# settylab/Mellon

Hardware: AMD Instinct MI355X
Metric: cells/sec fit_predict (higher is better)
Workload: dtype f64

## Files before the change

include/mellon_hip.h:

```cpp
#ifndef MELLON_HIP_H
#define MELLON_HIP_H

#include <stdint.h>

#ifdef __cplusplus
extern "C" {
#endif

typedef struct mln_ctx mln_ctx;
typedef struct mln_fit mln_fit;

typedef enum {
  MLN_OK = 0,
  MLN_ERR_NOT_PD = 1,
  MLN_ERR_SHAPE = 2,
  MLN_ERR_HIP = 3,
  MLN_ERR_RCCL = 4,
  MLN_ERR_ARG = 5,
  MLN_ERR_UNSUPPORTED = 6,
  MLN_ERR_NOCONV = 7
} mln_status;

typedef enum {
  MLN_K_MATERN32 = 1,
  MLN_K_MATERN52 = 2,
  MLN_K_EXPQUAD = 3,
  MLN_K_EXPONENTIAL = 4,
  MLN_K_RATQUAD = 5,
  MLN_K_LINEAR = 6,
  MLN_K_DISTANCE = 7
} mln_kind;

typedef struct {
  int32_t kind;
  int32_t ndims;
  double ls;
  double alpha;
  const int32_t* dims;
} mln_leaf;

typedef enum { MLN_OP_LEAF = 0, MLN_OP_CONST = 1, MLN_OP_ADD = 2, MLN_OP_MUL = 3, MLN_OP_POW = 4 } mln_op;

typedef struct {
  int32_t op;
  int32_t leaf;
  double value;
} mln_tok;

#define MLN_MAX_LEAVES 4
#define MLN_MAX_TOKS 16
#define MLN_MAX_DIMS 256

typedef struct {
  int32_t n_leaves;
  int32_t n_toks;
  const mln_leaf* leaves;
  const mln_tok* toks;
} mln_kernel_desc;

int mln_ctx_create(int device, mln_ctx** out);
void mln_ctx_destroy(mln_ctx* ctx);
const char* mln_last_error(mln_ctx* ctx);
int mln_device_info(mln_ctx* ctx, char* name, int name_cap, int* n_cu, int64_t* mem_bytes);
int mln_device_count(int* count_out);
int mln_synchronize(mln_ctx* ctx);

int mln_malloc(mln_ctx* ctx, int64_t bytes, void** dev_ptr);
int mln_free(mln_ctx* ctx, void* dev_ptr);
int mln_memcpy(mln_ctx* ctx, void* dst, const void* src, int64_t bytes);
int mln_host_register(mln_ctx* ctx, const void* host_ptr, int64_t bytes);
int mln_host_unregister(mln_ctx* ctx, const void* host_ptr);
int mln_release_cached_memory(void);
int mln_diag_alloc_stats(int64_t* out);

#define MLN_UNIQUE_ID_BYTES 128
int mln_comm_unique_id(void* id_out );
int mln_comm_init(mln_ctx* ctx, const void* id, int n_ranks, int rank);
int mln_comm_allreduce_sum(mln_ctx* ctx, double* buf, int64_t count);
typedef struct mln_loopback mln_loopback;
int mln_loopback_create(int n_ranks , mln_loopback** out);
void mln_loopback_destroy(mln_loopback* group);
int mln_comm_init_loopback(mln_ctx* ctx, mln_loopback* group, int rank);
typedef int (*mln_host_collective_fn)(void* user, int op, double* buf, double* buf2, int64_t count);
int mln_comm_init_host(mln_ctx* ctx, int n_ranks, int rank, mln_host_collective_fn fn, void* user);
void mln_loopback_abort(mln_loopback* group);
int mln_comm_info(mln_ctx* ctx, int32_t* info, double* stats, int32_t flags);

int mln_kernel_matrix(mln_ctx* ctx, const mln_kernel_desc* cov, const double* x, int64_t n,
                      const double* y, int64_t m, int32_t d, double* out);

int mln_kernel_gram(mln_ctx* ctx, const mln_kernel_desc* cov, const double* x, int64_t n_local, int32_t d,
                    const double* xu, int64_t m, double* out );
int mln_nn_distances(mln_ctx* ctx, const double* x, int64_t n, const double* y, int64_t m, int32_t d,
                     int64_t self_offset, double* out );
int mln_knn(mln_ctx* ctx, const double* x, int64_t n, const double* y, int64_t m, int32_t d, int32_t k,
            int32_t exclude, int64_t self_offset, double* dist , int64_t* idx );
int mln_local_dimensionality(mln_ctx* ctx, const double* x, int64_t n, int32_t d, const int64_t* nbr, int64_t q,
                             int32_t k, double* out );

int mln_kmeans(mln_ctx* ctx, const double* x, int64_t n, int32_t d, int64_t m, int64_t seed,
               int32_t max_iter, double tol, double* centers, int32_t* n_iter_out, double* inertia_out);
int mln_kmeans_sklearn(mln_ctx* ctx, const double* x, int64_t n, int32_t d, int64_t m, int64_t first_id,
                       const double* uniforms, int32_t n_local_trials, int32_t max_iter, double tol, double* centers,
                       int64_t* indices_out, int32_t* n_iter_out, double* inertia_out);

int mln_chol_lower(mln_ctx* ctx, double* A, int64_t m, double add_diag);

int mln_trsm_lower(mln_ctx* ctx, const double* Lf, int64_t m, int32_t trans, double* B, int64_t p);

#define MLN_FIT_IMPLICIT 1
int mln_fit_prepare(mln_ctx* ctx, const mln_kernel_desc* cov, const double* x, int64_t n_local,
                    int32_t d, const double* xu, int64_t m, double jitter, const double* Lp_in,
                    int32_t flags, mln_fit** out);
int mln_fit_from_L(mln_ctx* ctx, const double* L, int64_t n_local, int64_t m, const double* Lp,
                   mln_fit** out);
#define MLN_FIT_FULL 2
#define MLN_FIT_DEFER_LP 4
int mln_fit_prepare_from_K(mln_ctx* ctx, const double* Kuu, int64_t n_local, int64_t m, double jitter,
                           const double* Lp_in, int32_t flags, mln_fit** out);
int mln_fit_set_K_rows(mln_fit* fit, int64_t row0, int64_t n_rows, const double* K_rows);
int mln_fit_finish_K(mln_fit* fit);
int mln_gemm(mln_ctx* ctx, int32_t ta, int32_t tb, int64_t M, int64_t N, int64_t K, double alpha, const double* A,
             int64_t lda, const double* B, int64_t ldb, double beta, double* C, int64_t ldc);
int mln_ewise(mln_ctx* ctx, int32_t op, const double* a, const double* b, double scalar, double* out, int64_t count);

void mln_fit_destroy(mln_fit* fit);
int mln_fit_get_Lp(mln_fit* fit, double* out );
int mln_fit_get_L(mln_fit* fit, int64_t row0, int64_t n_rows, double* out );
int mln_fit_rank(mln_fit* fit, int64_t* m_out);

int mln_kernel_grad(mln_ctx* ctx, const mln_kernel_desc* cov, const double* x, int64_t n, const double* y,
                    int64_t m, int32_t d, double* out );
int mln_predict_gradient(mln_ctx* ctx, const mln_kernel_desc* cov, const double* xnew, int64_t n_new,
                         int32_t d, const double* centers, int64_t m, const double* W ,
                         double* out );
int mln_predict_hessian(mln_ctx* ctx, const mln_kernel_desc* cov, const double* xnew, int64_t n_new, int32_t d,
                        const double* centers, int64_t m, const double* W , double* out);


int mln_eigh(mln_ctx* ctx, const double* A, int64_t m, double* w, double* V, int32_t* n_sweeps);
int mln_fit_gram_eigh(mln_fit* fit, double* w , int32_t* n_sweeps);
int mln_fit_gram_rank(mln_fit* fit, double tol, int64_t* rank_out, double* sigma_max_out);
int mln_fit_project(mln_fit* fit, int64_t p, mln_fit** out);

int mln_ridge_init(mln_fit* fit, const double* target, double* z0 );

int mln_precond_build(mln_fit* fit, int64_t row_stride );
int mln_fit_set_row_offset(mln_fit* fit, int64_t global_row0);
int mln_precond_apply(mln_fit* fit, int32_t mode, const double* in, double* out);
int mln_objective_precond(mln_fit* fit, const double* u, double* loss, double* grad_u ,
                          double* z_out );

int mln_fit_set_likelihood(mln_fit* fit, const double* V, const double* Vdr, double mu);

int mln_objective(mln_fit* fit, const double* z, double* loss, double* grad ,
                  double* hess_diag );

int mln_objective_batch(mln_fit* fit, const double* Z, int32_t S, double* loss , double* grad );

typedef struct {
  int32_t maxiter;
  int32_t maxcor;
  int32_t maxls;
  double ftol;
  double gtol;
} mln_solver_opts;
int mln_map_solve(mln_fit* fit, const double* z0, const mln_solver_opts* opts ,
                  double* z_out , double* loss_out, int32_t* n_eval_out, int32_t* n_iter_out,
                  int32_t* status_out);

int mln_fit_set_dim_likelihood(mln_fit* fit, const double* ell, int32_t k, double mu_dim, double mu_dens);
int mln_dim_objective(mln_fit* fit, const double* z, double* loss, double* grad ,
                      double* hess_diag );

int mln_dim_objective_batch(mln_fit* fit, const double* Z, int32_t S, double* loss , double* grad );

int mln_transform(mln_fit* fit, const double* z, double mu, double* f_out );

int mln_weights_cholesky(mln_fit* fit, const double* z, double* w );
int mln_weights_full(mln_fit* fit, const double* y, int64_t p, double mu, double* w );

int mln_sparse_solve(mln_ctx* ctx, const mln_kernel_desc* cov, const double* x, int64_t n_local,
                     int32_t d, const double* xu, int64_t m, const double* y, int64_t p, double mu,
                     double sigma, double jitter, double* W );
int mln_sparse_solve_factors(mln_ctx* ctx, const mln_kernel_desc* cov, const double* x, int64_t n_local,
                             int32_t d, const double* xu, int64_t m, const double* y, int64_t p, double mu,
                             double sigma, double jitter, double* W, double* Lp_out, double* Cs_out);

enum { MLN_SIGMA_SCALAR = 0, MLN_SIGMA_PER_OUTPUT = 1, MLN_SIGMA_PER_CELL = 2 };
int mln_sparse_solve_noise(mln_ctx* ctx, const mln_kernel_desc* cov, const double* x, int64_t n_local,
                           int32_t d, const double* xu, int64_t m, const double* y, int64_t p, double mu,
                           const double* sigma, int32_t sigma_kind, double jitter, double* W );

int mln_full_conditional_noise(mln_ctx* ctx, const mln_kernel_desc* cov, const double* x, int64_t n, int32_t d,
                               const double* y, int64_t p, double mu, const double* sigma , double jitter,
                               double* W, double* leverage, double* corrected_r2, double* variance_W);

int mln_landmark_leverage(mln_ctx* ctx, const mln_kernel_desc* cov, const double* x, int64_t n_local, int32_t d,
                          const double* xu, int64_t m, const double* Lk, const double* sigma, int64_t p,
                          double jitter, double* out );

int mln_predict_mean(mln_ctx* ctx, const mln_kernel_desc* cov, const double* xnew, int64_t n_new,
                     int32_t d, const double* centers, int64_t m, const double* W, int64_t p,
                     double mu, double* out);

int mln_diag_peak(mln_ctx* ctx, int32_t what, int64_t bytes, double* result);
int mln_diag_dgemm(mln_ctx* ctx, int32_t ta, int32_t tb, int64_t M, int64_t N, int64_t K,
                   int32_t lower_only, int32_t split_k, int32_t reps, double* ms_out);
int mln_diag_dgemm_compare(mln_ctx* ctx, int32_t ta, int32_t tb, int64_t M, int64_t N, int64_t K, int32_t lower_only,
                           int32_t kmode, double beta, int32_t any_size, double* out);
int mln_diag_gram_i8(mln_ctx* ctx, const double* A, int64_t rows, int64_t m, double* out, int32_t reps, double* ms_out);
int mln_diag_overlap(mln_ctx* ctx, int64_t n, int64_t m, int32_t d, int64_t gram_rows, double* out );

int mln_predict_covariance(mln_ctx* ctx, const mln_kernel_desc* cov, const double* xnew, int64_t n_new,
                           int32_t d, const double* centers, int64_t m, const double* Lf, int32_t diag,
                           double* out);
int mln_predict_mean_covariance(mln_ctx* ctx, const mln_kernel_desc* cov, const double* xnew, int64_t n_new,
                                int32_t d, const double* centers, int64_t m, const double* W, int64_t q,
                                int32_t diag, double* out);

#define MLN_N_STAGE_TIMES 22
int mln_stage_times(mln_fit* fit, double* out );

#ifdef __cplusplus
}
#endif
#endif
```

mellon_amd/_lib.py:

```python
import ctypes as C
import os
import threading

import numpy as np

_HERE = os.path.dirname(os.path.abspath(__file__))
LIB_PATH = os.path.join(_HERE, "libmellon_hip.so")

MLN_OK, MLN_ERR_NOT_PD, MLN_ERR_SHAPE, MLN_ERR_HIP, MLN_ERR_RCCL, MLN_ERR_ARG, MLN_ERR_UNSUPPORTED = range(7)
MLN_UNIQUE_ID_BYTES = 128
MLN_N_STAGE_TIMES = 22

K_MATERN32, K_MATERN52, K_EXPQUAD, K_EXPONENTIAL, K_RATQUAD, K_LINEAR, K_DISTANCE = 1, 2, 3, 4, 5, 6, 7
OP_LEAF, OP_CONST, OP_ADD, OP_MUL, OP_POW = 0, 1, 2, 3, 4


HOST_COLLECTIVE_FN = C.CFUNCTYPE(C.c_int, C.c_void_p, C.c_int, C.c_void_p, C.c_void_p, C.c_int64)


class MellonHipError(RuntimeError):
    """HIP / RCCL / argument failure inside libmellon_hip.so."""


class Leaf(C.Structure):
    _fields_ = [("kind", C.c_int32), ("ndims", C.c_int32), ("ls", C.c_double), ("alpha", C.c_double),
                ("dims", C.POINTER(C.c_int32))]


class Tok(C.Structure):
    _fields_ = [("op", C.c_int32), ("leaf", C.c_int32), ("value", C.c_double)]


class SolverOpts(C.Structure):
    _fields_ = [("maxiter", C.c_int32), ("maxcor", C.c_int32), ("maxls", C.c_int32), ("ftol", C.c_double),
                ("gtol", C.c_double)]


class KernelDesc(C.Structure):
    _fields_ = [("n_leaves", C.c_int32), ("n_toks", C.c_int32), ("leaves", C.POINTER(Leaf)),
                ("toks", C.POINTER(Tok))]


_vp, _i64, _i32, _dbl, _dp = C.c_void_p, C.c_int64, C.c_int32, C.c_double, C.c_void_p
_KD = C.POINTER(KernelDesc)
SYMBOLS = [
    ("mln_ctx_create", C.c_int, [C.c_int, C.POINTER(_vp)]),
    ("mln_ctx_destroy", None, [_vp]),
    ("mln_last_error", C.c_char_p, [_vp]),
    ("mln_device_info", C.c_int, [_vp, C.c_char_p, C.c_int, C.POINTER(C.c_int), C.POINTER(_i64)]),
    ("mln_device_count", C.c_int, [C.POINTER(C.c_int)]),
    ("mln_synchronize", C.c_int, [_vp]),
    ("mln_malloc", C.c_int, [_vp, _i64, C.POINTER(_vp)]),
    ("mln_free", C.c_int, [_vp, _vp]),
    ("mln_memcpy", C.c_int, [_vp, _vp, _vp, _i64]),
    ("mln_host_register", C.c_int, [_vp, _vp, _i64]),
    ("mln_host_unregister", C.c_int, [_vp, _vp]),
    ("mln_release_cached_memory", C.c_int, []),
    ("mln_diag_alloc_stats", C.c_int, [_vp]),
    ("mln_comm_unique_id", C.c_int, [_vp]),
    ("mln_comm_init", C.c_int, [_vp, _vp, C.c_int, C.c_int]),
    ("mln_comm_allreduce_sum", C.c_int, [_vp, _dp, _i64]),
    ("mln_loopback_create", C.c_int, [C.c_int, C.POINTER(_vp)]),
    ("mln_loopback_destroy", None, [_vp]),
    ("mln_comm_init_loopback", C.c_int, [_vp, _vp, C.c_int]),
    ("mln_comm_init_host", C.c_int, [_vp, C.c_int, C.c_int, _vp, _vp]),
    ("mln_loopback_abort", None, [_vp]),
    ("mln_comm_info", C.c_int, [_vp, C.POINTER(_i32), _dp, _i32]),
    ("mln_kernel_matrix", C.c_int, [_vp, _KD, _dp, _i64, _dp, _i64, _i32, _dp]),
    ("mln_kernel_grad", C.c_int, [_vp, _KD, _dp, _i64, _dp, _i64, _i32, _dp]),
    ("mln_predict_gradient", C.c_int, [_vp, _KD, _dp, _i64, _i32, _dp, _i64, _dp, _dp]),
    ("mln_predict_hessian", C.c_int, [_vp, _KD, _dp, _i64, _i32, _dp, _i64, _dp, _dp]),
    ("mln_kernel_gram", C.c_int, [_vp, _KD, _dp, _i64, _i32, _dp, _i64, _dp]),
    ("mln_nn_distances", C.c_int, [_vp, _dp, _i64, _dp, _i64, _i32, _i64, _dp]),
    ("mln_knn", C.c_int, [_vp, _dp, _i64, _dp, _i64, _i32, _i32, _i32, _i64, _dp, _vp]),
    ("mln_local_dimensionality", C.c_int, [_vp, _dp, _i64, _i32, _vp, _i64, _i32, _dp]),
    ("mln_kmeans", C.c_int, [_vp, _dp, _i64, _i32, _i64, _i64, _i32, _dbl, _dp, C.POINTER(_i32), C.POINTER(_dbl)]),
    ("mln_kmeans_sklearn", C.c_int, [_vp, _dp, _i64, _i32, _i64, _i64, _dp, _i32, _i32, _dbl, _dp, _vp, C.POINTER(_i32),
                                     C.POINTER(_dbl)]),
    ("mln_chol_lower", C.c_int, [_vp, _dp, _i64, _dbl]),
    ("mln_trsm_lower", C.c_int, [_vp, _dp, _i64, _i32, _dp, _i64]),
    ("mln_fit_prepare", C.c_int, [_vp, _KD, _dp, _i64, _i32, _dp, _i64, _dbl, _dp, _i32, C.POINTER(_vp)]),
    ("mln_fit_from_L", C.c_int, [_vp, _dp, _i64, _i64, _dp, C.POINTER(_vp)]),
    ("mln_fit_prepare_from_K", C.c_int, [_vp, _dp, _i64, _i64, _dbl, _dp, _i32, C.POINTER(_vp)]),
    ("mln_fit_set_K_rows", C.c_int, [_vp, _i64, _i64, _dp]),
    ("mln_fit_finish_K", C.c_int, [_vp]),
    ("mln_gemm", C.c_int, [_vp, _i32, _i32, _i64, _i64, _i64, _dbl, _dp, _i64, _dp, _i64, _dbl, _dp, _i64]),
    ("mln_ewise", C.c_int, [_vp, _i32, _dp, _dp, _dbl, _dp, _i64]),
    ("mln_fit_destroy", None, [_vp]),
    ("mln_fit_get_Lp", C.c_int, [_vp, _dp]),
    ("mln_fit_get_L", C.c_int, [_vp, _i64, _i64, _dp]),
    ("mln_fit_rank", C.c_int, [_vp, C.POINTER(_i64)]),
    ("mln_eigh", C.c_int, [_vp, _dp, _i64, _dp, _dp, C.POINTER(_i32)]),
    ("mln_fit_gram_eigh", C.c_int, [_vp, _dp, C.POINTER(_i32)]),
    ("mln_fit_gram_rank", C.c_int, [_vp, _dbl, C.POINTER(_i64), C.POINTER(_dbl)]),
    ("mln_fit_project", C.c_int, [_vp, _i64, C.POINTER(_vp)]),
    ("mln_ridge_init", C.c_int, [_vp, _dp, _dp]),
    ("mln_precond_build", C.c_int, [_vp, _i64]),
    ("mln_fit_set_row_offset", C.c_int, [_vp, _i64]),
    ("mln_precond_apply", C.c_int, [_vp, _i32, _dp, _dp]),
    ("mln_objective_precond", C.c_int, [_vp, _dp, C.POINTER(_dbl), _dp, _dp]),
    ("mln_map_solve", C.c_int, [_vp, _dp, C.POINTER(SolverOpts), _dp, C.POINTER(_dbl), C.POINTER(_i32),
                                C.POINTER(_i32), C.POINTER(_i32)]),
    ("mln_fit_set_likelihood", C.c_int, [_vp, _dp, _dp, _dbl]),
    ("mln_objective", C.c_int, [_vp, _dp, C.POINTER(_dbl), _dp, _dp]),
    ("mln_objective_batch", C.c_int, [_vp, _dp, _i32, _dp, _dp]),
    ("mln_fit_set_dim_likelihood", C.c_int, [_vp, _dp, _i32, _dbl, _dbl]),
    ("mln_dim_objective", C.c_int, [_vp, _dp, C.POINTER(_dbl), _dp, _dp]),
    ("mln_dim_objective_batch", C.c_int, [_vp, _dp, _i32, _dp, _dp]),
    ("mln_transform", C.c_int, [_vp, _dp, _dbl, _dp]),
    ("mln_weights_cholesky", C.c_int, [_vp, _dp, _dp]),
    ("mln_weights_full", C.c_int, [_vp, _dp, _i64, _dbl, _dp]),
    ("mln_sparse_solve", C.c_int, [_vp, _KD, _dp, _i64, _i32, _dp, _i64, _dp, _i64, _dbl, _dbl, _dbl, _dp]),
    ("mln_sparse_solve_factors", C.c_int, [_vp, _KD, _dp, _i64, _i32, _dp, _i64, _dp, _i64, _dbl, _dbl, _dbl, _dp,
                                           _dp, _dp]),
    ("mln_sparse_solve_noise", C.c_int, [_vp, _KD, _dp, _i64, _i32, _dp, _i64, _dp, _i64, _dbl, _dp, _i32, _dbl, _dp]),
    ("mln_full_conditional_noise", C.c_int, [_vp, _KD, _dp, _i64, _i32, _dp, _i64, _dbl, _dp, _dbl, _dp, _dp, _dp, _dp]),
    ("mln_landmark_leverage", C.c_int, [_vp, _KD, _dp, _i64, _i32, _dp, _i64, _dp, _dp, _i64, _dbl, _dp]),
    ("mln_predict_mean", C.c_int, [_vp, _KD, _dp, _i64, _i32, _dp, _i64, _dp, _i64, _dbl, _dp]),
    ("mln_predict_covariance", C.c_int, [_vp, _KD, _dp, _i64, _i32, _dp, _i64, _dp, _i32, _dp]),
    ("mln_predict_mean_covariance", C.c_int, [_vp, _KD, _dp, _i64, _i32, _dp, _i64, _dp, _i64, _i32, _dp]),
    ("mln_stage_times", C.c_int, [_vp, _dp]),
    ("mln_diag_peak", C.c_int, [_vp, _i32, _i64, C.POINTER(_dbl)]),
    ("mln_diag_overlap", C.c_int, [_vp, _i64, _i64, _i32, _i64, _dp]),
    ("mln_diag_gram_i8", C.c_int, [_vp, _vp, _i64, _i64, _vp, _i32, C.POINTER(_dbl)]),
    ("mln_diag_dgemm", C.c_int, [_vp, _i32, _i32, _i64, _i64, _i64, _i32, _i32, _i32, C.POINTER(_dbl)]),
    ("mln_diag_dgemm_compare", C.c_int, [_vp, _i32, _i32, _i64, _i64, _i64, _i32, _i32, _dbl, _i32, C.POINTER(_dbl)]),
]

_lib = None
_lib_lock = threading.Lock()


def load_library():
    global _lib
    with _lib_lock:
        if _lib is not None:
            return _lib
        if not os.path.exists(LIB_PATH):
            raise MellonHipError(
                f"{LIB_PATH} is missing: build it with `python -c \"import __graft_entry__ as g; g.build()\"` "
                "(hipcc --offload-arch=gfx950).  mellon_amd has no CPU fallback.")
        lib = C.CDLL(LIB_PATH, mode=C.RTLD_GLOBAL)
        for name, res, args in SYMBOLS:
            fn = getattr(lib, name)
            fn.restype = res
            fn.argtypes = args
        _lib = lib
        return lib


def device_count():
    n = C.c_int(0)
    load_library().mln_device_count(C.byref(n))
    return int(n.value)


class BlockEvaluatedCov:
    rows_per_block = 8192

    def block(self, x, y):
        raise NotImplementedError


def _needs_program(desc, what):
    if isinstance(desc, BlockEvaluatedCov):
        raise NotImplementedError(
            f"{what} needs a covariance that lowers to one device program (built-in kernels combined with + * ** within "
            "the program limits); user-defined Python kernels and larger trees support k(), fit and the predictive mean.")


class DeviceArray:

    def __init__(self, ctx, shape):
        self.ctx = ctx
        self.shape = tuple(int(s) for s in shape)
        self.size = int(np.prod(self.shape)) if self.shape else 1
        ptr = C.c_void_p()
        ctx._check(ctx.lib.mln_malloc(ctx.handle, self.size * 8, C.byref(ptr)))
        self.ptr = ptr.value

    @property
    def nbytes(self):
        return self.size * 8

    @property
    def ndim(self):
        return len(self.shape)

    def to_host(self):
        out = np.empty(self.shape, dtype=np.float64)
        self.ctx._check(self.ctx.lib.mln_memcpy(self.ctx.handle, out.ctypes.data, self.ptr, self.nbytes))
        return out

    def free(self):
        if self.ptr is not None and self.ctx.handle is not None:
            self.ctx.lib.mln_free(self.ctx.handle, self.ptr)
        self.ptr = None

    def __del__(self):
        try:
            self.free()
        except Exception:
            pass


def _f64(a):
    return np.ascontiguousarray(a, dtype=np.float64)


def _ptr(a):
    if a is None:
        return None
    if isinstance(a, DeviceArray):
        return a.ptr
    return a.ctypes.data


class Context:

    def __init__(self, device=None):
        self.lib = load_library()
        if device is None:
            device = int(os.environ.get("LOCAL_RANK", "0")) if "MELLON_AMD_DEVICE" not in os.environ \
                else int(os.environ["MELLON_AMD_DEVICE"])
        h = C.c_void_p()
        rc = self.lib.mln_ctx_create(int(device), C.byref(h))
        self.handle = None
        if rc != MLN_OK:
            msg = self.lib.mln_last_error(None).decode()
            raise MellonHipError(f"mln_ctx_create(device={device}) failed: {msg}")
        self.handle = h.value
        self.device = int(device)
        self.n_ranks, self.rank = 1, 0

    def close(self):
        if self.handle is not None:
            self.lib.mln_ctx_destroy(self.handle)
            self.handle = None

    def __del__(self):
        try:
            self.close()
        except Exception:
            pass

    def _check(self, rc, jitter=None):
        if rc == MLN_OK:
            return
        msg = self.lib.mln_last_error(self.handle).decode()
        if rc == MLN_ERR_NOT_PD:
            raise ValueError(
                f"Covariance not positively definite with jitter={jitter}. "
                "Consider increasing the jitter for numerical stabilization.")
        if rc == MLN_ERR_SHAPE:
            raise ValueError(f"libmellon_hip: {msg}")
        if rc == MLN_ERR_UNSUPPORTED:
            raise NotImplementedError(f"libmellon_hip: {msg}")
        cause = None
        staged = getattr(self, "_host_collective", None)
        if staged is not None and getattr(staged[1], "failure", None) is not None:
            cause, staged[1].failure = staged[1].failure, None
        raise MellonHipError(f"libmellon_hip error {rc}: {msg}" + (f" ({type(cause).__name__}: {cause})" if cause else "")) from cause

    def device_info(self):
        name = C.create_string_buffer(64)
        cu, mem = C.c_int(), C.c_int64()
        self._check(self.lib.mln_device_info(self.handle, name, 64, C.byref(cu), C.byref(mem)))
        return {"arch": name.value.decode(), "n_cu": cu.value, "mem_bytes": mem.value}

    def synchronize(self):
        self._check(self.lib.mln_synchronize(self.handle))

    def to_device(self, a):
        a = _f64(a)
        d = DeviceArray(self, a.shape)
        self._check(self.lib.mln_memcpy(self.handle, d.ptr, a.ctypes.data, a.nbytes))
        return d

    def empty(self, shape):
        return DeviceArray(self, shape)

    def pinned(self, a):
        return _Pinned(self, a)

    def comm_unique_id(self):
        buf = C.create_string_buffer(MLN_UNIQUE_ID_BYTES)
        self._check(self.lib.mln_comm_unique_id(buf))
        return buf.raw

    def comm_init(self, unique_id, n_ranks, rank):
        buf = C.create_string_buffer(bytes(unique_id), MLN_UNIQUE_ID_BYTES)
        self._check(self.lib.mln_comm_init(self.handle, buf, int(n_ranks), int(rank)))
        self.n_ranks, self.rank = int(n_ranks), int(rank)

    def comm_init_host(self, n_ranks, rank, collective):
        fn = HOST_COLLECTIVE_FN(collective)
        self._check(self.lib.mln_comm_init_host(self.handle, int(n_ranks), int(rank), C.cast(fn, C.c_void_p), None))
        self._host_collective = (fn, collective)
        self.n_ranks, self.rank = int(n_ranks), int(rank)

    def comm_info(self, timing=None, reset=False):
        info = (_i32 * 4)()
        stats = np.zeros(10, dtype=np.float64)
        flags = (1 if timing is True else 2 if timing is False else 0) | (4 if reset else 0)
        self._check(self.lib.mln_comm_info(self.handle, info, stats.ctypes.data, flags))
        names = {0: "none", 1: "rccl", 2: "loopback", 3: "host"}
        return {"transport": names.get(int(info[0]), "?"), "ranks_reported_by_transport": int(info[1]),
                "rank_reported_by_transport": int(info[2]), "rccl_version_code": int(info[3]),
                "allreduce_calls": int(stats[0]), "allreduce_bytes": float(stats[1]),
                "broadcast_calls": int(stats[2]), "broadcast_bytes": float(stats[3]),
                "allgather_calls": int(stats[4]), "allgather_bytes": float(stats[5]),
                "small_allreduce_calls": int(stats[6]), "large_allreduce_ms": float(stats[7]),
                "broadcast_allgather_ms": float(stats[8]), "small_allreduce_ms": float(stats[9])}

    def comm_init_loopback(self, group, rank):
        self._check(self.lib.mln_comm_init_loopback(self.handle, group.handle, int(rank)))
        self._loop_group = group
        self.n_ranks, self.rank = group.n_ranks, int(rank)

    def allreduce_sum(self, a):
        if isinstance(a, DeviceArray):
            self._check(self.lib.mln_comm_allreduce_sum(self.handle, a.ptr, a.size))
            return a
        a = _f64(a).copy()
        self._check(self.lib.mln_comm_allreduce_sum(self.handle, a.ctypes.data, a.size))
        return a

    def kernel_matrix(self, desc, x, y):
        x, y = _as2d(x), _as2d(y)
        if x.shape[1] != y.shape[1]:
            raise ValueError("x and y must have the same number of features")
        if isinstance(desc, BlockEvaluatedCov):
            out = np.empty((x.shape[0], y.shape[0]), dtype=np.float64)
            for i0 in range(0, x.shape[0], desc.rows_per_block):
                blk = desc.block(x[i0:i0 + desc.rows_per_block], y)
                out[i0:i0 + desc.rows_per_block] = blk.to_host() if isinstance(blk, DeviceArray) else blk
            return out
        out = np.empty((x.shape[0], y.shape[0]), dtype=np.float64)
        self._check(self.lib.mln_kernel_matrix(self.handle, desc.ref, _ptr(x), x.shape[0], _ptr(y), y.shape[0],
                                               x.shape[1], out.ctypes.data))
        return out

    def kernel_gram(self, desc, x, xu):
        if isinstance(desc, BlockEvaluatedCov):
            xh = x.to_host() if isinstance(x, DeviceArray) else _as2d(x)
            xu = _as2d(xu)
            G = self.to_device(np.zeros((xu.shape[0], xu.shape[0])))
            for i0 in range(0, xh.shape[0], desc.rows_per_block):
                blk = desc.block(xh[i0:i0 + desc.rows_per_block], xu)
                self.gemm(blk, blk, ta=True, out=G, beta=1.0)
            G = self.allreduce_sum(G)
            return G.to_host()
        x = x if isinstance(x, DeviceArray) else _as2d(x)
        xu = _as2d(xu)
        out = np.empty((xu.shape[0], xu.shape[0]), dtype=np.float64)
        self._check(self.lib.mln_kernel_gram(self.handle, desc.ref, _ptr(x), x.shape[0], x.shape[1], _ptr(xu),
                                             xu.shape[0], out.ctypes.data))
        return out

    def kernel_grad(self, desc, x, y):
        _needs_program(desc, "kernel_grad")
        x, y = _as2d(x), _as2d(y)
        if x.shape[1] != y.shape[1]:
            raise ValueError("x and y must have the same number of features")
        out = np.empty((x.shape[0], y.shape[0], x.shape[1]), dtype=np.float64)
        self._check(self.lib.mln_kernel_grad(self.handle, desc.ref, _ptr(x), x.shape[0], _ptr(y), y.shape[0],
                                             x.shape[1], out.ctypes.data))
        return out

    def predict_gradient(self, desc, xnew, centers, W):
        _needs_program(desc, "predict_gradient")
        xnew = xnew if isinstance(xnew, DeviceArray) else _as2d(xnew)
        centers = centers if isinstance(centers, DeviceArray) else _as2d(centers)
        Wd = _f64(W)
        if Wd.ndim != 1 or Wd.shape[0] != centers.shape[0]:
            raise NotImplementedError("gradients are available for single-output predictors (weights of shape (m,))")
        n_new, d = xnew.shape
        out = np.empty((n_new, d), dtype=np.float64)
        self._check(self.lib.mln_predict_gradient(self.handle, desc.ref, _ptr(xnew), n_new, d, _ptr(centers),
                                                  centers.shape[0], Wd.ctypes.data, out.ctypes.data))
        return out


    def predict_hessian(self, desc, xnew, centers, W):
        _needs_program(desc, "predict_hessian")
        xnew = xnew if isinstance(xnew, DeviceArray) else _as2d(xnew)
        centers = centers if isinstance(centers, DeviceArray) else _as2d(centers)
        Wd = _f64(W)
        if Wd.ndim != 1 or Wd.shape[0] != centers.shape[0]:
            raise NotImplementedError("hessians are available for single-output predictors (weights of shape (m,))")
        n_new, d = xnew.shape
        out = np.empty((n_new, d, d), dtype=np.float64)
        self._check(self.lib.mln_predict_hessian(self.handle, desc.ref, _ptr(xnew), n_new, d, _ptr(centers),
                                                 centers.shape[0], Wd.ctypes.data, out.ctypes.data))
        return out

    def nn_distances(self, x, y=None, self_offset=0):
        x = x if isinstance(x, DeviceArray) else _as2d(x)
        y = x if y is None else (y if isinstance(y, DeviceArray) else _as2d(y))
        out = np.empty(x.shape[0], dtype=np.float64)
        self._check(self.lib.mln_nn_distances(self.handle, _ptr(x), x.shape[0], _ptr(y), y.shape[0], x.shape[1],
                                              int(self_offset), out.ctypes.data))
        return out

    KNN_MAX_K = 64

    def knn(self, x, k, y=None, exclude_self=False, self_offset=0, return_index=True):
        x = x if isinstance(x, DeviceArray) else _as2d(x)
        y = x if y is None else (y if isinstance(y, DeviceArray) else _as2d(y))
        k = int(k)
        avail = y.shape[0] - (1 if exclude_self else 0)
        if not 1 <= k <= self.KNN_MAX_K or k > avail:
            raise ValueError(f"k={k} is outside [1, min({self.KNN_MAX_K}, {avail})] for {y.shape[0]} candidate rows")
        if x.shape[1] != y.shape[1]:
            raise ValueError(f"x has {x.shape[1]} features, y has {y.shape[1]}")
        n = x.shape[0]
        dist = np.empty((n, k), dtype=np.float64)
        idx = np.empty((n, k), dtype=np.int64) if return_index else None
        self._check(self.lib.mln_knn(self.handle, _ptr(x), n, _ptr(y), y.shape[0], x.shape[1], k, int(bool(exclude_self)),
                                     int(self_offset), dist.ctypes.data, None if idx is None else idx.ctypes.data))
        return (dist, idx) if return_index else dist

    def local_dimensionality(self, x, neighbor_idx):
        x = x if isinstance(x, DeviceArray) else _as2d(x)
        nbr = np.ascontiguousarray(neighbor_idx, dtype=np.int64)
        if nbr.ndim != 2:
            raise ValueError(f"neighbor_idx must be 2-d, got shape {nbr.shape}")
        q, k = nbr.shape
        if not 2 <= k <= self.KNN_MAX_K:
            raise ValueError(f"neighbourhoods of {k} rows: the local dimension needs 2 ... {self.KNN_MAX_K}")
        if nbr.size and (nbr.min() < -x.shape[0] or nbr.max() >= x.shape[0]):
            raise IndexError(f"neighbor_idx outside [0, {x.shape[0]})")
        nbr = np.where(nbr < 0, nbr + x.shape[0], nbr)
        out = np.empty(q, dtype=np.float64)
        self._check(self.lib.mln_local_dimensionality(self.handle, _ptr(x), x.shape[0], x.shape[1], nbr.ctypes.data, q, k,
                                                      out.ctypes.data))
        return out

    def kmeans(self, x, m, seed=42, max_iter=300, tol=1e-4, return_info=False, init="device"):
        x = x if isinstance(x, DeviceArray) else _as2d(x)
        centers = np.empty((int(m), x.shape[1]), dtype=np.float64)
        nit, inertia = C.c_int32(), C.c_double()
        if init == "sklearn":
            if not sklearn_seeding_compatible():
                import warnings
                warnings.warn("kmeans(init='sklearn'): the installed sklearn does not draw its k-means++ seeds the way this "
                              "library replays them (or is not importable); the seeds are k-means++ seeds of RandomState(seed), "
                              "but not necessarily the cells sklearn.cluster.k_means would pick.", RuntimeWarning)
            first, uni, trials = sklearn_seeding_numbers(x.shape[0], int(m), seed)
            idx = np.empty(int(m), dtype=np.int64)
            self._check(self.lib.mln_kmeans_sklearn(self.handle, _ptr(x), x.shape[0], x.shape[1], int(m), int(first),
                                                    uni.ctypes.data, trials, int(max_iter), float(tol), centers.ctypes.data,
                                                    idx.ctypes.data, C.byref(nit), C.byref(inertia) if return_info else None))
            self.last_kmeans_seed_indices = idx
            return (centers, nit.value, inertia.value) if return_info else centers
        if init != "device":
            raise ValueError("init must be 'device' or 'sklearn'")
        self._check(self.lib.mln_kmeans(self.handle, _ptr(x), x.shape[0], x.shape[1], int(m), int(seed),
                                        int(max_iter), float(tol), centers.ctypes.data, C.byref(nit),
                                        C.byref(inertia) if return_info else None))
        return (centers, nit.value, inertia.value) if return_info else centers

    def chol_lower(self, A, add_diag=0.0, jitter=None):
        A = _f64(A).copy()
        if A.ndim != 2 or A.shape[0] != A.shape[1]:
            raise ValueError("A must be square")
        self._check(self.lib.mln_chol_lower(self.handle, A.ctypes.data, A.shape[0], float(add_diag)),
                    jitter=add_diag if jitter is None else jitter)
        return A

    def eigh(self, A):
        A = _f64(A)
        if A.ndim != 2 or A.shape[0] != A.shape[1]:
            raise ValueError("A must be square")
        m = A.shape[0]
        w, V, sw = np.empty(m), np.empty((m, m)), _i32(0)
        self._check(self.lib.mln_eigh(self.handle, A.ctypes.data, m, w.ctypes.data, V.ctypes.data, C.byref(sw)))
        self.last_eigh_sweeps = int(sw.value)
        return w, V

    def trsm_lower(self, Lf, B, trans=False):
        Lf = _f64(Lf)
        B2 = _f64(B).copy()
        shape = B2.shape
        B2 = B2.reshape(Lf.shape[0], -1)
        self._check(self.lib.mln_trsm_lower(self.handle, Lf.ctypes.data, Lf.shape[0], 1 if trans else 0,
                                            B2.ctypes.data, B2.shape[1]))
        return B2.reshape(shape)

    def predict_mean(self, desc, xnew, centers, W, mu, out=None):
        xnew = xnew if isinstance(xnew, DeviceArray) else _as2d(xnew)
        centers = centers if isinstance(centers, DeviceArray) else _as2d(centers)
        Wd = W if isinstance(W, DeviceArray) else _f64(W)
        n_new, d = xnew.shape
        m = centers.shape[0]
        p = 1 if len(Wd.shape) == 1 else Wd.shape[1]
        shape = (n_new,) if len(Wd.shape) == 1 else (n_new, p)
        if out is not None:
            if not isinstance(out, DeviceArray) or tuple(out.shape) != shape:
                raise ValueError(f"out must be a DeviceArray of shape {shape}")
            _needs_program(desc, "predict_mean(out=DeviceArray)")
            self._check(self.lib.mln_predict_mean(self.handle, desc.ref, _ptr(xnew), n_new, d, _ptr(centers), m,
                                                  _ptr(Wd), p, float(mu), out.ptr))
            return out
        out = np.empty(shape, dtype=np.float64)
        if isinstance(desc, BlockEvaluatedCov):
            xh = xnew.to_host() if isinstance(xnew, DeviceArray) else xnew
            ch = centers.to_host() if isinstance(centers, DeviceArray) else centers
            W2 = Wd if isinstance(Wd, DeviceArray) else self.to_device(np.ascontiguousarray(Wd.reshape(m, p)))
            for i0 in range(0, n_new, desc.rows_per_block):
                blk = desc.block(xh[i0:i0 + desc.rows_per_block], ch)
                res = self.gemm(blk, W2).to_host() + float(mu)
                out[i0:i0 + desc.rows_per_block] = res[:, 0] if out.ndim == 1 else res
            return out
        self._check(self.lib.mln_predict_mean(self.handle, desc.ref, _ptr(xnew), n_new, d, _ptr(centers), m,
                                              _ptr(Wd), p, float(mu), out.ctypes.data))
        return out

    def _rows_sq_blocks(self, desc, xnew, centers, Mt, diag):
        xnew, centers = _as2d(xnew), _as2d(centers)
        Md = self.to_device(np.ascontiguousarray(Mt))
        n = xnew.shape[0]
        if not diag:
            blk = desc.block(xnew, centers)
            T = self.gemm(blk if isinstance(blk, DeviceArray) else self.to_device(blk), Md)
            return self.gemm(T, T, tb=True).to_host()
        out = np.empty(n)
        ones = self.to_device(np.ones((Md.shape[1], 1)))
        for i0 in range(0, n, desc.rows_per_block):
            blk = desc.block(xnew[i0:i0 + desc.rows_per_block], centers)
            T = self.gemm(blk if isinstance(blk, DeviceArray) else self.to_device(blk), Md)
            out[i0:i0 + desc.rows_per_block] = self.gemm(self.ewise(OP_MUL, T, T), ones).to_host()[:, 0]
        return out

    def predict_covariance(self, desc, xnew, centers, Lf, diag=True):
        if isinstance(desc, BlockEvaluatedCov):
            Lf = _f64(Lf)
            LinvT = np.ascontiguousarray(self.trsm_lower(Lf, np.eye(Lf.shape[0])).T)
            kss = desc.diag(_as2d(xnew)) if diag else desc.block(_as2d(xnew), _as2d(xnew))
            kss = kss.to_host() if isinstance(kss, DeviceArray) else kss
            return kss - self._rows_sq_blocks(desc, xnew, centers, LinvT, diag)
        xnew, centers, Lf = _as2d(xnew), _as2d(centers), _f64(Lf)
        n = xnew.shape[0]
        out = np.empty((n,) if diag else (n, n), dtype=np.float64)
        self._check(self.lib.mln_predict_covariance(self.handle, desc.ref, _ptr(xnew), n, xnew.shape[1],
                                                    _ptr(centers), centers.shape[0], _ptr(Lf), 1 if diag else 0,
                                                    out.ctypes.data))
        return out

    def predict_mean_covariance(self, desc, xnew, centers, W, diag=True):
        if isinstance(desc, BlockEvaluatedCov):
            return self._rows_sq_blocks(desc, xnew, centers, _as2d(W), diag)
        xnew, centers, W = _as2d(xnew), _as2d(centers), _as2d(W)
        n = xnew.shape[0]
        out = np.empty((n,) if diag else (n, n), dtype=np.float64)
        self._check(self.lib.mln_predict_mean_covariance(self.handle, desc.ref, _ptr(xnew), n, xnew.shape[1],
                                                         _ptr(centers), centers.shape[0], _ptr(W), W.shape[1],
                                                         1 if diag else 0, out.ctypes.data))
        return out

    def sparse_solve(self, desc, x, xu, y, mu, sigma, jitter, return_factors=False):
        if isinstance(desc, BlockEvaluatedCov):
            W, Lp, Cs = self._sparse_solve_blocks(desc, x, xu, y, mu, np.array([float(sigma)]), jitter, return_factors)
            return (W, Lp, Cs) if return_factors else W
        x = x if isinstance(x, DeviceArray) else _as2d(x)
        xu = _as2d(xu)
        y2 = y if isinstance(y, DeviceArray) else _f64(y)
        y_ndim = len(y2.shape)
        m = xu.shape[0]
        p = 1 if y_ndim == 1 else y2.shape[1]
        W = np.empty((m,) if y_ndim == 1 else (m, p), dtype=np.float64)
        if not return_factors:
            self._check(self.lib.mln_sparse_solve(self.handle, desc.ref, _ptr(x), x.shape[0], x.shape[1], _ptr(xu),
                                                  m, _ptr(y2), p, float(mu), float(sigma),
                                                  float(jitter), W.ctypes.data), jitter=jitter)
            return W
        Lp, Cs = np.empty((m, m)), np.empty((m, m))
        self._check(self.lib.mln_sparse_solve_factors(self.handle, desc.ref, _ptr(x), x.shape[0], x.shape[1],
                                                      _ptr(xu), m, _ptr(y2), p, float(mu), float(sigma),
                                                      float(jitter), W.ctypes.data, Lp.ctypes.data,
                                                      Cs.ctypes.data), jitter=jitter)
        return W, Lp, Cs

    SIGMA_SCALAR, SIGMA_PER_OUTPUT, SIGMA_PER_CELL = 0, 1, 2

    def _sparse_solve_blocks(self, desc, x, xu, y, mu, sigma, jitter, return_factors):
        xh = x.to_host() if isinstance(x, DeviceArray) else _as2d(x)
        xu = _as2d(xu)
        yh = y.to_host() if isinstance(y, DeviceArray) else _f64(y)
        y_ndim = yh.ndim
        r = (yh - float(mu)).reshape(xh.shape[0], -1)
        m, p = xu.shape[0], r.shape[1]
        if sigma.shape[0] not in (1, p):
            raise ValueError(f"sigma has shape {sigma.shape}, expected (1,) or ({p},)")
        G, R = self.to_device(np.zeros((m, m))), self.to_device(np.zeros((m, p)))
        for i0 in range(0, xh.shape[0], desc.rows_per_block):
            blk = desc.block(xh[i0:i0 + desc.rows_per_block], xu)
            blk = blk if isinstance(blk, DeviceArray) else self.to_device(blk)
            self.gemm(blk, blk, ta=True, out=G, beta=1.0)
            self.gemm(blk, np.ascontiguousarray(r[i0:i0 + desc.rows_per_block]), ta=True, out=R, beta=1.0)
        G, R = self.allreduce_sum(G).to_host(), self.allreduce_sum(R).to_host()
        Kuu = desc.block(xu, xu)
        Kuu = Kuu.to_host() if isinstance(Kuu, DeviceArray) else Kuu
        Lp = self.chol_lower(Kuu, add_diag=float(jitter))
        T = self.trsm_lower(Lp, G)
        AAt = self.trsm_lower(Lp, np.ascontiguousarray(T.T))
        AAt = 0.5 * (AAt + AAt.T)
        Ar = self.trsm_lower(Lp, R)
        W = np.empty((m, p))
        Cs = None
        sig_cols = np.broadcast_to(sigma, (p,))
        for sg in np.unique(sig_cols):
            cols = np.nonzero(sig_cols == sg)[0]
            s2 = float(sg) ** 2
            L_B = self.chol_lower(AAt / s2, add_diag=1.0)
            c = self.trsm_lower(L_B, np.ascontiguousarray(Ar[:, cols]) / s2)
            W[:, cols] = self.trsm_lower(Lp, self.trsm_lower(L_B, c, trans=True), trans=True)
            if return_factors:
                Cs = self.gemm(Lp, L_B).to_host()
        W = W[:, 0] if y_ndim == 1 else W
        return W, Lp, Cs

    def sparse_solve_noise(self, desc, x, xu, y, mu, sigma, kind, jitter):
        if isinstance(desc, BlockEvaluatedCov):
            if kind == self.SIGMA_PER_CELL:
                _needs_program(desc, "sparse_solve_noise with one sigma per cell")
            return self._sparse_solve_blocks(desc, x, xu, y, mu, _f64(np.atleast_1d(sigma)), jitter, False)[0]
        x = x if isinstance(x, DeviceArray) else _as2d(x)
        xu = _as2d(xu)
        y2 = _f64(y)
        sig = _f64(np.atleast_1d(sigma))
        m = xu.shape[0]
        p = 1 if y2.ndim == 1 else y2.shape[1]
        want = {self.SIGMA_SCALAR: 1, self.SIGMA_PER_OUTPUT: p, self.SIGMA_PER_CELL: x.shape[0]}[kind]
        if sig.shape != (want,):
            raise ValueError(f"sigma has shape {sig.shape}, expected {(want,)} for noise kind {kind}")
        W = np.empty((m,) if y2.ndim == 1 else (m, p), dtype=np.float64)
        self._check(self.lib.mln_sparse_solve_noise(self.handle, desc.ref, _ptr(x), x.shape[0], x.shape[1], _ptr(xu),
                                                    m, y2.ctypes.data, p, float(mu), sig.ctypes.data, int(kind),
                                                    float(jitter), W.ctypes.data), jitter=jitter)
        return W

    def full_conditional_noise(self, desc, x, y, mu, sigma, jitter, leverage=False, obs_variance=False):
        _needs_program(desc, "full_conditional_noise")
        x = _as2d(x)
        y2 = np.ascontiguousarray(_f64(y))
        sig = _f64(np.atleast_1d(sigma))
        n, p = y2.shape
        if sig.shape != (p,) or x.shape[0] != n:
            raise ValueError("sigma must hold one value per output column and x, y must agree in length")
        leverage = leverage or obs_variance
        W = np.empty((n, p))
        H = np.empty((n, p)) if leverage else None
        Cr, VW = (np.empty((n, p)), np.empty((n, p))) if obs_variance else (None, None)
        ptr = lambda a: None if a is None else a.ctypes.data
        self._check(self.lib.mln_full_conditional_noise(self.handle, desc.ref, _ptr(x), n, x.shape[1], y2.ctypes.data, p,
                                                        float(mu), sig.ctypes.data, float(jitter), W.ctypes.data,
                                                        ptr(H), ptr(Cr), ptr(VW)), jitter=jitter)
        if obs_variance:
            return W, H, Cr, VW
        return (W, H) if leverage else W

    def pairwise_distance(self, x, y):
        from .base_cov import LoweredCov
        d = _as2d(x).shape[1]
        desc = LoweredCov([(K_DISTANCE, 1.0, 1.0, np.arange(d))], [(OP_LEAF, 0, 0.0)])
        return self.kernel_matrix(desc, x, y)

    def landmark_leverage(self, desc, x, xu, Lk, sigma, jitter):
        _needs_program(desc, "landmark_leverage")
        x = x if isinstance(x, DeviceArray) else _as2d(x)
        xu = _as2d(xu)
        Lk = _f64(Lk)
        sig = _f64(np.atleast_1d(sigma))
        m = xu.shape[0]
        if Lk.shape != (m, m):
            raise ValueError(f"Lk has shape {Lk.shape}, expected {(m, m)}")
        out = np.empty((x.shape[0], sig.shape[0]), dtype=np.float64)
        self._check(self.lib.mln_landmark_leverage(self.handle, desc.ref, _ptr(x), x.shape[0], x.shape[1], _ptr(xu), m,
                                                   Lk.ctypes.data, sig.ctypes.data, sig.shape[0], float(jitter),
                                                   out.ctypes.data), jitter=jitter)
        return out

    def diag_overlap(self, n, m, d, gram_rows):
        out = np.zeros(6)
        self._check(self.lib.mln_diag_overlap(self.handle, int(n), int(m), int(d), int(gram_rows), out.ctypes.data))
        return dict(zip(["k_ms", "gram_ms", "k_par_gram_ms", "chol_ms", "k_par_chol_ms", "k_par_chol_gram_ms"], out))

    def diag_gram_i8(self, a, reps=1):
        a = np.ascontiguousarray(a, dtype=np.float64)
        out = np.empty((a.shape[1], a.shape[1]))
        ms = C.c_double()
        self._check(self.lib.mln_diag_gram_i8(self.handle, a.ctypes.data, a.shape[0], a.shape[1], out.ctypes.data, int(reps),
                                              C.byref(ms)))
        return out, ms.value

    def diag_peak(self, what, nbytes=1 << 32):
        r = C.c_double()
        self._check(self.lib.mln_diag_peak(self.handle, int(what), int(nbytes), C.byref(r)))
        return r.value

    def diag_dgemm(self, ta, tb, M, N, K, lower_only=0, split_k=1, reps=3):
        r = C.c_double()
        self._check(self.lib.mln_diag_dgemm(self.handle, ta, tb, M, N, K, lower_only, split_k, reps, C.byref(r)))
        return r.value

    def fit_prepare(self, desc, x, landmarks, jitter, Lp=None, implicit=False):
        if isinstance(desc, BlockEvaluatedCov):
            return Fit.from_blocks(self, desc, x, landmarks, jitter, Lp, implicit)
        return Fit(self, desc, x, landmarks, jitter, Lp, implicit)

    def diag_dgemm_compare(self, ta, tb, M, N, K, lower_only=0, kmode=0, beta=0.0, any_size=True):
        r = (C.c_double * 2)()
        self._check(self.lib.mln_diag_dgemm_compare(self.handle, int(ta), int(tb), M, N, K, lower_only, kmode, float(beta),
                                                    1 if any_size else 0, r))
        return float(r[0]), float(r[1])

    def diag_dgemm_batch(self, ta, tb, M, N, K, lower_only=0, kmode=0, beta=0.0):
        r = (C.c_double * 2)()
        self._check(self.lib.mln_diag_dgemm_compare(self.handle, int(ta), int(tb), M, N, K, lower_only, kmode, float(beta), 2, r))
        return float(r[0])

    def gemm(self, A, B, ta=False, tb=False, alpha=1.0, beta=0.0, out=None):
        A = A if isinstance(A, DeviceArray) else _as2d(A)
        B = B if isinstance(B, DeviceArray) else _as2d(B)
        M, K = (A.shape[1], A.shape[0]) if ta else A.shape
        Kb, N = (B.shape[1], B.shape[0]) if tb else B.shape
        if K != Kb:
            raise ValueError(f"gemm: inner dimensions differ ({K} vs {Kb})")
        if out is None:
            out = self.empty((M, N))
            beta = 0.0
        if tuple(out.shape) != (M, N):
            raise ValueError(f"gemm: out has shape {tuple(out.shape)}, expected {(M, N)}")
        self._check(self.lib.mln_gemm(self.handle, 1 if ta else 0, 1 if tb else 0, M, N, K, float(alpha), _ptr(A),
                                      A.shape[1], _ptr(B), B.shape[1], float(beta), _ptr(out), N))
        return out

    def ewise(self, op, a, b, out=None):
        a = a if isinstance(a, DeviceArray) else self.to_device(a)
        out = a if out is None else out
        scalar = 0.0
        bp = None
        if isinstance(b, (int, float, np.floating, np.integer)):
            scalar = float(b)
        else:
            b = b if isinstance(b, DeviceArray) else self.to_device(b)
            if tuple(b.shape) != tuple(a.shape):
                raise ValueError("ewise: shapes differ")
            bp = b.ptr
        self._check(self.lib.mln_ewise(self.handle, int(op), a.ptr, bp, scalar, out.ptr, a.size))
        return out


class LoopbackGroup:

    def __init__(self, n_ranks):
        self.lib = load_library()
        h = C.c_void_p()
        if self.lib.mln_loopback_create(int(n_ranks), C.byref(h)) != MLN_OK:
            raise MellonHipError(f"mln_loopback_create({n_ranks}) failed")
        self.handle, self.n_ranks = h.value, int(n_ranks)

    def abort(self):
        if self.handle is not None:
            self.lib.mln_loopback_abort(self.handle)

    def __del__(self):
        try:
            if self.handle is not None:
                self.lib.mln_loopback_destroy(self.handle)
            self.handle = None
        except Exception:
            pass


def _as2d(a):
    a = _f64(a)
    if a.ndim == 1:
        a = a.reshape(-1, 1)
    return np.ascontiguousarray(a)


def sklearn_seeding_numbers(n, m, seed):
    rs = np.random.RandomState(seed)
    trials = 2 + int(np.log(m))
    sw = np.ones(n, dtype=np.float64)
    first = int(rs.choice(n, p=sw / sw.sum()))
    uni = np.ascontiguousarray(rs.uniform(size=(max(m - 1, 0), trials)), dtype=np.float64)
    return first, uni, trials


_sklearn_seeding_ok = None


def sklearn_seeding_compatible():
    global _sklearn_seeding_ok
    if _sklearn_seeding_ok is not None:
        return _sklearn_seeding_ok
    try:
        from sklearn.cluster import kmeans_plusplus
        n, m, seed = 60, 6, 11
        g = np.random.RandomState(5)
        x = np.ascontiguousarray(g.normal(size=(n, 3)) + 20.0 * g.randint(0, 6, size=(n, 1)))
        _, want = kmeans_plusplus(x, m, random_state=seed)
        first, uni, trials = sklearn_seeding_numbers(n, m, seed)
        got = [first]
        d2 = ((x - x[first]) ** 2).sum(1)
        for c in range(1, m):
            cand = np.searchsorted(np.cumsum(d2), uni[c - 1] * d2.sum())
            cand = np.clip(cand, None, n - 1)
            dc = ((x[cand][:, None, :] - x[None, :, :]) ** 2).sum(2)
            pots = np.minimum(d2[None, :], dc).sum(1)
            best = int(np.argmin(pots))
            got.append(int(cand[best]))
            d2 = np.minimum(d2, dc[best])
        _sklearn_seeding_ok = [int(v) for v in want] == got
    except Exception:
        _sklearn_seeding_ok = False
    return _sklearn_seeding_ok


class _Pinned:
    def __init__(self, ctx, a):
        if not (isinstance(a, np.ndarray) and a.flags.c_contiguous):
            raise TypeError("pinned(): a C-contiguous NumPy array is required")
        self.ctx, self.a, self.on = ctx, a, False

    def __enter__(self):
        self.ctx._check(self.ctx.lib.mln_host_register(self.ctx.handle, self.a.ctypes.data, self.a.nbytes))
        self.on = True
        return self.a

    def __exit__(self, *exc):
        if self.on:
            self.on = False
            self.ctx._check(self.ctx.lib.mln_host_unregister(self.ctx.handle, self.a.ctypes.data))
        return False


class Fit:

    @classmethod
    def from_L(cls, ctx, L, Lp=None):
        self = cls.__new__(cls)
        self.ctx, self.lib, self.handle = ctx, ctx.lib, None
        L = L if isinstance(L, DeviceArray) else _as2d(L)
        n, m = L.shape
        Lp_ = None if Lp is None else _f64(Lp)
        if Lp_ is not None and Lp_.shape != (m, m):
            raise ValueError(f"Lp has shape {Lp_.shape}, expected {(m, m)}")
        h = C.c_void_p()
        ctx._check(self.lib.mln_fit_from_L(ctx.handle, _ptr(L), n, m, _ptr(Lp_), C.byref(h)))
        self.handle = h.value
        self.n, self.d, self.m, self.jitter = n, None, m, None
        self.implicit = False
        self._has_lp = Lp_ is not None
        return self

    @classmethod
    def from_blocks(cls, ctx, cov, x, landmarks, jitter, Lp=None, implicit=False):
        self = cls.__new__(cls)
        self.ctx, self.lib, self.handle = ctx, ctx.lib, None
        xh = x.to_host() if isinstance(x, DeviceArray) else _as2d(x)
        n, d = xh.shape
        full = landmarks is None
        xu = xh if full else (landmarks.to_host() if isinstance(landmarks, DeviceArray) else _as2d(landmarks))
        m = xu.shape[0]
        self.implicit = bool(implicit) and not full
        Lp_ = None if Lp is None else _f64(Lp)
        if Lp_ is not None and Lp_.shape != (m, m):
            raise ValueError(f"Lp has shape {Lp_.shape}, expected {(m, m)}")
        Kuu = None
        if Lp_ is None:
            Kuu = cov.block(xu, xu)
        flags = (1 if self.implicit else 0) | (2 if full else 0)
        h = C.c_void_p()
        ctx._check(self.lib.mln_fit_prepare_from_K(ctx.handle, _ptr(Kuu), n, m, float(jitter), _ptr(Lp_), flags,
                                                   C.byref(h)), jitter=jitter)
        self.handle = h.value
        self.n, self.d, self.m, self.jitter = n, d, m, jitter
        self._has_lp = True
        if not full:
            for i0 in range(0, n, cov.rows_per_block):
                blk = cov.block(xh[i0:i0 + cov.rows_per_block], xu)
                rows = min(cov.rows_per_block, n - i0)
                if tuple(blk.shape) != (rows, m):
                    raise ValueError(f"covariance returned a block of shape {tuple(blk.shape)}, expected {(rows, m)}")
                blk = blk if isinstance(blk, DeviceArray) else _f64(blk)
                ctx._check(self.lib.mln_fit_set_K_rows(self.handle, i0, rows, _ptr(blk)))
        ctx._check(self.lib.mln_fit_finish_K(self.handle))
        return self

    def gram_eigh(self):
        w, sw = np.empty(self.m), _i32(0)
        self._check(self.lib.mln_fit_gram_eigh(self.handle, w.ctypes.data, C.byref(sw)))
        self.last_eigh_sweeps = int(sw.value)
        return w

    def gram_rank(self, tol):
        r, smax = _i64(0), C.c_double()
        self._check(self.lib.mln_fit_gram_rank(self.handle, float(tol), C.byref(r), C.byref(smax)))
        return int(r.value), smax.value

    def project(self, p):
        new = Fit.__new__(Fit)
        new.ctx, new.lib, new.handle = self.ctx, self.lib, None
        h = C.c_void_p()
        self._check(self.lib.mln_fit_project(self.handle, int(p), C.byref(h)))
        new.handle = h.value
        new.n, new.d, new.m, new.jitter = self.n, None, int(p), None
        new.implicit = False
        new._has_lp = False
        return new

    def __init__(self, ctx, desc, x, landmarks, jitter, Lp=None, implicit=False):
        self.ctx, self.lib, self.handle = ctx, ctx.lib, None
        self.implicit = bool(implicit) and landmarks is not None
        x = x if isinstance(x, DeviceArray) else _as2d(x)
        n, d = x.shape
        xu = None if landmarks is None else (landmarks if isinstance(landmarks, DeviceArray) else _as2d(landmarks))
        m = n if xu is None else xu.shape[0]
        Lp_ = None if Lp is None else _f64(Lp)
        if Lp_ is not None and Lp_.shape != (m, m):
            raise ValueError(f"Lp has shape {Lp_.shape}, expected {(m, m)}")
        h = C.c_void_p()
        flags = (1 | (4 if Lp_ is None else 0)) if self.implicit else 0
        ctx._check(self.lib.mln_fit_prepare(ctx.handle, desc.ref, _ptr(x), n, d, _ptr(xu), m, float(jitter),
                                            _ptr(Lp_), flags, C.byref(h)), jitter=jitter)
        self.handle = h.value
        self.n, self.d, self.m, self.jitter = n, d, m, jitter
        self._has_lp = True

    def _check(self, rc, jitter=None):
        if rc == MLN_ERR_NOT_PD and self.lib.mln_last_error(self.ctx.handle).startswith(b"cov(xu, xu)"):
            jitter = self.jitter
        self.ctx._check(rc, jitter=jitter)

    def close(self):
        if self.handle is not None and self.ctx.handle is not None:
            self.lib.mln_fit_destroy(self.handle)
        self.handle = None

    def __del__(self):
        try:
            self.close()
        except Exception:
            pass

    def Lp(self):
        out = np.empty((self.m, self.m), dtype=np.float64)
        self._check(self.lib.mln_fit_get_Lp(self.handle, out.ctypes.data))
        return out

    def L(self, row0=0, n_rows=None):
        n_rows = self.n - row0 if n_rows is None else n_rows
        out = np.empty((n_rows, self.m), dtype=np.float64)
        self._check(self.lib.mln_fit_get_L(self.handle, row0, n_rows, out.ctypes.data))
        return out

    def ridge_init(self, target):
        target = target if isinstance(target, DeviceArray) else _f64(target)
        z0 = np.empty(self.m, dtype=np.float64)
        self._check(self.lib.mln_ridge_init(self.handle, _ptr(target), z0.ctypes.data), jitter="ridge")
        return z0

    def set_likelihood(self, V, Vdr, mu):
        V = V if isinstance(V, DeviceArray) else _f64(V)
        Vdr = Vdr if isinstance(Vdr, DeviceArray) else _f64(Vdr)
        self._check(self.lib.mln_fit_set_likelihood(self.handle, _ptr(V), _ptr(Vdr), float(mu)))

    def objective(self, z, with_hess=False):
        z = _f64(z)
        loss = C.c_double()
        grad = np.empty(self.m, dtype=np.float64)
        hess = np.empty(self.m, dtype=np.float64) if with_hess else None
        self._check(self.lib.mln_objective(self.handle, z.ctypes.data, C.byref(loss), grad.ctypes.data,
                                               _ptr(hess)))
        return (loss.value, grad, hess) if with_hess else (loss.value, grad)

    def objective_batch(self, Z):
        Z = _f64(Z)
        if Z.ndim != 2 or Z.shape[1] != self.m or Z.shape[0] < 1:
            raise ValueError(f"Z has shape {Z.shape}, expected (S >= 1, {self.m})")
        loss = np.empty(Z.shape[0], dtype=np.float64)
        grad = np.empty(Z.shape, dtype=np.float64)
        self._check(self.lib.mln_objective_batch(self.handle, Z.ctypes.data, int(Z.shape[0]), loss.ctypes.data,
                                                 grad.ctypes.data))
        return loss, grad

    def set_dim_likelihood(self, ell, mu_dim, mu_dens):
        ell = _f64(ell)
        if ell.ndim != 2 or ell.shape[0] != self.n:
            raise ValueError(f"ell has shape {ell.shape}, expected ({self.n}, k)")
        self._check(self.lib.mln_fit_set_dim_likelihood(self.handle, ell.ctypes.data, int(ell.shape[1]), float(mu_dim),
                                                        float(mu_dens)))

    def dim_objective(self, z, with_hess=False):
        z = _f64(z)
# ... 109 lines not shown
```

mellon_amd/csrc/api.hip:

```cpp
#include "api_internal.h"

static thread_local std::string g_last_error;

void mln_set_error(mln_ctx* ctx, const std::string& msg) {
  g_last_error = msg;
  if (ctx) ctx->err = msg;
}

int mln_hip_fail(mln_ctx* ctx, hipError_t e, const char* what, const char* file, int line) {
  mln_set_error(ctx, std::string("HIP error ") + hipGetErrorString(e) + " in " + what + " (" + file + ":" +
                         std::to_string(line) + ")");
  (void)hipGetLastError();
  return MLN_ERR_HIP;
}

double now_s() {
  return std::chrono::duration<double>(std::chrono::steady_clock::now().time_since_epoch()).count();
}

bool is_device_ptr(const void* p) {
  if (!p) return false;
  hipPointerAttribute_t attr;
  hipError_t e = hipPointerGetAttributes(&attr, p);
  if (e != hipSuccess) { (void)hipGetLastError(); return false; }
// ... 31 lines not shown
    out->leaves[l].kind = lf.kind; out->leaves[l].ndims = lf.ndims; out->leaves[l].dims_off = off;
    out->leaves[l].ls = lf.ls; out->leaves[l].alpha = lf.alpha;
    out->leaves[l].alpha_inv_ls[0] = lf.alpha; out->leaves[l].alpha_inv_ls[1] = 1.0 / lf.ls;
    for (int k = 0; k < lf.ndims; ++k) {
      if (lf.dims[k] < 0 || lf.dims[k] >= d) { mln_set_error(ctx, "active dim out of range"); return MLN_ERR_SHAPE; }
      out->dims[off + k] = (short)lf.dims[k];
    }
    off += lf.ndims;
  }
  int depth = 0;
  for (int t = 0; t < cov->n_toks; ++t) {
    const mln_tok& tk = cov->toks[t];
    out->tok_op[t] = tk.op; out->tok_leaf[t] = tk.leaf; out->tok_val[t] = tk.value;
    if (tk.op == MLN_OP_LEAF) {
      if (tk.leaf < 0 || tk.leaf >= cov->n_leaves) { mln_set_error(ctx, "token references unknown leaf"); return MLN_ERR_ARG; }
      ++depth;
    } else if (tk.op == MLN_OP_CONST) {
      ++depth;
    } else if (tk.op == MLN_OP_ADD || tk.op == MLN_OP_MUL || tk.op == MLN_OP_POW) {
      if (depth < 2) { mln_set_error(ctx, "malformed covariance program"); return MLN_ERR_ARG; }
      --depth;
    } else { mln_set_error(ctx, "unknown token op"); return MLN_ERR_ARG; }
    if (depth > 3) { mln_set_error(ctx, "covariance expression nests deeper than the device stack (3)"); return MLN_ERR_UNSUPPORTED; }
  }
  if (depth != 1) { mln_set_error(ctx, "malformed covariance program"); return MLN_ERR_ARG; }
  if (cov->n_toks == 1 && cov->toks[0].op != MLN_OP_LEAF) { mln_set_error(ctx, "constant covariance"); return MLN_ERR_ARG; }
  return MLN_OK;
}

extern "C" const char* mln_last_error(mln_ctx* ctx) { return ctx ? ctx->err.c_str() : g_last_error.c_str(); }

extern "C" int mln_ctx_create(int device, mln_ctx** out) {
  if (!out) return MLN_ERR_ARG;
  *out = nullptr;
  int count = 0;
  hipError_t e = hipGetDeviceCount(&count);
  if (e != hipSuccess || count <= 0) {
    (void)hipGetLastError();
    mln_set_error(nullptr, "no HIP device visible: libmellon_hip has no CPU fallback");
    return MLN_ERR_HIP;
  }
  if (device < 0 || device >= count) { mln_set_error(nullptr, "device index out of range"); return MLN_ERR_ARG; }
  hipDeviceProp_t prop;
  if (hipGetDeviceProperties(&prop, device) != hipSuccess) { mln_set_error(nullptr, "hipGetDeviceProperties failed"); return MLN_ERR_HIP; }
  if (std::strncmp(prop.gcnArchName, "gfx950", 6) != 0) {
    mln_set_error(nullptr, std::string("device is ") + prop.gcnArchName + "; this library is built for gfx950 only");
    return MLN_ERR_UNSUPPORTED;
  }
  mln_ctx* ctx = new mln_ctx();
  ctx->device = device;
  ctx->n_cu = prop.multiProcessorCount;
  if (hipSetDevice(device) != hipSuccess || hipStreamCreate(&ctx->stream) != hipSuccess ||
      ctx->d_info.alloc(ctx, 4, "d_info") != MLN_OK) {
    mln_set_error(nullptr, "failed to initialise the HIP context");
    delete ctx;
    return MLN_ERR_HIP;
  }
  *out = ctx;
  return MLN_OK;
}

void fit_release_copy_lane(mln_ctx* ctx);

extern "C" void mln_ctx_destroy(mln_ctx* ctx) {
  if (!ctx) return;
  (void)hipSetDevice(ctx->device);
  (void)hipStreamSynchronize(ctx->stream);
  comm_release(ctx);
  fit_release_copy_lane(ctx);
  ctx->scratch.reset();
  ctx->d_info.reset();
  (void)hipStreamDestroy(ctx->stream);
  delete ctx;
}

extern "C" int mln_device_info(mln_ctx* ctx, char* name, int name_cap, int* n_cu, int64_t* mem_bytes) {
  if (!ctx) return MLN_ERR_ARG;
  hipDeviceProp_t prop;
  MLN_HIP(ctx, hipGetDeviceProperties(&prop, ctx->device));
  if (name && name_cap > 0) { std::strncpy(name, prop.gcnArchName, name_cap - 1); name[name_cap - 1] = 0; }
  if (n_cu) *n_cu = prop.multiProcessorCount;
  if (mem_bytes) *mem_bytes = (int64_t)prop.totalGlobalMem;
  return MLN_OK;
}

extern "C" int mln_device_count(int* count_out) {
  if (!count_out) return MLN_ERR_ARG;
  int count = 0;
  if (hipGetDeviceCount(&count) != hipSuccess) { (void)hipGetLastError(); count = 0; }
  *count_out = count;
  return MLN_OK;
}

extern "C" int mln_synchronize(mln_ctx* ctx) {
  if (!ctx) return MLN_ERR_ARG;
  MLN_HIP(ctx, hipStreamSynchronize(ctx->stream));
  return MLN_OK;
}

extern "C" int mln_malloc(mln_ctx* ctx, int64_t bytes, void** dev_ptr) {
  if (!ctx || !dev_ptr || bytes < 0) return MLN_ERR_ARG;
  MLN_HIP(ctx, hipSetDevice(ctx->device));
  MLN_HIP(ctx, hipMalloc(dev_ptr, (size_t)(bytes > 0 ? bytes : 8)));
  return MLN_OK;
}

extern "C" int mln_free(mln_ctx* ctx, void* dev_ptr) {
  if (!ctx) return MLN_ERR_ARG;
  if (dev_ptr) { MLN_HIP(ctx, hipStreamSynchronize(ctx->stream)); MLN_HIP(ctx, hipFree(dev_ptr)); }
  return MLN_OK;
}

extern "C" int mln_host_register(mln_ctx* ctx, const void* host_ptr, int64_t bytes) {
  if (!ctx || !host_ptr || bytes < 1) return MLN_ERR_ARG;
  MLN_HIP(ctx, hipSetDevice(ctx->device));
  MLN_HIP(ctx, hipHostRegister(const_cast<void*>(host_ptr), (size_t)bytes, hipHostRegisterDefault));
  return MLN_OK;
}

extern "C" int mln_host_unregister(mln_ctx* ctx, const void* host_ptr) {
  if (!ctx || !host_ptr) return MLN_ERR_ARG;
  MLN_HIP(ctx, hipSetDevice(ctx->device));
  MLN_HIP(ctx, hipStreamSynchronize(ctx->stream));
  MLN_HIP(ctx, hipHostUnregister(const_cast<void*>(host_ptr)));
  return MLN_OK;
}

extern "C" int mln_release_cached_memory(void) {
  mln_dcache_flush();
  return MLN_OK;
}

extern "C" int mln_memcpy(mln_ctx* ctx, void* dst, const void* src, int64_t bytes) {
  if (!ctx || bytes < 0 || (bytes > 0 && (!dst || !src))) return MLN_ERR_ARG;
  if (bytes == 0) return MLN_OK;
  MLN_HIP(ctx, hipMemcpyAsync(dst, src, (size_t)bytes, hipMemcpyDefault, ctx->stream));
  MLN_HIP(ctx, hipStreamSynchronize(ctx->stream));
  return MLN_OK;
}

int dev_allreduce(mln_ctx* ctx, double* dev, int64_t count) { return comm_allreduce(ctx, dev, count); }
int dev_bcast0(mln_ctx* ctx, double* dev, int64_t count) { return comm_bcast0(ctx, dev, count); }

extern "C" int mln_comm_allreduce_sum(mln_ctx* ctx, double* buf, int64_t count) {
  if (!ctx || (count > 0 && !buf)) return MLN_ERR_ARG;
  if (!ctx->comm && !ctx->loop && ctx->n_ranks <= 1) return MLN_OK;
  MLN_HIP(ctx, hipSetDevice(ctx->device));
  DevOut o;
  MLN_TRY(o.init(ctx, buf, (size_t)count, true));
  MLN_TRY(dev_allreduce(ctx, o.dev, count));
  return o.commit();
}

extern "C" int mln_kernel_matrix(mln_ctx* ctx, const mln_kernel_desc* cov, const double* x, int64_t n,
                                 const double* y, int64_t m, int32_t d, double* out) {
  if (!ctx) return MLN_ERR_ARG;
  if (n < 0 || m < 0 || d < 1) { mln_set_error(ctx, "bad shape"); return MLN_ERR_SHAPE; }
  if (n == 0 || m == 0) return MLN_OK;
  if (!x || !y || !out) return MLN_ERR_ARG;
  MLN_HIP(ctx, hipSetDevice(ctx->device));
  DevCov dc;
  MLN_TRY(mln_lower_cov(ctx, cov, d, &dc));
  DevIn dx, dy;
  DevOut o;
  MLN_TRY(dx.init(ctx, x, (size_t)n * d));
  MLN_TRY(dy.init(ctx, y, (size_t)m * d));
  MLN_TRY(o.init(ctx, out, (size_t)n * m));
  MLN_TRY(launch_kernel_matrix(ctx, dc, dx.dev, n, dy.dev, m, d, o.dev, m, 0.0));
  return o.commit();
}

int reject_distance_leaf(mln_ctx* ctx, const DevCov& dc) {
  for (int l = 0; l < dc.n_leaves; ++l)
    if (dc.leaves[l].kind == MLN_K_DISTANCE) {
      mln_set_error(ctx, "MLN_K_DISTANCE is a value-only leaf: no derivatives");
      return MLN_ERR_UNSUPPORTED;
    }
  return MLN_OK;
}

extern "C" int mln_kernel_grad(mln_ctx* ctx, const mln_kernel_desc* cov, const double* x, int64_t n,
                               const double* y, int64_t m, int32_t d, double* out) {
  if (!ctx) return MLN_ERR_ARG;
  if (n < 0 || m < 0 || d < 1) { mln_set_error(ctx, "bad shape"); return MLN_ERR_SHAPE; }
  if (n == 0 || m == 0) return MLN_OK;
  if (!x || !y || !out) return MLN_ERR_ARG;
  MLN_HIP(ctx, hipSetDevice(ctx->device));
  DevCov dc;
  MLN_TRY(mln_lower_cov(ctx, cov, d, &dc));
  MLN_TRY(reject_distance_leaf(ctx, dc));
  DevIn dx, dy;
  DevOut o;
  MLN_TRY(dx.init(ctx, x, (size_t)n * d));
  MLN_TRY(dy.init(ctx, y, (size_t)m * d));
  MLN_TRY(o.init(ctx, out, (size_t)n * m * d));
  MLN_TRY(launch_kernel_grad(ctx, dc, dx.dev, n, dy.dev, m, d, 0, o.dev));
  return o.commit();
}

extern "C" int mln_predict_gradient(mln_ctx* ctx, const mln_kernel_desc* cov, const double* xnew, int64_t n_new,
                                    int32_t d, const double* centers, int64_t m, const double* W, double* out) {
  if (!ctx) return MLN_ERR_ARG;
  if (n_new < 0 || m < 0 || d < 1) { mln_set_error(ctx, "bad shape"); return MLN_ERR_SHAPE; }
  if (n_new == 0) return MLN_OK;
  if (!xnew || !out || (m > 0 && (!centers || !W))) return MLN_ERR_ARG;
  MLN_HIP(ctx, hipSetDevice(ctx->device));
  DevCov dc;
  MLN_TRY(mln_lower_cov(ctx, cov, d, &dc));
  MLN_TRY(reject_distance_leaf(ctx, dc));
  DevIn dx, dc_, dw;
  DevOut o;
  MLN_TRY(dx.init(ctx, xnew, (size_t)n_new * d));
  MLN_TRY(dc_.init(ctx, centers, (size_t)m * d));
  MLN_TRY(dw.init(ctx, W, (size_t)m));
  MLN_TRY(o.init(ctx, out, (size_t)n_new * d));
  MLN_TRY(launch_predict_gradient(ctx, dc, dx.dev, n_new, dc_.dev, m, d, dw.dev, o.dev));
  return o.commit();
}

extern "C" int mln_predict_hessian(mln_ctx* ctx, const mln_kernel_desc* cov, const double* xnew, int64_t n_new,
                                   int32_t d, const double* centers, int64_t m, const double* W, double* out) {
  if (!ctx) return MLN_ERR_ARG;
  if (n_new < 0 || m < 1 || d < 1) { mln_set_error(ctx, "bad shape"); return MLN_ERR_SHAPE; }
  if (n_new == 0) return MLN_OK;
  if (!xnew || !out || !centers || !W) return MLN_ERR_ARG;
  MLN_HIP(ctx, hipSetDevice(ctx->device));
  DevCov dc;
  MLN_TRY(mln_lower_cov(ctx, cov, d, &dc));
  MLN_TRY(reject_distance_leaf(ctx, dc));
  DevIn dx, dc_, dw;
  DevOut o;
  MLN_TRY(dx.init(ctx, xnew, (size_t)n_new * d));
  MLN_TRY(dc_.init(ctx, centers, (size_t)m * d));
  MLN_TRY(dw.init(ctx, W, (size_t)m));
  MLN_TRY(o.init(ctx, out, (size_t)n_new * d * d));
  MLN_TRY(launch_predict_hessian(ctx, dc, dx.dev, n_new, dc_.dev, m, d, dw.dev, o.dev));
  return o.commit();
}


extern "C" int mln_kernel_gram(mln_ctx* ctx, const mln_kernel_desc* cov, const double* x, int64_t n, int32_t d,
                               const double* xu, int64_t m, double* out) {
  if (!ctx) return MLN_ERR_ARG;
  if (n < 0 || m < 1 || d < 1) { mln_set_error(ctx, "bad shape"); return MLN_ERR_SHAPE; }
  if (!xu || !out || (n > 0 && !x)) return MLN_ERR_ARG;
  MLN_HIP(ctx, hipSetDevice(ctx->device));
  DevCov dc;
  MLN_TRY(mln_lower_cov(ctx, cov, d, &dc));
  DevIn dx, du;
  DevOut o;
  if (n > 0) MLN_TRY(dx.init(ctx, x, (size_t)n * d));
  MLN_TRY(du.init(ctx, xu, (size_t)m * d));
  MLN_TRY(o.init(ctx, out, (size_t)m * m));
  const int64_t ld = pad16(m);
  const int64_t chunk = (n < 65536) ? (n > 0 ? n : 1) : 65536;
  DevBuf<double> K, G, acc;
  MLN_TRY(K.alloc(ctx, (size_t)chunk * ld, "K"));
  MLN_TRY(G.alloc(ctx, (size_t)m * ld, "G"));
  MLN_TRY(acc.alloc(ctx, (size_t)m * ld, "acc"));
  int rc = (hipMemsetAsync(acc, 0, sizeof(double) * (size_t)m * ld, ctx->stream) == hipSuccess) ? MLN_OK : MLN_ERR_HIP;
  bool any = false;
  for (int64_t r0 = 0; (r0 < n || !any) && rc == MLN_OK; r0 += chunk) {
    const int64_t rows = (n - r0 < chunk) ? (n - r0 > 0 ? n - r0 : 0) : chunk;
    if (rows > 0) rc = launch_kernel_matrix(ctx, dc, dx.dev + r0 * d, rows, du.dev, m, d, K, ld, 0.0);
    if (rc == MLN_OK) rc = gram_of(ctx, K, ld, rows, m, 1.0, G, ld);
    if (rc == MLN_OK) rc = launch_axpby(ctx, m * ld, 1.0, G, 1.0, acc);
    any = true;
    if (n == 0) break;
  }
  if (rc == MLN_OK) rc = launch_copy_block(ctx, acc, ld, o.dev, m, m, m);
  if (rc == MLN_OK) rc = o.commit();
  (void)hipStreamSynchronize(ctx->stream);
  return rc;
}

extern "C" int mln_nn_distances(mln_ctx* ctx, const double* x, int64_t n, const double* y, int64_t m, int32_t d,
                                int64_t self_offset, double* out) {
  if (!ctx) return MLN_ERR_ARG;
  if (n < 0 || m < 0 || d < 1) { mln_set_error(ctx, "bad shape"); return MLN_ERR_SHAPE; }
  if (n == 0) return MLN_OK;
  if (!x || !y || !out) return MLN_ERR_ARG;
  MLN_HIP(ctx, hipSetDevice(ctx->device));
  DevIn dx, dy;
  DevOut o;
  MLN_TRY(dx.init(ctx, x, (size_t)n * d));
  if (y == x && m == n) dy.dev = dx.dev, dy.ctx = ctx; else MLN_TRY(dy.init(ctx, y, (size_t)m * d));
  MLN_TRY(o.init(ctx, out, (size_t)n));
  MLN_TRY(launch_nn_distances(ctx, dx.dev, n, dy.dev, m, d, self_offset, o.dev));
  return o.commit();
}

int64_t pad16(int64_t m) { return ((m + 15) / 16) * 16; }

extern "C" int mln_chol_lower(mln_ctx* ctx, double* A, int64_t m, double add_diag) {
  if (!ctx || (m > 0 && !A)) return MLN_ERR_ARG;
  if (m < 0 || m > 65535) { mln_set_error(ctx, "cholesky: m out of range"); return MLN_ERR_SHAPE; }
  if (m == 0) return MLN_OK;
  MLN_HIP(ctx, hipSetDevice(ctx->device));
  DevOut o;
  MLN_TRY(o.init(ctx, A, (size_t)m * m, true));
  if (add_diag != 0.0) MLN_TRY(launch_add_diag(ctx, o.dev, m, m, add_diag));
  MLN_TRY(dev_cholesky_lower(ctx, o.dev, m, m));
  return o.commit();
}

extern "C" int mln_trsm_lower(mln_ctx* ctx, const double* Lf, int64_t m, int32_t trans, double* B, int64_t p) {
  if (!ctx || (m > 0 && (!Lf || (p > 0 && !B)))) return MLN_ERR_ARG;
  if (m < 0 || p < 0) return MLN_ERR_SHAPE;
  if (m == 0 || p == 0) return MLN_OK;
  MLN_HIP(ctx, hipSetDevice(ctx->device));
  DevIn dl;
  DevOut b;
  MLN_TRY(dl.init(ctx, Lf, (size_t)m * m));
  MLN_TRY(b.init(ctx, B, (size_t)m * p, true));
  TriInv t;
  MLN_TRY(triinv_build(ctx, dl.dev, m, m, trans == 0, trans != 0, &t));
  int rc = trans == 0 ? triinv_solve_left(ctx, t, b.dev, p, p) : triinv_solve_left_T(ctx, t, b.dev, p, p);
  if (rc == MLN_OK) rc = b.commit();
  (void)hipStreamSynchronize(ctx->stream);
  return rc;
}

__global__ void k_ewise(int op, const double* __restrict__ a, const double* __restrict__ b, double scalar,
                        double* __restrict__ out, int64_t count) {
  for (int64_t i = blockIdx.x * (int64_t)blockDim.x + threadIdx.x; i < count; i += (int64_t)gridDim.x * blockDim.x) {
    const double l = a[i], r = b ? b[i] : scalar;
    out[i] = op == MLN_OP_ADD ? l + r : (op == MLN_OP_MUL ? l * r : pow(l, r));
  }
}

extern "C" int mln_ewise(mln_ctx* ctx, int32_t op, const double* a, const double* b, double scalar, double* out,
                         int64_t count) {
  if (!ctx || count < 0 || (count > 0 && (!a || !out))) return MLN_ERR_ARG;
  if (op != MLN_OP_ADD && op != MLN_OP_MUL && op != MLN_OP_POW) { mln_set_error(ctx, "mln_ewise: unknown operation"); return MLN_ERR_ARG; }
  if (count == 0) return MLN_OK;
  MLN_HIP(ctx, hipSetDevice(ctx->device));
  DevIn da, db;
  DevOut o;
  const bool alias = (out == a);
  MLN_TRY(o.init(ctx, out, (size_t)count, alias));
  if (alias && is_device_ptr(a)) da.dev = a; else if (alias) da.dev = o.dev; else MLN_TRY(da.init(ctx, a, (size_t)count));
  if (b) MLN_TRY(db.init(ctx, b, (size_t)count));
  const int64_t blocks = std::min<int64_t>((count + 255) / 256, 65535);
  hipLaunchKernelGGL(k_ewise, dim3((unsigned)blocks), dim3(256), 0, ctx->stream, op, da.dev, b ? db.dev : nullptr, scalar, o.dev, count);
  MLN_HIP(ctx, hipGetLastError());
  return o.commit();
}

extern "C" int mln_gemm(mln_ctx* ctx, int32_t ta, int32_t tb, int64_t M, int64_t N, int64_t K, double alpha,
                        const double* A, int64_t lda, const double* B, int64_t ldb, double beta, double* Cm, int64_t ldc) {
  if (!ctx || M < 0 || N < 0 || K < 0) return MLN_ERR_ARG;
  if (M == 0 || N == 0) return MLN_OK;
  if (!A || !B || !Cm) return MLN_ERR_ARG;
  const int64_t ar = ta ? K : M, ac = ta ? M : K, br = tb ? N : K, bc = tb ? K : N;
  if (lda < ac || ldb < bc || ldc < N) { mln_set_error(ctx, "mln_gemm: leading dimension too small"); return MLN_ERR_SHAPE; }
  MLN_HIP(ctx, hipSetDevice(ctx->device));
  DevIn da, db;
  DevOut oc;
  const bool a_dev = is_device_ptr(A), b_dev = is_device_ptr(B), c_dev = is_device_ptr(Cm);
  std::vector<double> ha, hb, hc;
  const double* Ah = A; const double* Bh = B;
  int64_t lda_d = lda, ldb_d = ldb, ldc_d = ldc;
  if (!a_dev && lda != ac) { ha.resize((size_t)ar * ac); for (int64_t r = 0; r < ar; ++r) std::memcpy(&ha[(size_t)r * ac], A + r * lda, sizeof(double) * ac); Ah = ha.data(); }
  if (!b_dev && ldb != bc) { hb.resize((size_t)br * bc); for (int64_t r = 0; r < br; ++r) std::memcpy(&hb[(size_t)r * bc], B + r * ldb, sizeof(double) * bc); Bh = hb.data(); }
  if (!a_dev) lda_d = ac;
  if (!b_dev) ldb_d = bc;
  MLN_TRY(da.init(ctx, Ah, a_dev ? 1 : (size_t)ar * ac));
  MLN_TRY(db.init(ctx, Bh, b_dev ? 1 : (size_t)br * bc));
  if (a_dev) da.dev = A;
  if (b_dev) db.dev = B;
  double* Cd = Cm;
  DevBuf<double> c_owned;
  if (!c_dev) {
    ldc_d = (N + 1) & ~(int64_t)1;
    MLN_TRY(c_owned.alloc(ctx, (size_t)M * ldc_d, "c_owned"));
    Cd = c_owned;
    if (beta != 0.0)
      MLN_HIP(ctx, hipMemcpy2DAsync(Cd, sizeof(double) * ldc_d, Cm, sizeof(double) * ldc, sizeof(double) * N, (size_t)M, hipMemcpyHostToDevice, ctx->stream));
  }
  GemmArgs g{};
  g.A = da.dev; g.lda = lda_d; g.B = db.dev; g.ldb = ldb_d; g.C = Cd; g.ldc = ldc_d;
  g.M = M; g.N = N; g.K = K; g.alpha = alpha; g.beta = beta; g.ta = ta ? 1 : 0; g.tb = tb ? 1 : 0;
  int rc = (K > 0) ? launch_dgemm(ctx, g) : MLN_OK;
  if (rc == MLN_OK && K == 0) {
    mln_set_error(ctx, "mln_gemm: K = 0");
    rc = MLN_ERR_SHAPE;
  }
  if (rc == MLN_OK && !c_dev) {
    hipError_t e = hipMemcpy2DAsync(Cm, sizeof(double) * ldc, Cd, sizeof(double) * ldc_d, sizeof(double) * N, (size_t)M, hipMemcpyDeviceToHost, ctx->stream);
    if (e != hipSuccess) rc = mln_hip_fail(ctx, e, "mln_gemm download", __FILE__, __LINE__);
  }
  (void)hipStreamSynchronize(ctx->stream);
  return rc;
}

extern "C" int mln_eigh(mln_ctx* ctx, const double* A, int64_t m, double* w, double* V, int32_t* n_sweeps) {
  if (!ctx || (m > 0 && (!A || !w || !V))) return MLN_ERR_ARG;
  if (m < 0 || m > 32768) { mln_set_error(ctx, "eigh: m out of range"); return MLN_ERR_SHAPE; }
  if (n_sweeps) *n_sweeps = 0;
  if (m == 0) return MLN_OK;
  MLN_HIP(ctx, hipSetDevice(ctx->device));
  DevIn a;
  DevOut v;
  MLN_TRY(a.init(ctx, A, (size_t)m * m));
  MLN_TRY(v.init(ctx, V, (size_t)m * m));
  DevBuf<double> rows;
  MLN_TRY(rows.alloc(ctx, (size_t)m * m, "rows"));
  std::vector<double> wh((size_t)m);
  int sweeps = 0;
  int rc = dev_eigh(ctx, a.dev, m, m, wh.data(), rows, m, &sweeps);
  if (rc == MLN_OK) rc = launch_transpose(ctx, rows, m, v.dev, m, m);
  if (rc == MLN_OK) rc = v.commit();
  (void)hipStreamSynchronize(ctx->stream);
  rows.reset();
  if (rc != MLN_OK) return rc;
  if (n_sweeps) *n_sweeps = sweeps;
  if (is_device_ptr(w)) MLN_HIP(ctx, hipMemcpy(w, wh.data(), sizeof(double) * (size_t)m, hipMemcpyHostToDevice));
  else std::memcpy(w, wh.data(), sizeof(double) * (size_t)m);
  return MLN_OK;
}

extern "C" int mln_predict_mean(mln_ctx* ctx, const mln_kernel_desc* cov, const double* xnew, int64_t n_new,
                                int32_t d, const double* centers, int64_t m, const double* W, int64_t p,
                                double mu, double* out) {
  if (!ctx) return MLN_ERR_ARG;
  if (n_new < 0 || m < 1 || p < 1 || d < 1) { mln_set_error(ctx, "bad shape"); return MLN_ERR_SHAPE; }
  if (n_new == 0) return MLN_OK;
  if (!xnew || !centers || !W || !out) return MLN_ERR_ARG;
  MLN_HIP(ctx, hipSetDevice(ctx->device));
  DevCov dc;
  MLN_TRY(mln_lower_cov(ctx, cov, d, &dc));
  DevIn dx, dc_, dw;
  DevOut o;
  MLN_TRY(dx.init(ctx, xnew, (size_t)n_new * d));
  MLN_TRY(dc_.init(ctx, centers, (size_t)m * d));
  MLN_TRY(dw.init(ctx, W, (size_t)m * p));
  MLN_TRY(o.init(ctx, out, (size_t)n_new * p));
  if (p == 1) {
    MLN_TRY(launch_predict_mean1(ctx, dc, dx.dev, n_new, dc_.dev, m, d, dw.dev, mu, o.dev));
    return o.commit();
  }
  int64_t chunk = (int64_t)((1ull << 30) / (sizeof(double) * (size_t)m));
  chunk = (chunk / 128) * 128;
  if (chunk < 128) chunk = 128;
  if (chunk > n_new) chunk = n_new;
  DevBuf<double> Kc;
  DevBuf<double> mus;
  MLN_TRY(Kc.alloc(ctx, (size_t)chunk * m, "Kc"));
  int rc = MLN_OK;
  if (mu != 0.0) {
    std::vector<double> h((size_t)(chunk * p), mu);
    rc = (mus.alloc(ctx, h.size(), "mus") == MLN_OK &&
          hipMemcpy(mus, h.data(), sizeof(double) * h.size(), hipMemcpyHostToDevice) == hipSuccess) ? MLN_OK : MLN_ERR_HIP;
  }
  for (int64_t r0 = 0; r0 < n_new && rc == MLN_OK; r0 += chunk) {
    const int64_t rc_n = (n_new - r0 < chunk) ? (n_new - r0) : chunk;
    rc = launch_kernel_matrix(ctx, dc, dx.dev + r0 * d, rc_n, dc_.dev, m, d, Kc, m, 0.0);
    if (rc != MLN_OK) break;
    double* oc = o.dev + r0 * p;
    double beta = 0.0;
    if (mus) {
      rc = (hipMemcpyAsync(oc, mus, sizeof(double) * rc_n * p, hipMemcpyDeviceToDevice, ctx->stream) == hipSuccess) ? MLN_OK : MLN_ERR_HIP;
      beta = 1.0;
    }
    if (rc != MLN_OK) break;
    GemmArgs g{};
    g.A = Kc; g.lda = m; g.B = dw.dev; g.ldb = p; g.C = oc; g.ldc = p;
    g.M = rc_n; g.N = p; g.K = m; g.alpha = 1.0; g.beta = beta; g.ta = 0; g.tb = 0;
    rc = launch_dgemm(ctx, g);
  }
  if (rc == MLN_OK) rc = o.commit();
  (void)hipStreamSynchronize(ctx->stream);
  return rc;
}

extern "C" int mln_predict_covariance(mln_ctx* ctx, const mln_kernel_desc* cov, const double* xnew, int64_t n_new,
                                      int32_t d, const double* centers, int64_t m, const double* Lf, int32_t diag,
                                      double* out) {
  if (!ctx) return MLN_ERR_ARG;
  if (n_new < 0 || m < 1 || d < 1) { mln_set_error(ctx, "bad shape"); return MLN_ERR_SHAPE; }
  if (n_new == 0) return MLN_OK;
  if (!xnew || !centers || !Lf || !out) return MLN_ERR_ARG;
  if (!diag && n_new > 32768) { mln_set_error(ctx, "full covariance is limited to 32768 points"); return MLN_ERR_UNSUPPORTED; }
  MLN_HIP(ctx, hipSetDevice(ctx->device));
  DevCov dc;
  MLN_TRY(mln_lower_cov(ctx, cov, d, &dc));
  DevIn dx, dcen, dl;
  DevOut o;
  MLN_TRY(dx.init(ctx, xnew, (size_t)n_new * d));
  MLN_TRY(dcen.init(ctx, centers, (size_t)m * d));
  MLN_TRY(dl.init(ctx, Lf, (size_t)m * m));
  MLN_TRY(o.init(ctx, out, diag ? (size_t)n_new : (size_t)n_new * n_new));
  const int64_t ld = pad16(m);
  TriInv t;
  MLN_TRY(triinv_build(ctx, dl.dev, m, m, true, false, &t));
  int64_t chunk = diag ? (int64_t)((1ull << 30) / (sizeof(double) * (size_t)ld)) : n_new;
  if (chunk > n_new) chunk = n_new;
  if (chunk < 1) chunk = 1;
  DevBuf<double> A, kss;
  int rc = MLN_OK;
  if (rc == MLN_OK) rc = A.alloc(ctx, (size_t)chunk * ld, "A");
  if (rc == MLN_OK) rc = kss.alloc(ctx, (size_t)chunk, "kss");
  for (int64_t r0 = 0; r0 < n_new && rc == MLN_OK; r0 += chunk) {
    const int64_t rows = (n_new - r0 < chunk) ? (n_new - r0) : chunk;
    rc = launch_kernel_matrix(ctx, dc, dx.dev + r0 * d, rows, dcen.dev, m, d, A, ld, 0.0);
    if (rc == MLN_OK) rc = triinv_solve_right_T(ctx, t, A, rows, ld);
    if (rc != MLN_OK) break;
    if (diag) {
      rc = launch_cov_diag(ctx, dc, dx.dev + r0 * d, rows, d, kss);
      if (rc == MLN_OK) rc = launch_row_sumsq(ctx, A, ld, rows, m, kss, -1.0, o.dev + r0);
    } else {
      rc = launch_kernel_matrix(ctx, dc, dx.dev, n_new, dx.dev, n_new, d, o.dev, n_new, 0.0);
      GemmArgs g{};
      g.A = A; g.lda = ld; g.B = A; g.ldb = ld; g.C = o.dev; g.ldc = n_new;
      g.M = n_new; g.N = n_new; g.K = m; g.alpha = -1.0; g.beta = 1.0; g.ta = 0; g.tb = 1;
      if (rc == MLN_OK) rc = launch_dgemm(ctx, g);
    }
  }
  if (rc == MLN_OK) rc = o.commit();
  (void)hipStreamSynchronize(ctx->stream);
  return rc;
}

extern "C" int mln_predict_mean_covariance(mln_ctx* ctx, const mln_kernel_desc* cov, const double* xnew,
                                           int64_t n_new, int32_t d, const double* centers, int64_t m,
                                           const double* W, int64_t q, int32_t diag, double* out) {
  if (!ctx) return MLN_ERR_ARG;
  if (n_new < 0 || m < 1 || d < 1 || q < 1) { mln_set_error(ctx, "bad shape"); return MLN_ERR_SHAPE; }
  if (n_new == 0) return MLN_OK;
  if (!xnew || !centers || !W || !out) return MLN_ERR_ARG;
  if (!diag && n_new > 32768) { mln_set_error(ctx, "full covariance is limited to 32768 points"); return MLN_ERR_UNSUPPORTED; }
  MLN_HIP(ctx, hipSetDevice(ctx->device));
  DevCov dc;
  MLN_TRY(mln_lower_cov(ctx, cov, d, &dc));
  DevIn dx, dcen, dw;
  DevOut o;
  MLN_TRY(dx.init(ctx, xnew, (size_t)n_new * d));
  MLN_TRY(dcen.init(ctx, centers, (size_t)m * d));
  MLN_TRY(dw.init(ctx, W, (size_t)m * q));
  MLN_TRY(o.init(ctx, out, diag ? (size_t)n_new : (size_t)n_new * n_new));
  const int64_t ldq = pad16(q);
  int64_t chunk = diag ? (int64_t)((1ull << 30) / (sizeof(double) * (size_t)(m + ldq))) : n_new;
  if (chunk > n_new) chunk = n_new;
  if (chunk < 1) chunk = 1;
  DevBuf<double> Kc, T;
  int rc = MLN_OK;
  if (rc == MLN_OK) rc = Kc.alloc(ctx, (size_t)chunk * m, "Kc");
  if (rc == MLN_OK) rc = T.alloc(ctx, (size_t)chunk * ldq, "T");
  for (int64_t r0 = 0; r0 < n_new && rc == MLN_OK; r0 += chunk) {
    const int64_t rows = (n_new - r0 < chunk) ? (n_new - r0) : chunk;
    rc = launch_kernel_matrix(ctx, dc, dx.dev + r0 * d, rows, dcen.dev, m, d, Kc, m, 0.0);
    GemmArgs g{};
    g.A = Kc; g.lda = m; g.B = dw.dev; g.ldb = q; g.C = T; g.ldc = ldq;
    g.M = rows; g.N = q; g.K = m; g.alpha = 1.0; g.beta = 0.0; g.ta = 0; g.tb = 0;
    if (rc == MLN_OK) rc = launch_dgemm(ctx, g);
    if (rc != MLN_OK) break;
    if (diag) {
      rc = launch_row_sumsq(ctx, T, ldq, rows, q, nullptr, 1.0, o.dev + r0);
    } else {
      GemmArgs h{};
      h.A = T; h.lda = ldq; h.B = T; h.ldb = ldq; h.C = o.dev; h.ldc = n_new;
      h.M = n_new; h.N = n_new; h.K = q; h.alpha = 1.0; h.beta = 0.0; h.ta = 0; h.tb = 1;
      rc = launch_dgemm(ctx, h);
    }
  }
  if (rc == MLN_OK) rc = o.commit();
  (void)hipStreamSynchronize(ctx->stream);
  return rc;
}
```

mellon_amd/csrc/api_internal.h:

```cpp
#pragma once
#include <chrono>
#include <cmath>
#include <cstdio>
#include <cstdlib>
#include <algorithm>
#include <atomic>
#include <cstring>
#include <memory>
#include <mutex>
#include <string>
#include <thread>
#include <vector>

#include "linalg.h"
#include "mln_internal.h"
#include "objective.h"
#include "precond_rebuild.h"
#include "solver.h"

void fit_events_borrow(mln_ctx* ctx, std::vector<hipEvent_t>* evs);
void fit_events_return(mln_ctx* ctx, std::vector<hipEvent_t>* evs);

bool is_device_ptr(const void* p);
double now_s();

struct DevIn {
  mln_ctx* ctx;
  const double* dev = nullptr;
  DevBuf<double> owned;
  int init(mln_ctx* c, const double* p, size_t count) {
    ctx = c;
    if (count == 0 || !p) { dev = p; return MLN_OK; }
    if (is_device_ptr(p)) { dev = p; return MLN_OK; }
    MLN_TRY(owned.alloc(ctx, count, "device copy of an input"));
    MLN_HIP(ctx, hipMemcpyAsync(owned, p, count * sizeof(double), hipMemcpyHostToDevice, ctx->stream));
    dev = owned;
    return MLN_OK;
  }
  ~DevIn() {
    if (owned) (void)hipStreamSynchronize(ctx->stream);
  }
};

struct DevOut {
  mln_ctx* ctx;
  double* dev = nullptr;
  DevBuf<double> owned;
  double* host = nullptr;
  size_t count = 0;
  int init(mln_ctx* c, double* p, size_t n, bool copy_in = false) {
    ctx = c; count = n;
    if (n == 0) { dev = p; return MLN_OK; }
    if (is_device_ptr(p)) { dev = p; return MLN_OK; }
    host = p;
    MLN_TRY(owned.alloc(ctx, n, "device copy of an output"));
    if (copy_in) MLN_HIP(ctx, hipMemcpyAsync(owned, p, n * sizeof(double), hipMemcpyHostToDevice, ctx->stream));
    dev = owned;
    return MLN_OK;
  }
  int commit() {
    if (owned && count) {
      MLN_HIP(ctx, hipMemcpyAsync(host, owned, count * sizeof(double), hipMemcpyDeviceToHost, ctx->stream));
    }
    MLN_HIP(ctx, hipStreamSynchronize(ctx->stream));
    return MLN_OK;
  }
  ~DevOut() {
    if (owned) (void)hipStreamSynchronize(ctx->stream);
  }
};

struct Precond { DevBuf<double> C, Cinv, P, Q1, Q2; };

struct mln_fit {
  mln_ctx* ctx = nullptr;
  DevCov cov;
  int d = 0;
  int64_t n = 0, m = 0, ldl = 0, ldp = 0;
  bool full = false;
  DevBuf<double> L_own;
  double* L = nullptr;
  DevBuf<double> Lp;
  TriInv tri;
  DevBuf<double> V, Vdr;
  double mu = 0.0;
  int n_wg = 0;
  DevBuf<double> part_grad, part_hess, part_loss;
  DevBuf<double> d_z, d_out;
  PinnedBuf<double> h_z, h_out;
  hipEvent_t ev0 = nullptr, ev1 = nullptr;
  double times[MLN_N_STAGE_TIMES] = {0};
  Precond pc, pc_saved;
  DevBuf<double> d_u, d_gu, d_tmp;
  int n_wg_cap = 0;
  bool kspace = false;
  DevBuf<double> Kj;
  bool lp_pending = false, lp_failed = false, tri_pending = false;
  double jitter = 0.0;
  DevBuf<double> d_w;
  std::vector<double> z_cached;
  DevBuf<double> d_w_cached;
  DevBuf<double> d_zw, d_zr;
  DevBuf<double> eigU;
  DevBuf<float> L32;
  double emu_excluded = 0.0;
  bool cov_bounded01 = false;
  int l32_fixed = 0;
  int evals32 = 0;
  double times32 = 0.0;
  int64_t ld2 = 0;
  DevBuf<int> d_over;
  int64_t row0 = 0;
  SolverBuffers sv{};
  DevBuf<double> sv_block;
  PinnedBuf<SolverState> h_state;
  int sv_maxcor = 0;
  std::vector<hipEvent_t> evs;
  DevBuf<double> f_keep[2];
  int f_final = -1;
  int64_t precond_stride = 0;
  bool from_K = false, k_finished = false;
  int64_t k_rows_done = 0;
  int n_revert = 0, n_rebuild_skipped = 0, n_start_halvings = 0, rank_path = 0;
  double build_seconds = 0.0;
  double times_sub = 0.0, times_rebuild = 0.0, sub_pass_equiv = 0.0;
  int evals_sub = 0, n_rebuild = 0;
  DevBuf<double> dim_ell;
  int dim_k = 0;
  double mu_dim = 0.0, mu_dens = 0.0;
  DevBuf<double> dim_part, dim_z, dim_out;
  ~mln_fit();
};

int dev_allreduce(mln_ctx* ctx, double* dev, int64_t count);
int dev_bcast0(mln_ctx* ctx, double* dev, int64_t count);
int reject_distance_leaf(mln_ctx* ctx, const DevCov& dc);
int64_t pad16(int64_t m);
void fit_sample_rows(const mln_fit* f, int64_t s, int64_t* first, int64_t* rows);
int fit_alloc_workspace(mln_fit* f);
int fit_prepare_impl(mln_ctx* ctx, const mln_kernel_desc* cov, const double* x, int64_t n, int32_t d,
                            const double* xu, int64_t m, double jitter, const double* Lp_in, int32_t flags,
                            mln_fit* f);
ObjArgs obj_args(mln_fit* f);
void obj_account(mln_fit* f, bool f32 = false);
int fit_w_from_z(mln_fit* f, const double* z_dev, double* w_dev, const double* z_host = nullptr);
int fit_cache_pair_from_u(mln_fit* f, const double* u_dev);
int fit_enqueue_eval(mln_fit* f, const double* u_dev, double* gn_dev, bool use32, const int* gate,
                            hipEvent_t* ev, const std::vector<int64_t>* sub_strides = nullptr);
int fit_objective_u(mln_fit* f, const double* u, double* loss, double* grad_u, double* z_out,
                           bool use32 = false);
int fit_solver_alloc(mln_fit* f, int maxcor);
int gram_of(mln_ctx* ctx, const double* A, int64_t lda, int64_t rows, int64_t m, double alpha, double* G,
                   int64_t ldg, bool quantised = false);
int emulated_ranks(const mln_ctx* ctx);
int fit_ensure_kj(mln_fit* f);
int fit_ensure_lp(mln_fit* f, bool need_tri = true);
int fit_lp_finish(mln_fit* f, int rc_chol, double t0);
int fit_gram(mln_fit* f, double* G, int64_t ldg, int64_t row_stride, bool whiten = true);
int fit_gemvT(mln_fit* f, const double* t_dev, double* rhs_dev);
int fit_factor_precond(mln_fit* f);
int fit_build_precond(mln_fit* f, int64_t row_stride);
int fit_rebuild_precond(mln_fit* f, const double* f_dev, double rows_per_m, int* outcome, double cap = 1e300);
int fit_precond_revert(mln_fit* f);
int fit_small_gemv(mln_fit* f, const double* M, int trans, const double* w, double* y);
int launch_scale_rows_cols(mln_ctx* ctx, double* A, int64_t ld, int64_t rows, int64_t cols, const double* row,
                                  const double* col);
int sparse_solve_impl(mln_ctx* ctx, const mln_kernel_desc* cov, const double* x, int64_t n_local,
                             int32_t d, const double* xu, int64_t m, const double* y, int64_t p, double mu,
                             const double* sigmas, int32_t kind, double jitter, double* W, double* Lp_out,
                             double* Cs_out);
unsigned grid_1d(int64_t count);
```

mellon_amd/csrc/api_precond.hip:

```cpp
#include "api_internal.h"
#include "mln_options.h"

namespace {
__global__ void k_pack_lower(const double* __restrict__ G, int64_t m, int64_t ld, double* __restrict__ out) {
  const int64_t i = blockIdx.y;
  const int64_t j = (int64_t)blockIdx.x * blockDim.x + threadIdx.x;
  if (j <= i) out[i * (i + 1) / 2 + j] = G[i * ld + j];
}
__global__ void k_unpack_symmetric(const double* __restrict__ in, int64_t m, int64_t ld, double* __restrict__ G) {
  const int64_t i = blockIdx.y;
  const int64_t j = (int64_t)blockIdx.x * blockDim.x + threadIdx.x;
  if (j < m) G[i * ld + j] = (j <= i) ? in[i * (i + 1) / 2 + j] : in[j * (j + 1) / 2 + i];
}
}

int allreduce_symmetric_lower(mln_ctx* ctx, double* G, int64_t m, int64_t ldg) {
  const int64_t cnt = m * (m + 1) / 2;
  DevBuf<double> packed;
  MLN_TRY(packed.alloc(ctx, (size_t)cnt, "packed"));
  const dim3 grid((unsigned)((m + 255) / 256), (unsigned)m), block(256);
  hipLaunchKernelGGL(k_pack_lower, grid, block, 0, ctx->stream, G, m, ldg, packed);
  int rc = dev_allreduce(ctx, packed, cnt);
  if (rc == MLN_OK) {
    hipLaunchKernelGGL(k_unpack_symmetric, grid, block, 0, ctx->stream, packed, m, ldg, G);
    if (hipGetLastError() != hipSuccess) rc = MLN_ERR_HIP;
  }
  (void)hipStreamSynchronize(ctx->stream);
  return rc;
}

int gram_of(mln_ctx* ctx, const double* A, int64_t lda, int64_t rows, int64_t m, double alpha, double* G,
                   int64_t ldg, bool quantised) {
  int split = quantised ? gram_i8_splits(rows, m) : (int)(rows / 8192);
  if (split < 1) split = 1;
  if (split > 16 && !quantised) split = 16;
  const size_t stride = (size_t)m * ldg;
  DevBuf<double> parts;
  if (split > 1) MLN_TRY(parts.alloc(ctx, stride * split, "parts"));
  GemmArgs g{};
  g.A = A; g.lda = lda; g.B = A; g.ldb = lda;
  g.C = (split > 1) ? parts : G; g.ldc = ldg;
  g.M = m; g.N = m; g.K = rows; g.alpha = alpha; g.beta = 0.0; g.ta = 1; g.tb = 0; g.lower_only = 1;
  g.split_k = split; g.c_split_stride = (int64_t)stride;
  int rc = MLN_OK;
  if (split > 1) rc = (hipMemsetAsync(parts, 0, sizeof(double) * stride * split, ctx->stream) == hipSuccess) ? MLN_OK : MLN_ERR_HIP;
  else rc = (hipMemsetAsync(G, 0, sizeof(double) * stride, ctx->stream) == hipSuccess) ? MLN_OK : MLN_ERR_HIP;
  if (rc == MLN_OK && rows > 0)
    rc = quantised ? launch_gram_i8(ctx, A, lda, rows, m, alpha, g.C, ldg, (int64_t)stride, split) : launch_dgemm(ctx, g);
  if (rc == MLN_OK && split > 1) rc = launch_sum_partials(ctx, parts, split, (int64_t)stride, G, (int64_t)stride, 0.0);
  if (rc == MLN_OK && ctx->n_ranks > 1) rc = allreduce_symmetric_lower(ctx, G, m, ldg);
  else if (rc == MLN_OK) rc = launch_symmetrize_from_lower(ctx, G, m, ldg);
  (void)hipStreamSynchronize(ctx->stream);
  return rc;
}

extern "C" int mln_diag_gram_i8(mln_ctx* ctx, const double* A, int64_t rows, int64_t m, double* out, int32_t reps,
                                double* ms_out) {
  if (!ctx || !A || !out || rows < 1 || m < 1) return MLN_ERR_ARG;
  MLN_HIP(ctx, hipSetDevice(ctx->device));
  DevIn a;
  DevOut o;
  MLN_TRY(a.init(ctx, A, (size_t)rows * m));
  MLN_TRY(o.init(ctx, out, (size_t)m * m));
  const int split = gram_i8_splits(rows, m);
  const size_t stride = (size_t)m * m;
  DevBuf<double> parts, G;
  MLN_TRY(parts.alloc(ctx, stride * split, "parts"));
  MLN_TRY(G.alloc(ctx, stride, "G"));
  hipEvent_t e0, e1;
  MLN_HIP(ctx, hipEventCreate(&e0));
  MLN_HIP(ctx, hipEventCreate(&e1));
  int rc = MLN_OK;
  if (reps < 1) reps = 1;
  for (int r = 0; r <= reps && rc == MLN_OK; ++r) {
    if (r == 1) (void)hipEventRecord(e0, ctx->stream);
    rc = (hipMemsetAsync(parts, 0, sizeof(double) * stride * split, ctx->stream) == hipSuccess) ? MLN_OK : MLN_ERR_HIP;
    if (rc == MLN_OK) rc = launch_gram_i8(ctx, a.dev, m, rows, m, 1.0, parts, m, (int64_t)stride, split);
    if (rc == MLN_OK) rc = launch_sum_partials(ctx, parts, split, (int64_t)stride, G, (int64_t)stride, 0.0);
  }
  (void)hipEventRecord(e1, ctx->stream);
  (void)hipStreamSynchronize(ctx->stream);
  float ms = 0.f;
  (void)hipEventElapsedTime(&ms, e0, e1);
  if (ms_out) *ms_out = ms / reps;
  if (rc == MLN_OK) rc = launch_symmetrize_from_lower(ctx, G, m, m);
  if (rc == MLN_OK) rc = launch_copy_block(ctx, G, m, o.dev, m, m, m);
  if (rc == MLN_OK) rc = o.commit();
  (void)hipStreamSynchronize(ctx->stream);
  (void)hipEventDestroy(e0); (void)hipEventDestroy(e1);
  return rc;
}

int emulated_ranks(const mln_ctx* ctx) {
  if (ctx->n_ranks > 1) return 0;
  if (const char* ev = std::getenv("MELLON_AMD_EMULATE_RANKS")) { const int n = std::atoi(ev); return n > 1 ? n : 0; }
  return 0;
}

int fit_ensure_kj(mln_fit* f) {
  if (f->Kj) return MLN_OK;
  mln_ctx* ctx = f->ctx;
  if (!f->Lp) { mln_set_error(ctx, "this fit handle holds no Lp"); return MLN_ERR_ARG; }
  MLN_TRY(f->Kj.alloc_zeroed(ctx, (size_t)f->m * f->ldp, "Kj"));
  GemmArgs g{};
  g.A = f->Lp; g.lda = f->ldp; g.B = f->Lp; g.ldb = f->ldp; g.C = f->Kj; g.ldc = f->ldp;
  g.M = f->m; g.N = f->m; g.K = f->m; g.alpha = 1.0; g.beta = 0.0; g.ta = 0; g.tb = 1; g.lower_only = 1;
  MLN_TRY(launch_dgemm(ctx, g));
  return launch_symmetrize_from_lower(ctx, f->Kj, f->m, f->ldp);
}

int fit_gram(mln_fit* f, double* G, int64_t ldg, int64_t row_stride, bool whiten) {
  mln_ctx* ctx = f->ctx;
  if (row_stride < 1) row_stride = 1;
  const int64_t first = (row_stride - f->row0 % row_stride) % row_stride;
  const int64_t rows = (f->n > first) ? (f->n - first + row_stride - 1) / row_stride : 0;
  const double* Ls = f->L + first * f->ldl;
  if (!f->kspace) return gram_of(ctx, Ls, f->ldl * row_stride, rows, f->m, (double)row_stride, G, ldg);
  bool quant = f->cov_bounded01 && f->m >= 256 && row_stride > 1;
  if (const char* ev = mln_experiment("MELLON_AMD_GRAM_I8")) quant = quant && std::atoi(ev) != 0;
  int rc = gram_of(ctx, Ls, f->ldl * row_stride, rows, f->m, (double)row_stride, G, ldg, quant);
  if (rc != MLN_OK || !whiten) return rc;
  MLN_TRY(fit_ensure_lp(f));
  DevBuf<double> T;
  rc = T.alloc_zeroed(ctx, (size_t)f->m * ldg, "Gram temp");
  if (rc == MLN_OK) rc = triinv_solve_left(ctx, f->tri, G, f->m, ldg);
  if (rc == MLN_OK) rc = launch_transpose(ctx, G, ldg, T, ldg, f->m);
  if (rc == MLN_OK) rc = triinv_solve_left(ctx, f->tri, T, f->m, ldg);
  if (rc == MLN_OK) rc = (hipMemcpyAsync(G, T, sizeof(double) * (size_t)f->m * ldg, hipMemcpyDeviceToDevice,
                                         ctx->stream) == hipSuccess) ? MLN_OK : MLN_ERR_HIP;
  (void)hipStreamSynchronize(ctx->stream);
  return rc;
}

int fit_gemvT(mln_fit* f, const double* t_dev, double* rhs_dev) {
  mln_ctx* ctx = f->ctx;
  ObjArgs a = obj_args(f);
  a.weights = t_dev;
  a.part_loss = nullptr;
  MLN_TRY(launch_objective(ctx, a));
  MLN_TRY(launch_reduce_obj(ctx, a, f->d_out));
  MLN_TRY(dev_allreduce(ctx, f->d_out, 1 + f->m));
  if (f->kspace) { MLN_TRY(fit_ensure_lp(f)); MLN_TRY(triinv_solve_left(ctx, f->tri, f->d_out + 1, 1, 1)); }
  MLN_HIP(ctx, hipMemcpyAsync(rhs_dev, f->d_out + 1, sizeof(double) * f->m, hipMemcpyDeviceToDevice, ctx->stream));
  return MLN_OK;
}

int fit_factor_precond(mln_fit* f) {
  mln_ctx* ctx = f->ctx;
  const int64_t m = f->m, ldg = f->ldl;
  const size_t count = (size_t)m * ldg;
  int rc = f->kspace ? MLN_OK : launch_add_diag(ctx, f->pc.C, m, ldg, 1.0);
  if (rc == MLN_OK && f->kspace && f->lp_pending && !f->lp_failed && f->ldp == ldg) {
    const double t0 = now_s();
    int bad = 0;
    rc = dev_cholesky_lower2(ctx, f->pc.C, f->Lp, m, ldg, &bad);
    const int rc_lp = (rc == MLN_ERR_NOT_PD && !(bad & 2)) ? MLN_OK : rc;
    if (rc == MLN_OK || rc == MLN_ERR_NOT_PD) {
      const std::string msg = ctx->err;
      const int rl = fit_lp_finish(f, rc_lp, t0);
      if (rl != MLN_OK) return rl;
      if (rc != MLN_OK) mln_set_error(ctx, msg);
    }
  } else if (rc == MLN_OK) {
    rc = dev_cholesky_lower(ctx, f->pc.C, m, ldg);
  }
  TriInv t;
  if (rc == MLN_OK) rc = triinv_build(ctx, f->pc.C, m, ldg, true, false, &t);
  DevBuf<double> inv;
  if (rc == MLN_OK) rc = inv.alloc_zeroed(ctx, count, "factor inverse");
  if (rc == MLN_OK) rc = launch_add_diag(ctx, inv, m, ldg, 1.0);
  if (rc == MLN_OK) rc = triinv_solve_left(ctx, t, inv, m, ldg, true);
  if (rc == MLN_OK && f->kspace) {
    rc = f->pc.P.alloc_zeroed(ctx, count, "P");
    if (rc == MLN_OK) rc = launch_transpose(ctx, inv, ldg, f->pc.P, ldg, m);
  } else if (rc == MLN_OK) {
    const int64_t ld = ldg;
    rc = f->pc.Q1.alloc_zeroed(ctx, count, "stacked operator Q1");
    if (rc == MLN_OK) rc = f->pc.Q2.alloc_zeroed(ctx, count * 2, "stacked operator Q2");
    if (rc == MLN_OK) rc = launch_transpose(ctx, inv, ld, f->pc.Q1, ld, m);
    if (rc == MLN_OK) rc = launch_copy_block(ctx, inv, ld, f->pc.Q2, ld * 2, m, ld);
    if (rc == MLN_OK) rc = launch_copy_block(ctx, inv, ld, f->pc.Q2 + ld, ld * 2, m, ld);
  }
  (void)hipStreamSynchronize(ctx->stream);
  if (rc == MLN_OK) f->pc.Cinv = std::move(inv);
  return rc;
}

int fit_build_precond(mln_fit* f, int64_t row_stride) {
  if (f->pc.Cinv) return MLN_OK;
  mln_ctx* ctx = f->ctx;
  const int64_t m = f->m, ldg = f->ldl;
  double t0 = now_s();
  MLN_TRY(f->pc.C.alloc(ctx, (size_t)m * ldg, "C"));
  int rc = fit_gram(f, f->pc.C, ldg, row_stride, false);
  if (rc == MLN_OK && f->kspace) rc = fit_ensure_kj(f);
  if (rc == MLN_OK && f->kspace) rc = launch_axpby(ctx, m * ldg, 1.0, f->Kj, 1.0, f->pc.C);
  MLN_HIP(ctx, hipStreamSynchronize(ctx->stream));
  f->times[3] += now_s() - t0;
  double t1 = now_s();
  if (rc == MLN_OK) rc = fit_factor_precond(f);
  f->times[4] += now_s() - t1;
  if (rc == MLN_OK) { f->precond_stride = row_stride < 1 ? 1 : row_stride; f->build_seconds = now_s() - t0; }
  return rc;
}

int fit_precond_revert(mln_fit* f) {
  if (!f->pc_saved.C || !f->pc_saved.Cinv) return MLN_ERR_ARG;
  (void)hipStreamSynchronize(f->ctx->stream);
  f->pc = std::move(f->pc_saved);
  return MLN_OK;
}

int fit_rebuild_precond(mln_fit* f, const double* f_dev, double rows_per_m, int* outcome, double cap) {
  mln_ctx* ctx = f->ctx;
  const int64_t m = f->m, ldg = f->ldl;
  *outcome = 0;
  RebuildSelection sel;
  double target = rows_per_m * (double)m;
  if (const int n_emu = emulated_ranks(ctx)) target /= (double)n_emu;
  const bool tr_on = std::getenv("MELLON_AMD_TRACE") != nullptr;
  double tt[6] = {0, 0, 0, 0, 0, 0};
  auto lap = [&](int i, double& t0) { if (tr_on) { (void)hipStreamSynchronize(ctx->stream); const double t1 = now_s(); tt[i] += t1 - t0; t0 = t1; } };
  double tl = now_s();
  MLN_TRY(rebuild_select_rows(ctx, f_dev, f->V, f->n, f->row0, target, 0x6d656c6c6f6eull, &sel, cap));
  lap(0, tl);
  if (tr_on)
    fprintf(stderr, "[trace] rebuild: %lld of %lld local rows kept (target %.0f global), c = %.4g, 1/c = %.4g, w_max = %.4g, sum a = %.6g\n",
            (long long)sel.rows, (long long)f->n, target, sel.c, 1.0 / sel.c, sel.w_max, sel.sum_a);
  double range_cap = 1e7;
  if (const char* ev = mln_experiment("MELLON_AMD_REBUILD_RANGE")) range_cap = std::atof(ev);
  if (!(sel.w_max * sel.c <= range_cap) || !std::isfinite(sel.sum_a)) {
    (void)hipStreamSynchronize(ctx->stream);
    *outcome = 1;
    return MLN_OK;
  }
  DevBuf<double> R;
  const int64_t rr = sel.rows > 0 ? sel.rows : 1;
  int rc = R.alloc(ctx, (size_t)rr * f->ldl, "R");
  if (rc == MLN_OK) rc = launch_gather_scale_rows(ctx, f->L, f->ldl, sel.idx, sel.scale, sel.rows, R);
  Precond old = std::move(f->pc);
  if (rc == MLN_OK) rc = f->pc.C.alloc(ctx, (size_t)m * ldg, "C");
  lap(1, tl);
  if (rc == MLN_OK) {
    bool quant = f->kspace && f->cov_bounded01 && m >= 256;
    if (const char* ev = mln_experiment("MELLON_AMD_GRAM_I8")) quant = quant && std::atoi(ev) != 0;
    rc = gram_of(ctx, R, f->ldl, sel.rows, m, sel.w_max, f->pc.C, ldg, quant);
  }
  (void)hipStreamSynchronize(ctx->stream);
  R.reset();
  (void)hipStreamSynchronize(ctx->stream);
  sel.reset();
  lap(2, tl);
  if (rc == MLN_OK && f->kspace) rc = fit_ensure_kj(f);
  if (rc == MLN_OK && f->kspace) rc = launch_axpby(ctx, m * ldg, 1.0, f->Kj, 1.0, f->pc.C);
  lap(3, tl);
  if (rc == MLN_OK) rc = fit_factor_precond(f);
  lap(4, tl);
  if (tr_on) fprintf(stderr, "[trace] rebuild ms: select %.2f, gather %.2f, gram %.2f, + Kj %.2f, factor+inverses+stacks %.2f (rc %d)\n",
                     1e3 * tt[0], 1e3 * tt[1], 1e3 * tt[2], 1e3 * tt[3], 1e3 * tt[4], rc);
  if (rc != MLN_OK) {
    (void)hipStreamSynchronize(ctx->stream);
    f->pc = std::move(old);
    if (rc != MLN_ERR_NOT_PD) return rc;
    *outcome = 2;
    return MLN_OK;
  }
  if (f->pc_saved.C) (void)hipStreamSynchronize(ctx->stream);
  f->pc_saved = std::move(old);
  return MLN_OK;
}

int fit_small_gemv(mln_fit* f, const double* M, int trans, const double* w, double* y) {
  mln_ctx* ctx = f->ctx;
  ObjArgs a{};
  a.L = M; a.ldl = f->ldl; a.n = f->m; a.m = f->m; a.mu = 0.0;
  a.part_grad = f->part_grad; a.part_hess = nullptr; a.part_loss = nullptr;
  a.m_pad = f->ldl;
  int64_t steps = (f->m + 1) / 2;
  a.n_wg = (int)((steps < f->n_wg_cap) ? (steps > 0 ? steps : 1) : f->n_wg_cap);
  if (trans) {
    a.weights = w;
    MLN_TRY(launch_objective(ctx, a));
    MLN_TRY(launch_reduce_obj(ctx, a, f->d_tmp));
    MLN_HIP(ctx, hipMemcpyAsync(y, f->d_tmp + 1, sizeof(double) * f->m, hipMemcpyDeviceToDevice, ctx->stream));
  } else {
    a.z = w;
    a.f_out = y;
    MLN_TRY(launch_objective(ctx, a));
  }
  return MLN_OK;
}

extern "C" int mln_fit_set_row_offset(mln_fit* f, int64_t global_row0) {
  if (!f || global_row0 < 0) return MLN_ERR_ARG;
  f->row0 = global_row0;
  return MLN_OK;
}

extern "C" int mln_precond_build(mln_fit* f, int64_t row_stride) {
  if (!f) return MLN_ERR_ARG;
  MLN_HIP(f->ctx, hipSetDevice(f->ctx->device));
  if (row_stride < 1) row_stride = 1;
  if (f->pc.Cinv && f->precond_stride != row_stride) {
    (void)hipStreamSynchronize(f->ctx->stream);
    f->pc = Precond();
    f->precond_stride = 0;
  }
  return fit_build_precond(f, row_stride);
}

extern "C" int mln_ridge_init(mln_fit* f, const double* target, double* z0) {
  if (!f || !z0 || (f->n > 0 && !target)) return MLN_ERR_ARG;
  mln_ctx* ctx = f->ctx;
  MLN_HIP(ctx, hipSetDevice(ctx->device));
  MLN_TRY(fit_build_precond(f, 1));
  double t0 = now_s();
  DevIn dt;
  MLN_TRY(dt.init(ctx, target, (size_t)f->n));
  int64_t rs = (f->precond_stride >= 11 && f->m <= objective_max_m_one_pass()) ? f->precond_stride : 1;
  if (const char* ev = mln_experiment("MELLON_AMD_SUBSAMPLE")) { if (std::atoi(ev) == 0) rs = 1; }
  ObjArgs a = obj_args(f);
  a.weights = dt.dev;
  a.part_loss = nullptr;
  if (rs > 1) {
    int64_t first = 0, rows = 0;
    fit_sample_rows(f, rs, &first, &rows);
    a.n = rows; a.row_first = first; a.row_stride = rs; a.out_scale = (double)rs;
  }
  if (f->kspace) {
    a.L32 = f->L32;
    a.l32_fixed = f->l32_fixed;
    MLN_TRY(launch_objective(ctx, a));
    MLN_TRY(launch_reduce_obj(ctx, a, f->d_out));
    MLN_TRY(dev_allreduce(ctx, f->d_out, 1 + f->m));
    MLN_TRY(fit_small_gemv(f, f->pc.Cinv, 0, f->d_out + 1, f->d_gu));
    MLN_TRY(fit_small_gemv(f, f->pc.P, 0, f->d_gu, f->d_w));
    MLN_TRY(fit_ensure_lp(f, false));
    MLN_TRY(fit_small_gemv(f, f->Lp, 1, f->d_w, f->d_z));
  } else {
    MLN_TRY(launch_objective(ctx, a));
    MLN_TRY(launch_reduce_obj(ctx, a, f->d_out));
    MLN_TRY(dev_allreduce(ctx, f->d_out, 1 + f->m));
    MLN_TRY(fit_small_gemv(f, f->pc.Cinv, 0, f->d_out + 1, f->d_gu));
  }
  if (!f->kspace) MLN_TRY(fit_small_gemv(f, f->pc.Cinv, 1, f->d_gu, f->d_z));
  MLN_TRY(fit_cache_pair_from_u(f, f->d_gu));
  MLN_HIP(ctx, hipMemcpyAsync(z0, f->d_z, sizeof(double) * f->m, hipMemcpyDefault, ctx->stream));
  MLN_HIP(ctx, hipStreamSynchronize(ctx->stream));
  f->times[4] += now_s() - t0;
  return MLN_OK;
}

extern "C" int mln_precond_apply(mln_fit* f, int32_t mode, const double* in, double* out) {
  if (!f || !in || !out) return MLN_ERR_ARG;
  mln_ctx* ctx = f->ctx;
  MLN_HIP(ctx, hipSetDevice(ctx->device));
  MLN_TRY(fit_build_precond(f, 1));
  MLN_HIP(ctx, hipMemcpyAsync(f->d_u, in, sizeof(double) * f->m, hipMemcpyDefault, ctx->stream));
  if (f->kspace && mode >= 0 && mode <= 2) {
    MLN_TRY(fit_ensure_lp(f));
    if (mode == 0) {
      MLN_TRY(fit_w_from_z(f, f->d_u, f->d_w, is_device_ptr(in) ? nullptr : in));
      MLN_TRY(fit_small_gemv(f, f->pc.C, 1, f->d_w, f->d_gu));
    } else if (mode == 1) {
      MLN_TRY(fit_small_gemv(f, f->pc.P, 0, f->d_u, f->d_w));
      MLN_TRY(fit_small_gemv(f, f->Lp, 1, f->d_w, f->d_gu));
    } else {
      MLN_TRY(fit_small_gemv(f, f->Lp, 0, f->d_u, f->d_w));
      MLN_TRY(fit_small_gemv(f, f->pc.Cinv, 0, f->d_w, f->d_gu));
    }
  }
  else if (mode == 0) MLN_TRY(fit_small_gemv(f, f->pc.C, 1, f->d_u, f->d_gu));
  else if (mode == 1) MLN_TRY(fit_small_gemv(f, f->pc.Cinv, 1, f->d_u, f->d_gu));
  else if (mode == 2) MLN_TRY(fit_small_gemv(f, f->pc.Cinv, 0, f->d_u, f->d_gu));
  else { mln_set_error(ctx, "mln_precond_apply: unknown mode"); return MLN_ERR_ARG; }
  MLN_HIP(ctx, hipMemcpyAsync(out, f->d_gu, sizeof(double) * f->m, hipMemcpyDefault, ctx->stream));
  MLN_HIP(ctx, hipStreamSynchronize(ctx->stream));
  return MLN_OK;
}
```

mellon_amd/csrc/gram_i8.hip:

```cpp
#include "mln_internal.h"

#include <algorithm>
#include <cmath>
#include <vector>

namespace {

typedef int v4i_t __attribute__((ext_vector_type(4)));
typedef int v16i_t __attribute__((ext_vector_type(16)));

constexpr int GQ_SCALE = 8355711;
constexpr int GT = 128;
constexpr int GBK = 64;
constexpr int GROW = GBK + 16;
constexpr int GSTAGE = 2 * 3 * GT * GROW;

__device__ __forceinline__ void lds_barrier() { asm volatile("s_waitcnt lgkmcnt(0)\n\ts_barrier" ::: "memory"); }

__global__ __launch_bounds__(256) void k_gram_digits(const double* __restrict__ K, int64_t ldk, int64_t rows, int64_t m,
                                                     int8_t* __restrict__ planes, int64_t Mp, int64_t Kp) {
  __shared__ uint32_t tile[3][64][17];
  const int t = threadIdx.x, li = t & 63, kq = t >> 6;
  const int64_t k0 = (int64_t)blockIdx.x * 64, i0 = (int64_t)blockIdx.y * 64;
  const int64_t gi = i0 + li;
#pragma unroll
  for (int r = 0; r < 4; ++r) {
    const int g = kq * 4 + r;
    uint32_t w0 = 0, w1 = 0, w2 = 0;
#pragma unroll
    for (int e = 0; e < 4; ++e) {
      const int64_t k = k0 + g * 4 + e;
      double v = 0.0;
      if (k < rows && gi < m) v = K[k * ldk + gi];
      v = fmin(fmax(v, 0.0), 1.0);
      const int q = (int)rint(v * (double)GQ_SCALE);
      const int d0 = ((q + 128) & 255) - 128;
      const int q1 = (q - d0) >> 8;
      const int d1 = ((q1 + 128) & 255) - 128;
      const int d2 = (q1 - d1) >> 8;
      w0 |= (uint32_t)(d0 & 255) << (8 * e);
      w1 |= (uint32_t)(d1 & 255) << (8 * e);
      w2 |= (uint32_t)(d2 & 255) << (8 * e);
    }
    tile[0][li][g] = w0; tile[1][li][g] = w1; tile[2][li][g] = w2;
  }
  __syncthreads();
  const int oi = t >> 2, seg = t & 3;
#pragma unroll
  for (int a = 0; a < 3; ++a) {
    v4i_t o;
    o.x = (int)tile[a][oi][seg * 4 + 0]; o.y = (int)tile[a][oi][seg * 4 + 1];
    o.z = (int)tile[a][oi][seg * 4 + 2]; o.w = (int)tile[a][oi][seg * 4 + 3];
    const int64_t gi2 = i0 + oi;
    *reinterpret_cast<v4i_t*>(planes + (int64_t)a * Mp * Kp + (((gi2 >> 7) * (Kp >> 6) + (k0 >> 6)) * 128 + (gi2 & 127)) * 64 +
                              seg * 16) = o;
  }
}

struct GramTile { int ti, tj; };

template <int PASS, int NW>
__device__ __forceinline__ void gram_sweep(unsigned char* lds, const int8_t* gA, const int8_t* gB, int64_t plane_sz, int64_t half,
                                           int n_steps, int ldst0, int fa, int fb, double (&res)[2][8 / NW][16]) {
  constexpr int NP = PASS == 0 ? 3 : 2;
  constexpr int NA = PASS == 0 ? 3 : 2;
  constexpr int NBJ = 8 / NW;
  constexpr int NRH = 512 / (64 * NW);
  v4i_t stage[2][NRH * NP];
  auto g_load = [&](int st) {
#pragma unroll
    for (int o = 0; o < 2; ++o)
#pragma unroll
      for (int j = 0; j < NRH * NP; ++j) {
        const int8_t* src = (o == 0 ? gA : gB) + (j / NRH) * plane_sz + (j % NRH) * half + (int64_t)st * (GT * GBK);
        stage[o][j] = *reinterpret_cast<const v4i_t*>(src);
      }
  };
  auto l_store = [&](int buf) {
#pragma unroll
    for (int o = 0; o < 2; ++o)
#pragma unroll
      for (int j = 0; j < NRH * NP; ++j)
        *reinterpret_cast<v4i_t*>(lds + buf * GSTAGE + ldst0 + ((o * 3 + (j / NRH)) * GT + 64 * (j % NRH)) * GROW) = stage[o][j];
  };
  v16i_t acc[NA][2][NBJ];
#pragma unroll
  for (int w = 0; w < NA; ++w)
#pragma unroll
    for (int bi = 0; bi < 2; ++bi)
#pragma unroll
      for (int bj = 0; bj < NBJ; ++bj) acc[w][bi][bj] = v16i_t{};

  struct Ops { v4i_t A[NP][2], B[NP][NBJ]; };
  auto read_ops = [&](Ops& o, int buf, int ks) {
    const unsigned char* base = lds + buf * GSTAGE;
#pragma unroll
    for (int a = 0; a < NP; ++a) {
#pragma unroll
      for (int b = 0; b < 2; ++b) o.A[a][b] = *reinterpret_cast<const v4i_t*>(base + fa + (a * GT + b * 32) * GROW + ks * 32);
#pragma unroll
      for (int b = 0; b < NBJ; ++b) o.B[a][b] = *reinterpret_cast<const v4i_t*>(base + fb + (a * GT + b * 32) * GROW + ks * 32);
    }
  };
  auto mfma1 = [&](const Ops& o, int bi, int bj, int k) {
    if constexpr (PASS == 0) {
      if (k == 0) acc[0][bi][bj] = __builtin_amdgcn_mfma_i32_32x32x32_i8(o.A[2][bi], o.B[2][bj], acc[0][bi][bj], 0, 0, 0);
      if (k == 1) acc[1][bi][bj] = __builtin_amdgcn_mfma_i32_32x32x32_i8(o.A[1][bi], o.B[2][bj], acc[1][bi][bj], 0, 0, 0);
      if (k == 2) acc[2][bi][bj] = __builtin_amdgcn_mfma_i32_32x32x32_i8(o.A[0][bi], o.B[2][bj], acc[2][bi][bj], 0, 0, 0);
      if (k == 3) acc[1][bi][bj] = __builtin_amdgcn_mfma_i32_32x32x32_i8(o.A[2][bi], o.B[1][bj], acc[1][bi][bj], 0, 0, 0);
      if (k == 4) acc[2][bi][bj] = __builtin_amdgcn_mfma_i32_32x32x32_i8(o.A[1][bi], o.B[1][bj], acc[2][bi][bj], 0, 0, 0);
      if (k == 5) acc[2][bi][bj] = __builtin_amdgcn_mfma_i32_32x32x32_i8(o.A[2][bi], o.B[0][bj], acc[2][bi][bj], 0, 0, 0);
    } else {
      if (k == 0) acc[0][bi][bj] = __builtin_amdgcn_mfma_i32_32x32x32_i8(o.A[0][bi], o.B[1][bj], acc[0][bi][bj], 0, 0, 0);
      if (k == 1) acc[1][bi][bj] = __builtin_amdgcn_mfma_i32_32x32x32_i8(o.A[0][bi], o.B[0][bj], acc[1][bi][bj], 0, 0, 0);
      if (k == 2) acc[0][bi][bj] = __builtin_amdgcn_mfma_i32_32x32x32_i8(o.A[1][bi], o.B[0][bj], acc[0][bi][bj], 0, 0, 0);
    }
  };
  constexpr int NK = PASS == 0 ? 6 : 3;
  auto mfmas2 = [&](const Ops& o, int k0, int k1) {
#pragma unroll
    for (int k = k0; k < k1; ++k)
#pragma unroll
      for (int bj = 0; bj < NBJ; ++bj) { mfma1(o, 0, bj, k); mfma1(o, 1, bj, k); }
  };
  g_load(0); l_store(0);
  if (n_steps > 1) g_load(1);
  lds_barrier();
  Ops o0, o1;
  read_ops(o0, 0, 0);
  if (n_steps > 1) l_store(1);
  if (n_steps > 2) g_load(2);
  for (int st = 0; st < n_steps; ++st) {
    const int buf = st & 1;
    read_ops(o1, buf, 1);
    mfmas2(o0, 0, NK);
    __builtin_amdgcn_sched_barrier(0);
    lds_barrier();
    __builtin_amdgcn_sched_barrier(0);
    read_ops(o0, buf ^ 1, 0);
    mfmas2(o1, 0, NK / 2);
    l_store(buf);
    g_load(st + 3 < n_steps ? st + 3 : n_steps - 1);
    mfmas2(o1, NK / 2, NK);
  }
#pragma unroll
  for (int bi = 0; bi < 2; ++bi)
#pragma unroll
    for (int bj = 0; bj < NBJ; ++bj)
#pragma unroll
      for (int r = 0; r < 16; ++r) {
        if constexpr (PASS == 0)
          res[bi][bj][r] = ((double)acc[2][bi][bj][r] * 65536.0 + (double)acc[1][bi][bj][r] * 16777216.0) +
                           (double)acc[0][bi][bj][r] * 4294967296.0;
        else
          res[bi][bj][r] += (double)acc[1][bi][bj][r] + (double)acc[0][bi][bj][r] * 256.0;
      }
}

template <int NW>
__global__ __launch_bounds__(64 * NW, 1) void k_gram_i8(const int8_t* __restrict__ planes, int64_t Mp, int64_t Kp, int64_t kchunk,
                                                        const GramTile* __restrict__ tiles, int n_tiles, int n_wg, double scale,
                                                        double* __restrict__ parts, int64_t ldg, int64_t part_stride, int64_t m) {
  extern __shared__ __attribute__((aligned(16))) unsigned char lds[];
  const int id = blockIdx.x;
  const int per = (n_wg + 7) / 8;
  const int logical = (id & 7) * per + (id >> 3);
  if (logical >= n_wg) return;
  const int split = logical / n_tiles;
  const GramTile tl = tiles[logical - split * n_tiles];
  constexpr int NBJ = 8 / NW, WJ = 64 / (32 * NBJ) * 1;
  const int t = threadIdx.x, lane = t & 63, w = t >> 6;
  const int wi = (NW == 4) ? (w >> 1) : (w >> 2), wj = (NW == 4) ? (w & 1) : (w & 3);
  const int64_t kbeg = (int64_t)split * kchunk;
  const int n_steps = (int)(kchunk / GBK);
  const int64_t plane_sz = Mp * Kp;
  const int seg = t & 3, q = t >> 2, r0 = (q & ~7) | ((q & 1) << 2) | ((q >> 1) & 3);
  const int8_t* gA = planes + (((int64_t)tl.ti * (Kp >> 6) + (kbeg >> 6)) * GT + r0) * GBK + seg * 16;
  const int8_t* gB = planes + (((int64_t)tl.tj * (Kp >> 6) + (kbeg >> 6)) * GT + r0) * GBK + seg * 16;
  const int64_t half = 64 * GBK;
  const int ldst0 = r0 * GROW + seg * 16;
  const int fa = ((wi * 64 + (lane & 31)) * GROW) + (lane >> 5) * 16;
  const int fb = (3 * GT * GROW) + ((wj * 32 * NBJ + (lane & 31)) * GROW) + (lane >> 5) * 16;
  (void)WJ;

  double res[2][NBJ][16];
  gram_sweep<0, NW>(lds, gA, gB, plane_sz, half, n_steps, ldst0, fa, fb, res);
  gram_sweep<1, NW>(lds, gA, gB, plane_sz, half, n_steps, ldst0, fa, fb, res);

  double* out = parts + (int64_t)split * part_stride;
#pragma unroll
  for (int bi = 0; bi < 2; ++bi)
#pragma unroll
    for (int bj = 0; bj < NBJ; ++bj) {
      const int64_t gj = (int64_t)tl.tj * GT + wj * 32 * NBJ + bj * 32 + (lane & 31);
#pragma unroll
      for (int r = 0; r < 16; ++r) {
        const int64_t gi = (int64_t)tl.ti * GT + wi * 64 + bi * 32 + (r & 3) + 8 * (r >> 2) + 4 * (lane >> 5);
        if (gi < m && gj < m) out[gi * ldg + gj] = scale * res[bi][bj][r];
      }
    }
}

}

int gram_i8_splits(int64_t rows, int64_t m) {
  const int64_t T = (m + GT - 1) / GT, tiles = T * (T + 1) / 2;
  int smin = (int)((rows + 32767) / 32768);
  if (smin < 1) smin = 1;
  int best = smin;
  double best_eff = -1.0;
  for (int s = smin; s <= smin + 7; ++s) {
    if ((rows + s - 1) / s < 2048 && s > smin) break;
    const double wg = (double)tiles * s;
    const double eff = wg / (std::ceil(wg / 256.0) * 256.0);
    if (eff > best_eff + 0.02) { best_eff = eff; best = s; }
  }
  return best;
}

int launch_gram_i8(mln_ctx* ctx, const double* K, int64_t ldk, int64_t rows, int64_t m, double alpha, double* parts,
                   int64_t ldg, int64_t part_stride, int n_splits) {
  if (rows <= 0 || m <= 0) return MLN_OK;
  const int64_t T = (m + GT - 1) / GT, Mp = T * GT;
  int64_t kchunk = (rows + n_splits - 1) / n_splits;
  kchunk = (kchunk + GBK - 1) / GBK * GBK;
  if (kchunk > 32768) { mln_set_error(ctx, "gram_i8: k-chunk exceeds the exact int32 range"); return MLN_ERR_ARG; }
  const int64_t Kp = kchunk * n_splits;
  DevBuf<int8_t> planes;
  DevBuf<GramTile> d_tiles;
  MLN_TRY(planes.alloc(ctx, (size_t)3 * Mp * Kp, "Gram digit planes"));
  std::vector<GramTile> order;
  order.reserve((size_t)(T * (T + 1) / 2));
  for (int64_t s0 = 0; s0 < T; s0 += 8)
    for (int64_t j = 0; j < std::min(T, s0 + 8); ++j)
      for (int64_t i = std::max(s0, j); i < std::min(T, s0 + 8); ++i) order.push_back(GramTile{(int)i, (int)j});
  const int n_tiles = (int)order.size();
  MLN_TRY(d_tiles.alloc(ctx, order.size(), "Gram tile list"));
  int rc = MLN_OK;
  hipError_t e = hipMemcpyAsync(d_tiles, order.data(), sizeof(GramTile) * order.size(), hipMemcpyHostToDevice, ctx->stream);
  if (e == hipSuccess) e = hipStreamSynchronize(ctx->stream);
  if (e != hipSuccess) rc = mln_hip_fail(ctx, e, "upload Gram tile list", __FILE__, __LINE__);
  if (rc == MLN_OK) {
    hipLaunchKernelGGL(k_gram_digits, dim3((unsigned)(Kp / 64), (unsigned)(Mp / 64)), dim3(256), 0, ctx->stream, K, ldk, rows, m,
                       planes, Mp, Kp);
    static bool attr_set = false;
    const int lds_bytes = 2 * GSTAGE;
    if (!attr_set) {
      e = hipFuncSetAttribute(reinterpret_cast<const void*>(k_gram_i8<8>), hipFuncAttributeMaxDynamicSharedMemorySize, lds_bytes);
      if (e != hipSuccess) rc = mln_hip_fail(ctx, e, "gram_i8 LDS size", __FILE__, __LINE__);
      attr_set = true;
    }
    if (rc == MLN_OK) {
      const int n_wg = n_tiles * n_splits;
      const int grid = (n_wg + 7) / 8 * 8;
      const double scale = alpha / ((double)GQ_SCALE * (double)GQ_SCALE);
      hipLaunchKernelGGL(k_gram_i8<8>, dim3((unsigned)grid), dim3(512), lds_bytes, ctx->stream, planes, Mp, Kp, kchunk, d_tiles,
                         n_tiles, n_wg, scale, parts, ldg, part_stride, m);
      e = hipGetLastError();
      if (e != hipSuccess) rc = mln_hip_fail(ctx, e, "k_gram_i8", __FILE__, __LINE__);
    }
  }
  (void)hipStreamSynchronize(ctx->stream);
  return rc;
}
```

mellon_amd/csrc/linalg.hip:

```cpp
#include <cstdlib>
#include <map>
#include <mutex>
#include <vector>

#include "mln_internal.h"
#include "linalg.h"
#include "mln_options.h"

namespace {

constexpr int PB = 64;
constexpr int TB = 128;

__global__ __launch_bounds__(256) void k_trtri64(const double* __restrict__ Lf, int64_t m, int64_t ld,
                                                 double* __restrict__ W, int64_t ldw) {
  __shared__ double T[PB][PB + 1];
  __shared__ double X[PB][PB + 1];
  const int tid = threadIdx.x;
  const int64_t j0 = (int64_t)blockIdx.x * PB;
  const int nb = (int)((m - j0 < PB) ? (m - j0) : PB);
  for (int e = tid; e < PB * PB; e += 256) {
    int i = e / PB, j = e % PB;
    T[i][j] = (i < nb && j <= i) ? Lf[(j0 + i) * ld + j0 + j] : ((i == j) ? 1.0 : 0.0);
  }
  __syncthreads();
  if (tid < PB) {
    const int j = tid;
    for (int i = 0; i < PB; ++i) {
      double s = (i == j) ? 1.0 : 0.0;
      if (i < j) { X[i][j] = 0.0; continue; }
      for (int k = j; k < i; ++k) s = fma(-T[i][k], X[k][j], s);
      X[i][j] = s / T[i][i];
    }
  }
  __syncthreads();
  for (int e = tid; e < PB * PB; e += 256) {
    int i = e / PB, j = e % PB;
    if (i < nb && j < nb) W[(j0 + i) * ldw + j0 + j] = X[i][j];
  }
}

__global__ __launch_bounds__(256) void k_trtri_merge128(const double* __restrict__ Lf, int64_t m, int64_t ld,
                                                        double* W, int64_t ldw) {
  __shared__ double Ta[PB][PB + 1];
  __shared__ double Xa[PB][PB + 1];
  __shared__ double Xb[PB][PB + 1];
  const int tid = threadIdx.x;
  const int64_t j0 = (int64_t)blockIdx.x * TB;
  const int64_t r0 = j0 + PB;
  if (r0 >= m) return;
  const int nb2 = (int)((m - r0 < PB) ? (m - r0) : PB);
  for (int e = tid; e < PB * PB; e += 256) {
    int i = e / PB, j = e % PB;
    Ta[i][j] = (i < nb2) ? Lf[(r0 + i) * ld + j0 + j] : 0.0;
    Xa[i][j] = W[(j0 + i) * ldw + j0 + j];
    Xb[i][j] = (i < nb2 && j < nb2) ? W[(r0 + i) * ldw + r0 + j] : 0.0;
  }
  __syncthreads();
  const int ti = tid >> 2, tc = (tid & 3) * 16;
  double tmp[16];
#pragma unroll
  for (int q = 0; q < 16; ++q) tmp[q] = 0.0;
  for (int k = 0; k < PB; ++k) {
    const double a = Ta[ti][k];
#pragma unroll
    for (int q = 0; q < 16; ++q) tmp[q] = fma(a, Xa[k][tc + q], tmp[q]);
  }
  __syncthreads();
#pragma unroll
  for (int q = 0; q < 16; ++q) Ta[ti][tc + q] = tmp[q];
  __syncthreads();
  double out[16];
#pragma unroll
  for (int q = 0; q < 16; ++q) out[q] = 0.0;
  for (int k = 0; k < PB; ++k) {
    const double a = Xb[ti][k];
#pragma unroll
    for (int q = 0; q < 16; ++q) out[q] = fma(a, Ta[k][tc + q], out[q]);
  }
  if (ti < nb2) {
#pragma unroll
    for (int q = 0; q < 16; ++q) W[(r0 + ti) * ldw + j0 + tc + q] = -out[q];
  }
}

__global__ void k_add_diag(double* A, int64_t m, int64_t lda, double v) {
  int64_t i = (int64_t)blockIdx.x * blockDim.x + threadIdx.x;
  if (i < m) A[i * lda + i] += v;
}

__global__ void k_zero_upper(double* A, int64_t m, int64_t lda) {
  int64_t j = (int64_t)blockIdx.x * blockDim.x + threadIdx.x;
  int64_t i = blockIdx.y;
  if (j < m && j > i) A[i * lda + j] = 0.0;
}

__global__ void k_sym_from_lower(double* A, int64_t m, int64_t lda) {
  int64_t j = (int64_t)blockIdx.x * blockDim.x + threadIdx.x;
  int64_t i = blockIdx.y;
  if (j < m && j > i) A[i * lda + j] = A[j * lda + i];
}

__global__ void k_axpby(int64_t n, double a, const double* __restrict__ x, double b, double* __restrict__ y) {
  for (int64_t i = (int64_t)blockIdx.x * blockDim.x + threadIdx.x; i < n; i += (int64_t)gridDim.x * blockDim.x)
    y[i] = a * x[i] + ((b != 0.0) ? b * y[i] : 0.0);
}

__global__ void k_copy_block(const double* __restrict__ src, int64_t lds, double* __restrict__ dst, int64_t ldd,
                             int64_t rows, int64_t cols) {
  int64_t j = (int64_t)blockIdx.x * blockDim.x + threadIdx.x;
  int64_t i = blockIdx.y;
  if (i < rows && j < cols) dst[i * ldd + j] = src[i * lds + j];
}

__global__ void k_transpose(const double* __restrict__ src, int64_t lds, double* __restrict__ dst, int64_t ldd,
                            int64_t m) {
  __shared__ double tile[32][33];
  const int64_t bx = (int64_t)blockIdx.x * 32, by = (int64_t)blockIdx.y * 32;
  for (int r = threadIdx.y; r < 32; r += 8) {
    int64_t i = by + r, j = bx + threadIdx.x;
    tile[r][threadIdx.x] = (i < m && j < m) ? src[i * lds + j] : 0.0;
  }
  __syncthreads();
  for (int r = threadIdx.y; r < 32; r += 8) {
    int64_t i = bx + r, j = by + threadIdx.x;
    if (i < m && j < m) dst[i * ldd + j] = tile[threadIdx.x][r];
  }
}

}

int launch_transpose(mln_ctx* ctx, const double* src, int64_t lds, double* dst, int64_t ldd, int64_t m) {
  if (m <= 0) return MLN_OK;
  const unsigned t = (unsigned)((m + 31) / 32);
  hipLaunchKernelGGL(k_transpose, dim3(t, t), dim3(32, 8), 0, ctx->stream, src, lds, dst, ldd, m);
  MLN_HIP(ctx, hipGetLastError());
  return MLN_OK;
}

int launch_add_diag(mln_ctx* ctx, double* A, int64_t m, int64_t lda, double v) {
  if (m <= 0) return MLN_OK;
  hipLaunchKernelGGL(k_add_diag, dim3((unsigned)((m + 255) / 256)), dim3(256), 0, ctx->stream, A, m, lda, v);
  MLN_HIP(ctx, hipGetLastError());
  return MLN_OK;
}

int launch_symmetrize_from_lower(mln_ctx* ctx, double* A, int64_t m, int64_t lda) {
  if (m <= 0) return MLN_OK;
  hipLaunchKernelGGL(k_sym_from_lower, dim3((unsigned)((m + 255) / 256), (unsigned)m), dim3(256), 0, ctx->stream, A, m, lda);
  MLN_HIP(ctx, hipGetLastError());
  return MLN_OK;
}

int launch_axpby(mln_ctx* ctx, int64_t n, double a, const double* x, double b, double* y) {
  if (n <= 0) return MLN_OK;
  int64_t nb = (n + 255) / 256;
  if (nb > 8192) nb = 8192;
  hipLaunchKernelGGL(k_axpby, dim3((unsigned)nb), dim3(256), 0, ctx->stream, n, a, x, b, y);
  MLN_HIP(ctx, hipGetLastError());
  return MLN_OK;
}

int launch_copy_block(mln_ctx* ctx, const double* src, int64_t lds, double* dst, int64_t ldd, int64_t rows,
                      int64_t cols) {
  if (rows <= 0 || cols <= 0) return MLN_OK;
  if (rows > 65535) {
    for (int64_t r = 0; r < rows; r += 65535) {
      int64_t nr = (rows - r < 65535) ? rows - r : 65535;
      MLN_TRY(launch_copy_block(ctx, src + r * lds, lds, dst + r * ldd, ldd, nr, cols));
    }
    return MLN_OK;
  }
  hipLaunchKernelGGL(k_copy_block, dim3((unsigned)((cols + 255) / 256), (unsigned)rows), dim3(256), 0, ctx->stream,
                     src, lds, dst, ldd, rows, cols);
  MLN_HIP(ctx, hipGetLastError());
  return MLN_OK;
}

namespace {
__global__ void k_copy_below_blocks(const double* __restrict__ src, double* __restrict__ dst, int64_t m, int64_t ld) {
  const int64_t j = (int64_t)blockIdx.x * blockDim.x + threadIdx.x;
  const int64_t i = blockIdx.y;
  if (j < m && (j >> 7) < (i >> 7)) dst[i * ld + j] = src[i * ld + j];
}

}

static int cholesky_lower_batched(mln_ctx* ctx, double* A, int64_t m, int64_t lda, int nbatch, int64_t a_bs, int* bad) {
  if (bad) *bad = 0;
  if (m <= 0) return MLN_OK;
  constexpr int CB = 128;
  DevBuf<double> Dinv, Ls;
  const size_t mat = (size_t)m * (size_t)lda;
  MLN_TRY(Dinv.alloc_zeroed(ctx, CB * CB * nbatch, "Dinv"));
  MLN_HIP(ctx, hipMemsetAsync(ctx->d_info, 0, sizeof(int) * 2, ctx->stream));
  if (m > CB) MLN_TRY(Ls.alloc(ctx, mat * nbatch, "Ls"));
  int rc = MLN_OK;
  auto batched = [&](GemmArgs& g, int64_t bsa, int64_t bsb, int64_t bsc) { if (nbatch > 1) { g.batch = nbatch; g.bsa = bsa; g.bsb = bsb; g.bsc = bsc; } };
  auto panel = [&](int64_t j, int nb, int64_t rem) -> int {
    GemmArgs g{};
    g.A = A + (j + nb) * lda + j; g.lda = lda; g.B = Dinv; g.ldb = CB; g.C = Ls + (j + nb) * lda + j; g.ldc = lda;
    g.M = rem; g.N = nb; g.K = nb; g.alpha = 1.0; g.beta = 0.0; g.ta = 0; g.tb = 1;
    batched(g, a_bs, (int64_t)CB * CB, (int64_t)mat);
    return launch_dgemm(ctx, g);
  };
  for (int64_t j0 = 0; j0 < m && rc == MLN_OK; j0 += 2 * CB) {
    const int nb1 = (int)((m - j0 < CB) ? (m - j0) : CB);
    rc = launch_potrf128(ctx, A + j0 * lda + j0, lda, nb1, Dinv, ctx->d_info, j0, nbatch, a_bs);
    const int64_t rem1 = m - j0 - nb1;
    if (rc != MLN_OK || rem1 <= 0) break;
    rc = panel(j0, nb1, rem1);
    if (rc != MLN_OK) break;
    const int64_t j1 = j0 + nb1;
    const int nb2 = (int)((rem1 < CB) ? rem1 : CB);
    const double* P1 = Ls + j1 * lda + j0;
    {
      GemmArgs u{};
      u.A = P1; u.lda = lda; u.B = P1; u.ldb = lda; u.C = A + j1 * lda + j1; u.ldc = lda;
      u.M = rem1; u.N = nb2; u.K = nb1; u.alpha = -1.0; u.beta = 1.0; u.ta = 0; u.tb = 1;
      batched(u, (int64_t)mat, (int64_t)mat, a_bs);
      rc = launch_dgemm(ctx, u);
      if (rc != MLN_OK) break;
    }
    rc = launch_potrf128(ctx, A + j1 * lda + j1, lda, nb2, Dinv, ctx->d_info, j1, nbatch, a_bs);
    const int64_t rem2 = rem1 - nb2;
    if (rc != MLN_OK || rem2 <= 0) break;
    rc = panel(j1, nb2, rem2);
    if (rc != MLN_OK) break;
    const int64_t j2 = j1 + nb2;
    const double* Pw = Ls + j2 * lda + j0;
    GemmArgs t{};
    t.A = Pw; t.lda = lda; t.B = Pw; t.ldb = lda; t.C = A + j2 * lda + j2; t.ldc = lda;
    t.M = rem2; t.N = rem2; t.K = nb1 + nb2; t.alpha = -1.0; t.beta = 1.0; t.ta = 0; t.tb = 1; t.lower_only = 1;
    batched(t, (int64_t)mat, (int64_t)mat, a_bs);
    rc = launch_dgemm(ctx, t);
  }
  int info[2] = {0, 0};
  if (rc == MLN_OK) {
    for (int b = 0; b < nbatch; ++b) {
      if (Ls) hipLaunchKernelGGL(k_copy_below_blocks, dim3((unsigned)((m + 255) / 256), (unsigned)m), dim3(256), 0, ctx->stream, Ls + (size_t)b * mat, A + (int64_t)b * a_bs, m, lda);
      hipLaunchKernelGGL(k_zero_upper, dim3((unsigned)((m + 255) / 256), (unsigned)m), dim3(256), 0, ctx->stream, A + (int64_t)b * a_bs, m, lda);
    }
    hipError_t e = hipMemcpyAsync(info, ctx->d_info, sizeof(int) * 2, hipMemcpyDeviceToHost, ctx->stream);
    if (e == hipSuccess) e = hipStreamSynchronize(ctx->stream);
    if (e != hipSuccess) rc = mln_hip_fail(ctx, e, "cholesky sync", __FILE__, __LINE__);
  } else {
    (void)hipStreamSynchronize(ctx->stream);
  }
  if (rc != MLN_OK) return rc;
  for (int b = nbatch - 1; b >= 0; --b)
    if (info[b] != 0) {
      if (bad) *bad |= 1 << b;
      mln_set_error(ctx, "Cholesky failed: non-positive or NaN pivot at index " + std::to_string(info[b] - 1));
      rc = MLN_ERR_NOT_PD;
    }
  return rc;
}

int dev_cholesky_lower(mln_ctx* ctx, double* A, int64_t m, int64_t lda) { return cholesky_lower_batched(ctx, A, m, lda, 1, 0, nullptr); }

int dev_cholesky_lower2(mln_ctx* ctx, double* A, double* A2, int64_t m, int64_t lda, int* bad) {
  return cholesky_lower_batched(ctx, A, m, lda, 2, (int64_t)(A2 - A), bad);
}

int triinv_build(mln_ctx* ctx, const double* Lf, int64_t m, int64_t ld, bool need_w, bool need_w2, TriInv* out) {
  (void)need_w; (void)need_w2;
  out->m = m;
  out->Lf = Lf;
  out->ldf = ld;
  out->ld = ((m + 15) / 16) * 16;
  const size_t bytes = sizeof(double) * (size_t)m * (size_t)out->ld;
  MLN_TRY(out->W.alloc(ctx, (size_t)m * (size_t)out->ld, "W"));
  if (const int rc2 = out->W2.alloc(ctx, (size_t)m * (size_t)out->ld, "W2")) { out->reset(); return rc2; }
  double* D = out->W;
  MLN_HIP(ctx, hipMemsetAsync(D, 0, bytes, ctx->stream));
  const int64_t nb64 = (m + PB - 1) / PB, nb128 = (m + TB - 1) / TB;
  hipLaunchKernelGGL(k_trtri64, dim3((unsigned)nb64), dim3(256), 0, ctx->stream, Lf, m, ld, D, out->ld);
  hipLaunchKernelGGL(k_trtri_merge128, dim3((unsigned)nb128), dim3(256), 0, ctx->stream, Lf, m, ld, D, out->ld);
  MLN_HIP(ctx, hipGetLastError());
  MLN_HIP(ctx, hipMemcpyAsync(out->W2, D, bytes, hipMemcpyDeviceToDevice, ctx->stream));
  int rc = MLN_OK;
  if (m > TB) {
    GemmArgs g{};
    g.A = Lf; g.lda = ld; g.B = D; g.ldb = out->ld; g.C = out->W2; g.ldc = out->ld;
    g.M = m; g.N = m; g.K = m; g.alpha = -1.0; g.beta = 0.0; g.ta = 0; g.tb = 0; g.lower_only = 2; g.kmode = 2;
    rc = launch_dgemm(ctx, g);
    if (rc == MLN_OK) {
      GemmArgs h{};
      h.A = out->W2; h.lda = out->ld; h.B = Lf; h.ldb = ld; h.C = out->W; h.ldc = out->ld;
      h.M = m; h.N = m; h.K = m; h.alpha = -1.0; h.beta = 0.0; h.ta = 0; h.tb = 0; h.lower_only = 2; h.kmode = 1;
      rc = launch_dgemm(ctx, h);
    }
  }
  if (rc != MLN_OK) { (void)hipStreamSynchronize(ctx->stream); out->reset(); mln_set_error(ctx, "triinv_build failed"); }
  return rc;
}

int triinv_solve_right_T(mln_ctx* ctx, const TriInv& t, double* X, int64_t n, int64_t ldx) {
  if (n < 32768 && t.W && t.W2 && t.m > TB) {
    for (int64_t j0 = 0; j0 < t.m; j0 += TB) {
      const int64_t nb = (t.m - j0 < TB) ? (t.m - j0) : TB;
      const int64_t rem = t.m - j0 - nb;
      if (rem <= 0) break;
      GemmArgs u{};
      u.A = X + j0; u.lda = ldx; u.B = t.W2 + (j0 + nb) * t.ld + j0; u.ldb = t.ld; u.C = X + j0 + nb; u.ldc = ldx;
      u.M = n; u.N = rem; u.K = nb; u.alpha = 1.0; u.beta = 1.0; u.ta = 0; u.tb = 1;
      MLN_TRY(launch_dgemm(ctx, u));
    }
    GemmArgs g{};
    g.A = X; g.lda = ldx; g.B = t.W; g.ldb = t.ld; g.C = X; g.ldc = ldx;
    g.M = n; g.N = t.m; g.K = t.m; g.alpha = 1.0; g.beta = 0.0; g.ta = 0; g.tb = 1; g.kmode = 2;
    return launch_dgemm(ctx, g);
  }
  for (int64_t j0 = 0; j0 < t.m; j0 += TB) {
    const int64_t nb = (t.m - j0 < TB) ? (t.m - j0) : TB;
    GemmArgs g{};
    g.A = X; g.lda = ldx; g.B = t.W + j0 * t.ld; g.ldb = t.ld; g.C = X + j0; g.ldc = ldx;
    g.M = n; g.N = nb; g.K = j0 + nb; g.alpha = 1.0; g.beta = 0.0; g.ta = 0; g.tb = 1;
    MLN_TRY(launch_dgemm(ctx, g));
  }
  return MLN_OK;
}

int triinv_solve_left(mln_ctx* ctx, const TriInv& t, double* B, int64_t p, int64_t ldb, bool tri_b) {
  const bool right_looking = (p >= 256) && t.W && t.W2;
  tri_b = tri_b && right_looking && p == t.m;
  if (!right_looking) {
    for (int64_t j0 = 0; j0 < t.m; j0 += TB) {
      const int64_t nb = (t.m - j0 < TB) ? (t.m - j0) : TB;
      GemmArgs g{};
      g.A = t.W + j0 * t.ld; g.lda = t.ld; g.B = B; g.ldb = ldb; g.C = B + j0 * ldb; g.ldc = ldb;
      g.M = nb; g.N = p; g.K = j0 + nb; g.alpha = 1.0; g.beta = 0.0; g.ta = 0; g.tb = 0;
      MLN_TRY(launch_dgemm(ctx, g));
    }
    return MLN_OK;
  }
  for (int64_t j0 = 0; j0 < t.m; j0 += TB) {
    const int64_t nb = (t.m - j0 < TB) ? (t.m - j0) : TB;
    const int64_t rem = t.m - j0 - nb;
    if (rem <= 0) break;
    const int64_t ncol = tri_b ? (j0 + nb) : p;
    GemmArgs u{};
    u.A = t.W2 + (j0 + nb) * t.ld + j0; u.lda = t.ld; u.B = B + j0 * ldb; u.ldb = ldb;
    u.C = B + (j0 + nb) * ldb; u.ldc = ldb;
    u.M = rem; u.N = ncol; u.K = nb; u.alpha = 1.0; u.beta = 1.0; u.ta = 0; u.tb = 0;
    MLN_TRY(launch_dgemm(ctx, u));
  }
  GemmArgs g{};
  g.A = t.W; g.lda = t.ld; g.B = B; g.ldb = ldb; g.C = B; g.ldc = ldb;
  g.M = t.m; g.N = p; g.K = t.m; g.alpha = 1.0; g.beta = 0.0; g.ta = 0; g.tb = 0; g.kmode = 1;
  g.lower_only = tri_b ? 1 : 0;
  return launch_dgemm(ctx, g);
}

int triinv_solve_left_T(mln_ctx* ctx, const TriInv& t, double* B, int64_t p, int64_t ldb, bool tri_b) {
  const bool right_looking = (p >= 256) && t.W && t.W2;
  tri_b = tri_b && right_looking && p == t.m;
  const int64_t nblk = (t.m + TB - 1) / TB;
  if (!right_looking) {
    for (int64_t jb = nblk - 1; jb >= 0; --jb) {
      const int64_t j0 = jb * TB;
      const int64_t nb = (t.m - j0 < TB) ? (t.m - j0) : TB;
      GemmArgs g{};
      g.A = t.W2 + j0 * t.ld + j0; g.lda = t.ld; g.B = B + j0 * ldb; g.ldb = ldb;
      g.C = B + j0 * ldb; g.ldc = ldb;
      g.M = nb; g.N = p; g.K = t.m - j0; g.alpha = 1.0; g.beta = 0.0; g.ta = 1; g.tb = 0;
      MLN_TRY(launch_dgemm(ctx, g));
    }
    return MLN_OK;
  }
  for (int64_t jb = nblk - 1; jb >= 1; --jb) {
    const int64_t j0 = jb * TB;
    const int64_t nb = (t.m - j0 < TB) ? (t.m - j0) : TB;
    const int64_t c0 = tri_b ? j0 : 0;
    GemmArgs u{};
    u.A = t.W + j0 * t.ld; u.lda = t.ld; u.B = B + j0 * ldb + c0; u.ldb = ldb; u.C = B + c0; u.ldc = ldb;
    u.M = j0; u.N = p - c0; u.K = nb; u.alpha = 1.0; u.beta = 1.0; u.ta = 1; u.tb = 0;
    MLN_TRY(launch_dgemm(ctx, u));
  }
  GemmArgs g{};
  g.A = t.W; g.lda = t.ld; g.B = B; g.ldb = ldb; g.C = B; g.ldc = ldb;
  g.M = t.m; g.N = p; g.K = t.m; g.alpha = 1.0; g.beta = 0.0; g.ta = 1; g.tb = 0; g.kmode = 1;
  g.lower_only = tri_b ? 3 : 0;
  return launch_dgemm(ctx, g);
}
```

mellon_amd/csrc/mln_internal.h:

```cpp
#pragma once
#include "mln_core.h"

int comm_allreduce(mln_ctx* ctx, double* dev, int64_t count);
int comm_bcast0(mln_ctx* ctx, double* dev, int64_t count);
int comm_allgather(mln_ctx* ctx, const double* send, double* recv, int64_t count);
void comm_release(mln_ctx* ctx);

int launch_kernel_matrix(mln_ctx* ctx, const DevCov& cov, const double* x, int64_t n, const double* y,
                         int64_t m, int d, double* out, int64_t ldo, double add_diag, float* out32 = nullptr,
                         int q32 = 0);
__device__ __forceinline__ float mln_surrogate_bits(double v, int q32) {
  const unsigned fx = (unsigned)fmin(fma(v, 4294967296.0, 0.5), 4294967295.0);
  return q32 ? __uint_as_float(fx) : (float)v;
}
int launch_predict_mean1(mln_ctx* ctx, const DevCov& cov, const double* x, int64_t n, const double* y,
                         int64_t m, int d, const double* w, double mu, double* out);

int launch_cov_diag(mln_ctx* ctx, const DevCov& cov, const double* x, int64_t n, int d, double* out);
int launch_row_sumsq(mln_ctx* ctx, const double* T, int64_t ld, int64_t rows, int64_t cols, const double* base,
                     double sign, double* out);
int launch_nn_distances(mln_ctx* ctx, const double* x, int64_t n, const double* y, int64_t m, int d,
                        int64_t self_offset, double* out);

struct GemmArgs {
  const double* A; int64_t lda;
  const double* B; int64_t ldb;
  double* C; int64_t ldc;
  int64_t M, N, K;
  double alpha, beta;
  int ta, tb;
  int lower_only;
  int split_k; int64_t c_split_stride;
  int kmode;
  int batch; int64_t bsa, bsb, bsc;
};
int launch_dgemm(mln_ctx* ctx, const GemmArgs& g);
int launch_sum_partials(mln_ctx* ctx, const double* parts, int n_parts, int64_t stride, double* out,
                        int64_t count, double beta);

int dev_cholesky_lower(mln_ctx* ctx, double* A, int64_t m, int64_t lda);
int dev_cholesky_lower2(mln_ctx* ctx, double* A, double* A2, int64_t m, int64_t lda, int* bad);
int launch_add_diag(mln_ctx* ctx, double* A, int64_t m, int64_t lda, double v);
int launch_symmetrize_from_lower(mln_ctx* ctx, double* A, int64_t m, int64_t lda);
int dev_sym_rank_above(mln_ctx* ctx, double* A, int64_t m, int64_t ld, double tol2, int64_t* rank, double* lambda_max);
int dev_sym_rank_above_ldl(mln_ctx* ctx, double* A, int64_t m, int64_t ld, double tol2, int64_t* rank, double* lambda_max, bool* ok);
int gram_i8_splits(int64_t rows, int64_t m);
int launch_gram_i8(mln_ctx* ctx, const double* K, int64_t ldk, int64_t rows, int64_t m, double alpha, double* parts,
                   int64_t ldg, int64_t part_stride, int n_splits);
int launch_axpby(mln_ctx* ctx, int64_t n, double a, const double* x, double b, double* y);

int launch_kernel_grad(mln_ctx* ctx, const DevCov& cov, const double* x, int64_t n, const double* y, int64_t m,
                       int d, int exact_denominator, double* out);
int launch_predict_gradient_gemm(mln_ctx* ctx, const DevCov& cov, const double* x, int64_t n, const double* c,
                                 int64_t m, int d, const double* w, double* out);
int launch_predict_gradient_gemm_multi(mln_ctx* ctx, const DevCov& cov, const double* x, int64_t n, const double* c,
                                       int64_t m, int d, const double* w, double* out);
int launch_predict_hessian(mln_ctx* ctx, const DevCov& cov, const double* x, int64_t n, const double* c, int64_t m,
                           int d, const double* w, double* out);
int launch_predict_gradient(mln_ctx* ctx, const DevCov& cov, const double* x, int64_t n, const double* c, int64_t m,
                            int d, const double* w, double* out);

int dev_eigh(mln_ctx* ctx, const double* A, int64_t m, int64_t lda, double* w_host, double* Vrows, int64_t ldv,
             int* n_sweeps_out);
```

mellon_amd/csrc/potrf.hip:

```cpp
#include "mln_internal.h"
#include "linalg.h"

#ifdef MLN_POTRF_TIMING
__device__ long long g_potrf_ts[64];
#define TS(i) do { if (threadIdx.x == 0) { g_potrf_ts[i] = wall_clock64(); g_potrf_ts[32 + i] = clock64(); } } while (0)
#else
#define TS(i) do { } while (0)
#endif
namespace {

typedef double v4d __attribute__((ext_vector_type(4)));

constexpr int NB = 128, LDT = 130, MB = 16, NMB = NB / MB, LDX = 18;
constexpr bool NEWTON2 = true;

__device__ __forceinline__ double bcast_lane(double v, int lane) {
  const int lo = __builtin_amdgcn_readlane(__double2loint(v), lane);
  const int hi = __builtin_amdgcn_readlane(__double2hiint(v), lane);
  return __hiloint2double(hi, lo);
}

template <int K> __device__ __forceinline__ double row_bcast_c(double v) {
  return __builtin_amdgcn_update_dpp(0.0, v, 0x150 + K, 0xf, 0xf, false);
}
__device__ __forceinline__ double row_bcast(double v, int k) {
  switch (k) {
    case 0: return row_bcast_c<0>(v);   case 1: return row_bcast_c<1>(v);   case 2: return row_bcast_c<2>(v);
    case 3: return row_bcast_c<3>(v);   case 4: return row_bcast_c<4>(v);   case 5: return row_bcast_c<5>(v);
    case 6: return row_bcast_c<6>(v);   case 7: return row_bcast_c<7>(v);   case 8: return row_bcast_c<8>(v);
    case 9: return row_bcast_c<9>(v);   case 10: return row_bcast_c<10>(v); case 11: return row_bcast_c<11>(v);
    case 12: return row_bcast_c<12>(v); case 13: return row_bcast_c<13>(v); case 14: return row_bcast_c<14>(v);
    default: return row_bcast_c<15>(v);
  }
}
#ifdef MLN_POTRF_LDS_BCAST
constexpr bool DPP_BCAST = false;
#else
constexpr bool DPP_BCAST = true;
#endif

__device__ __forceinline__ double frag(const double* M, int ldm, int r0, int c0, int s, int lane) {
  return M[(r0 + (lane & 15)) * ldm + c0 + 4 * s + (lane >> 4)];
}

template <bool SIGNED>
__global__ __launch_bounds__(256) void k_potrf128(double* A, int64_t lda, int nb, double* __restrict__ Dinv,
                                                  int* info, int64_t j0, double* __restrict__ DinvS, int* n_neg,
                                                  unsigned long long* min_piv, int64_t a_bs) {
  extern __shared__ double smem[];
  A += (int64_t)blockIdx.x * a_bs; Dinv += (int64_t)blockIdx.x * NB * NB; info += blockIdx.x;
  double* T = smem;
  double* Xd = smem + NB * LDT;
  double* Sg = Xd + NMB * MB * LDX;
  __shared__ int bad_s;
  const int tid = threadIdx.x, lane = tid & 63, wave = tid >> 6;
  TS(0);
  if (tid == 0) bad_s = 0;
  {
    typedef double d2_t __attribute__((ext_vector_type(2)));
    const bool pairs_ok = ((lda & 1) == 0) && ((reinterpret_cast<uintptr_t>(A) & 15) == 0);
#pragma unroll
    for (int b = 0; b < 2; ++b) {
      d2_t v[16];
#pragma unroll
      for (int q = 0; q < 16; ++q) {
        const int e = tid + 256 * (16 * b + q), i = e >> 6, j = (e & 63) * 2;
        const int ic = (i < nb) ? i : (nb - 1), jc = (j + 1 < nb) ? j : 0;
        if (pairs_ok) v[q] = *reinterpret_cast<const d2_t*>(A + (int64_t)ic * lda + jc);
        else { v[q].x = A[(int64_t)ic * lda + jc]; v[q].y = A[(int64_t)ic * lda + jc + 1]; }
      }
#pragma unroll
      for (int q = 0; q < 16; ++q) {
        const int e = tid + 256 * (16 * b + q), i = e >> 6, j = (e & 63) * 2;
        const bool in0 = i < nb && j <= i && j + 1 < nb, in1 = i < nb && j + 1 <= i && j + 1 < nb;
        double x0 = in0 ? v[q].x : ((i == j) ? 1.0 : 0.0);
        double x1 = in1 ? v[q].y : ((i == j + 1) ? 1.0 : 0.0);
        if (i < nb && j <= i && j + 1 >= nb) x0 = A[(int64_t)i * lda + j];
        T[i * LDT + j] = x0;
        T[i * LDT + j + 1] = x1;
      }
    }
  }
  __syncthreads();
  TS(1);

  auto diag_tile = [&](int p) {
    if (DPP_BCAST) {
      const int c0 = p * MB;
      const int li = lane & 15;
      double* Tt = T + c0 * LDT + c0;
      double a[MB], x[MB];
#pragma unroll
      for (int j = 0; j < MB; ++j) a[j] = (j <= li) ? Tt[li * LDT + j] : 0.0;
      int badk = -1;
      double minabs = INFINITY;
      double dk = row_bcast(a[0], 0);
      double sg = 1.0;
      if (SIGNED) { sg = (dk < 0.0) ? -1.0 : 1.0; dk = fabs(dk); }
      double inv = __builtin_amdgcn_rsq(dk);
      inv = inv * fma(-0.5 * dk, inv * inv, 1.5);
      if (NEWTON2) inv = inv * fma(-0.5 * dk, inv * inv, 1.5);
#pragma unroll
      for (int k = 0; k < MB; ++k) {
        badk = (!(dk > 0.0) && badk < 0) ? k : badk;
        if (SIGNED) {
          minabs = fmin(minabs, (c0 + k < nb) ? dk : INFINITY);
          if (lane == 0) Sg[c0 + k] = sg;
        }
        const double sq = dk * inv;
        const double lsg = SIGNED ? inv * sg : inv;
        const double lik = (li == k) ? sq : ((li > k) ? a[k] * lsg : 0.0);
        a[k] = lik;
        const double nlik = SIGNED ? -lik * sg : -lik;
        double dk1 = 1.0, inv1 = 1.0, sg1 = 1.0;
        if (k + 1 < MB) {
          a[k + 1] = fma(nlik, row_bcast(lik, k + 1), a[k + 1]);
          dk1 = row_bcast(a[k + 1], k + 1);
          if (SIGNED) { sg1 = (dk1 < 0.0) ? -1.0 : 1.0; dk1 = fabs(dk1); }
          inv1 = __builtin_amdgcn_rsq(dk1);
          inv1 = inv1 * fma(-0.5 * dk1, inv1 * inv1, 1.5);
          if (NEWTON2) inv1 = inv1 * fma(-0.5 * dk1, inv1 * inv1, 1.5);
        }
#pragma unroll
        for (int j = k + 2; j < MB; ++j) a[j] = fma(nlik, row_bcast(lik, j), a[j]);
        double s0 = (k == li) ? 1.0 : 0.0, s1 = 0.0, s2 = 0.0, s3 = 0.0;
#pragma unroll
        for (int j = 0; j < k; ++j) {
          const double lkj = row_bcast(a[j], k);
          if ((j & 3) == 0) s0 = fma(-lkj, x[j], s0);
          else if ((j & 3) == 1) s1 = fma(-lkj, x[j], s1);
          else if ((j & 3) == 2) s2 = fma(-lkj, x[j], s2);
          else s3 = fma(-lkj, x[j], s3);
        }
        x[k] = ((s0 + s1) + (s2 + s3)) * inv;
        dk = dk1; inv = inv1; sg = sg1;
      }
      if (badk >= 0 && lane == 0) { atomicCAS(info, 0, (int)(j0 + c0 + badk + 1)); bad_s = 1; }
      if (SIGNED && lane == 0 && c0 < nb) {
        int real_negs = 0;
        for (int k = 0; k < MB; ++k) real_negs += (c0 + k < nb && Sg[c0 + k] < 0.0) ? 1 : 0;
        if (real_negs) atomicAdd(n_neg, real_negs);
        atomicMin(min_piv, (unsigned long long)__double_as_longlong(minabs));
      }
      if (lane < MB) {
#pragma unroll
        for (int j = 0; j < MB; ++j) {
          Tt[li * LDT + j] = (j <= li) ? a[j] : 0.0;
          Xd[(p * MB + j) * LDX + li] = x[j];
        }
      }
      return;
    }
    const int c0 = p * MB;
    const int li = lane & 15;
    double* Tt = T + c0 * LDT + c0;
    double a[MB];
#pragma unroll
    for (int j = 0; j < MB; ++j) a[j] = (j <= li) ? Tt[li * LDT + j] : 0.0;
    double x[MB];
    int badk = -1;
    double dk = bcast_lane(a[0], 0);
    double sg = 1.0;
    double minabs = INFINITY;
    if (SIGNED) { sg = (dk < 0.0) ? -1.0 : 1.0; dk = fabs(dk); }
    double inv = __builtin_amdgcn_rsq(dk);
    inv = inv * fma(-0.5 * dk, inv * inv, 1.5);
    if (NEWTON2) inv = inv * fma(-0.5 * dk, inv * inv, 1.5);
#pragma unroll
    for (int k = 0; k < MB; ++k) {
      badk = (!(dk > 0.0) && badk < 0) ? k : badk;
      if (SIGNED) {
        minabs = fmin(minabs, (c0 + k < nb) ? dk : INFINITY);
        if (lane == 0) Sg[c0 + k] = sg;
      }
      const double sq = dk * inv;
      const double lsg = SIGNED ? inv * sg : inv;
      const double lik = (li == k) ? sq : ((li > k) ? a[k] * lsg : 0.0);
      a[k] = lik;
      if (lane < MB && li >= k) Tt[li * LDT + k] = lik;
      double lcol[MB];
#pragma unroll
      for (int j = k + 1; j < MB; ++j) lcol[j] = Tt[j * LDT + k];
      double s0 = (k == li) ? 1.0 : 0.0, s1 = 0.0, s2 = 0.0, s3 = 0.0;
#pragma unroll
      for (int j = 0; j < k; ++j) {
        const double lkj = Tt[k * LDT + j];
        if ((j & 3) == 0) s0 = fma(-lkj, x[j], s0);
        else if ((j & 3) == 1) s1 = fma(-lkj, x[j], s1);
        else if ((j & 3) == 2) s2 = fma(-lkj, x[j], s2);
        else s3 = fma(-lkj, x[j], s3);
      }
      x[k] = ((s0 + s1) + (s2 + s3)) * inv;
      const double nlik = SIGNED ? -lik * sg : -lik;
      double dk1 = 1.0, inv1 = 1.0, sg1 = 1.0;
      if (k + 1 < MB) {
        dk1 = bcast_lane(fma(nlik, lik, a[k + 1]), k + 1);
        if (SIGNED) { sg1 = (dk1 < 0.0) ? -1.0 : 1.0; dk1 = fabs(dk1); }
        inv1 = __builtin_amdgcn_rsq(dk1);
        inv1 = inv1 * fma(-0.5 * dk1, inv1 * inv1, 1.5);
        if (NEWTON2) inv1 = inv1 * fma(-0.5 * dk1, inv1 * inv1, 1.5);
      }
#pragma unroll
      for (int j = k + 1; j < MB; ++j) a[j] = fma(nlik, lcol[j], a[j]);
      dk = dk1; inv = inv1; sg = sg1;
    }
    if (badk >= 0 && lane == 0) { atomicCAS(info, 0, (int)(j0 + c0 + badk + 1)); bad_s = 1; }
    if (SIGNED && lane == 0 && c0 < nb) {
      int real_negs = 0;
      for (int k = 0; k < MB; ++k) real_negs += (c0 + k < nb && Sg[c0 + k] < 0.0) ? 1 : 0;
      if (real_negs) atomicAdd(n_neg, real_negs);
      atomicMin(min_piv, (unsigned long long)__double_as_longlong(minabs));
    }
    if (lane < MB) {
#pragma unroll
      for (int j = 0; j < MB; ++j) {
        if (j > li) Tt[li * LDT + j] = 0.0;
        Xd[(p * MB + j) * LDX + li] = x[j];
      }
    }
  };
  auto trailing_tile = [&](int p, int t) {
    const int c0 = p * MB;
    int ii = 0, rem = t;
    while (rem > ii) { rem -= ii + 1; ++ii; }
    const int jj = rem;
    const int r0 = (p + 1 + ii) * MB, q0 = (p + 1 + jj) * MB;
    v4d acc;
#pragma unroll
    for (int r = 0; r < 4; ++r) acc[r] = T[(r0 + (lane >> 4) + 4 * r) * LDT + q0 + (lane & 15)];
#pragma unroll
    for (int s = 0; s < 4; ++s)
    {
      const double sk = SIGNED ? -Sg[c0 + 4 * s + (lane >> 4)] : -1.0;
      acc = __builtin_amdgcn_mfma_f64_16x16x4f64(sk * frag(T, LDT, r0, c0, s, lane), frag(T, LDT, q0, c0, s, lane), acc, 0, 0, 0);
    }
#pragma unroll
    for (int r = 0; r < 4; ++r) T[(r0 + (lane >> 4) + 4 * r) * LDT + q0 + (lane & 15)] = acc[r];
  };

  if (wave == 0) diag_tile(0);
  __syncthreads();
  TS(2);
  if (bad_s) return;
  for (int p = 0; p < NMB; ++p) {
    const int c0 = p * MB;
    for (int i = p + 1 + wave; i < NMB; i += 4) {
      const int r0 = i * MB;
      v4d acc = {0.0, 0.0, 0.0, 0.0};
#pragma unroll
      for (int s = 0; s < 4; ++s)
        acc = __builtin_amdgcn_mfma_f64_16x16x4f64(frag(T, LDT, r0, c0, s, lane), frag(Xd + p * MB * LDX, LDX, 0, 0, s, lane),
                                                   acc, 0, 0, 0);
      const double sc = SIGNED ? Sg[c0 + (lane & 15)] : 1.0;
#pragma unroll
      for (int r = 0; r < 4; ++r) T[(r0 + (lane >> 4) + 4 * r) * LDT + c0 + (lane & 15)] = SIGNED ? sc * acc[r] : acc[r];
    }
    __syncthreads();
    TS(3 + 2 * p);
    if (p + 1 == NMB) break;
    {
      const int nt = NMB - 1 - p;
      const int ntri = nt * (nt + 1) / 2;
      if (wave == 0) {
        if (p == 3) TS(23);
        trailing_tile(p, 0);
        diag_tile(p + 1);
        if (p == 3) TS(26);
      } else {
        for (int t = wave; t < ntri; t += 3) trailing_tile(p, t);
      }
    }
    __syncthreads();
    TS(4 + 2 * p);
    if (bad_s) return;
  }
  TS(20);

  for (int e = tid; e < NB * NB; e += 256) {
    const int i = e >> 7, j = e & 127;
    if (i < nb && j < nb) A[(int64_t)i * lda + j] = (j <= i) ? T[i * LDT + j] : 0.0;
  }
  __syncthreads(); TS(21);
  for (int pass = 0; pass < 2; ++pass) {
    const int j = pass == 0 ? wave : (NMB - 1 - wave);
    v4d X[NMB];
#pragma unroll
    for (int k = 0; k < NMB; ++k) X[k] = v4d{0.0, 0.0, 0.0, 0.0};
#pragma unroll
    for (int k = 0; k < NMB; ++k) {
      if (k == j) {
#pragma unroll
        for (int r = 0; r < 4; ++r) X[k][r] = Xd[(j * MB + (lane >> 4) + 4 * r) * LDX + (lane & 15)];
      }
    }
#pragma unroll
    for (int i = 1; i < NMB; ++i) {
      if (i > j) {
        v4d acc = {0.0, 0.0, 0.0, 0.0};
#pragma unroll
        for (int k = 0; k < NMB; ++k) {
          if (k >= j && k < i) {
#pragma unroll
            for (int s = 0; s < 4; ++s)
              acc = __builtin_amdgcn_mfma_f64_16x16x4f64(frag(T, LDT, i * MB, k * MB, s, lane), X[k][s], acc, 0, 0, 0);
          }
        }
        v4d out = {0.0, 0.0, 0.0, 0.0};
#pragma unroll
        for (int s = 0; s < 4; ++s)
          out = __builtin_amdgcn_mfma_f64_16x16x4f64(-frag(Xd + i * MB * LDX, LDX, 0, 0, s, lane), acc[s], out, 0, 0, 0);
        X[i] = out;
      }
    }
#pragma unroll
    for (int i = 0; i < NMB; ++i) {
      if (i >= j) {
#pragma unroll
        for (int r = 0; r < 4; ++r) {
          Dinv[(i * MB + (lane >> 4) + 4 * r) * NB + j * MB + (lane & 15)] = X[i][r];
          if (SIGNED) DinvS[(i * MB + (lane >> 4) + 4 * r) * NB + j * MB + (lane & 15)] = Sg[i * MB + (lane >> 4) + 4 * r] * X[i][r];
        }
      }
    }
  }
  __syncthreads(); TS(22);
}

}

int launch_potrf128(mln_ctx* ctx, double* A, int64_t lda, int nb, double* Dinv, int* info, int64_t j0, int nbatch, int64_t a_bs) {
  const size_t lds = sizeof(double) * (size_t)(NB * LDT + NMB * MB * LDX + NB);
  static bool configured = false;
  if (!configured) {
    MLN_HIP(ctx, hipFuncSetAttribute(reinterpret_cast<const void*>(k_potrf128<false>), hipFuncAttributeMaxDynamicSharedMemorySize, (int)lds));
    configured = true;
  }
  hipLaunchKernelGGL(k_potrf128<false>, dim3((unsigned)(nbatch > 1 ? nbatch : 1)), dim3(256), lds, ctx->stream, A, lda, nb, Dinv, info, j0,
                     (double*)nullptr, (int*)nullptr, (unsigned long long*)nullptr, a_bs);
  MLN_HIP(ctx, hipGetLastError());
  return MLN_OK;
}

int launch_potrf128_signed(mln_ctx* ctx, double* A, int64_t lda, int nb, double* Dinv, double* DinvS, int* info, int64_t j0,
                           int* n_neg, unsigned long long* min_piv) {
  const size_t lds = sizeof(double) * (size_t)(NB * LDT + NMB * MB * LDX + NB);
  static bool configured = false;
  if (!configured) {
    MLN_HIP(ctx, hipFuncSetAttribute(reinterpret_cast<const void*>(k_potrf128<true>), hipFuncAttributeMaxDynamicSharedMemorySize, (int)lds));
    configured = true;
  }
  hipLaunchKernelGGL(k_potrf128<true>, dim3(1), dim3(256), lds, ctx->stream, A, lda, nb, Dinv, info, j0, DinvS, n_neg, min_piv, (int64_t)0);
  MLN_HIP(ctx, hipGetLastError());
  return MLN_OK;
}

#ifdef MLN_POTRF_TIMING
extern "C" int mln_diag_potrf_times(long long* out) { return hipMemcpyFromSymbol(out, HIP_SYMBOL(g_potrf_ts), sizeof(long long) * 64) == hipSuccess ? 0 : 1; }
#endif
```

Before: 7.689 million.

## Fuse Gram partial-sum fold with Kj add and gather rows inside int8 Gram

A new fold kernel sums the split-K Gram partials, adds the Kj matrix, and symmetrizes in one pass. This replaces separate sum-partials, symmetrize and axpby launches. The int8 Gram digit kernel now gathers and scales the sampled rows directly, so the preconditioner rebuild no longer materializes R. The potrf128 kernel also computes the diagonal-block inverse tiles while the Cholesky runs, storing them into the spare upper triangle of T, instead of a separate pass at the end. New diagnostic entry points expose these pieces for testing, at the cost of more complex kernels.

Result: no change. 7.774 million, median of 6 (+1.1%).

```diff
diff --git a/include/mellon_hip.h b/include/mellon_hip.h
--- a/include/mellon_hip.h
+++ b/include/mellon_hip.h
@@ -210,6 +210,10 @@
 int mln_diag_dgemm_compare(mln_ctx* ctx, int32_t ta, int32_t tb, int64_t M, int64_t N, int64_t K, int32_t lower_only,
                            int32_t kmode, double beta, int32_t any_size, double* out);
 int mln_diag_gram_i8(mln_ctx* ctx, const double* A, int64_t rows, int64_t m, double* out, int32_t reps, double* ms_out);
+int mln_diag_chol_pair(mln_ctx* ctx, double* A, double* A2, int64_t m, int32_t* bad_out);
+int mln_diag_potrf128(mln_ctx* ctx, double* A, int32_t nb, double* dinv_out, int32_t* info_out);
+int mln_diag_precond_assemble(mln_ctx* ctx, const double* A, int64_t n, int64_t m, const int64_t* idx, const double* scale,
+                              int64_t rows, const double* Kj, double alpha, int32_t fused, double* out);
 int mln_diag_overlap(mln_ctx* ctx, int64_t n, int64_t m, int32_t d, int64_t gram_rows, double* out );
 
 int mln_predict_covariance(mln_ctx* ctx, const mln_kernel_desc* cov, const double* xnew, int64_t n_new,
diff --git a/mellon_amd/_lib.py b/mellon_amd/_lib.py
--- a/mellon_amd/_lib.py
+++ b/mellon_amd/_lib.py
@@ -123,6 +123,9 @@
     ("mln_diag_peak", C.c_int, [_vp, _i32, _i64, C.POINTER(_dbl)]),
     ("mln_diag_overlap", C.c_int, [_vp, _i64, _i64, _i32, _i64, _dp]),
     ("mln_diag_gram_i8", C.c_int, [_vp, _vp, _i64, _i64, _vp, _i32, C.POINTER(_dbl)]),
+    ("mln_diag_chol_pair", C.c_int, [_vp, _vp, _vp, _i64, C.POINTER(_i32)]),
+    ("mln_diag_potrf128", C.c_int, [_vp, _vp, _i32, _vp, C.POINTER(_i32)]),
+    ("mln_diag_precond_assemble", C.c_int, [_vp, _vp, _i64, _i64, _vp, _vp, _i64, _vp, _dbl, _i32, _vp]),
     ("mln_diag_dgemm", C.c_int, [_vp, _i32, _i32, _i64, _i64, _i64, _i32, _i32, _i32, C.POINTER(_dbl)]),
     ("mln_diag_dgemm_compare", C.c_int, [_vp, _i32, _i32, _i64, _i64, _i64, _i32, _i32, _dbl, _i32, C.POINTER(_dbl)]),
 ]
@@ -695,6 +698,45 @@
                                               C.byref(ms)))
         return out, ms.value
 
+    def diag_chol_pair(self, A, A2):
+        A, A2 = _f64(A).copy(), _f64(A2).copy()
+        if A.ndim != 2 or A.shape[0] != A.shape[1] or A2.shape != A.shape:
+            raise ValueError("A and A2 must be square and of one shape")
+        bad = _i32(0)
+        rc = self.lib.mln_diag_chol_pair(self.handle, A.ctypes.data, A2.ctypes.data, A.shape[0], C.byref(bad))
+        if rc not in (MLN_OK, MLN_ERR_NOT_PD):
+            self._check(rc)
+        msg = self.lib.mln_last_error(self.handle).decode() if rc != MLN_OK else ""
+        return rc, int(bad.value), msg, A, A2
+
+    def diag_potrf128(self, A):
+        A = _f64(A).copy()
+        if A.ndim != 2 or A.shape[0] != A.shape[1] or not 1 <= A.shape[0] <= 128:
+            raise ValueError("A must be square with 1 to 128 rows")
+        dinv, info = np.empty((128, 128)), _i32(0)
+        self._check(self.lib.mln_diag_potrf128(self.handle, A.ctypes.data, A.shape[0], dinv.ctypes.data, C.byref(info)))
+        return A, dinv, int(info.value)
+
+    def diag_precond_assemble(self, a, kj=None, alpha=1.0, idx=None, scale=None, fused=True):
+        a = np.ascontiguousarray(a, dtype=np.float64)
+        n, m = a.shape
+        out = np.empty((m, m))
+        ptr = lambda v: None if v is None else v.ctypes.data
+        if kj is not None:
+            kj = np.ascontiguousarray(kj, dtype=np.float64)
+            if kj.shape != (m, m):
+                raise ValueError(f"kj has shape {kj.shape}, expected {(m, m)}")
+        rows = n
+        if idx is not None:
+            idx = np.ascontiguousarray(idx, dtype=np.int64)
+            scale = np.ascontiguousarray(scale, dtype=np.float64)
+            rows = idx.shape[0]
+            if scale.shape != (rows,):
+                raise ValueError("idx and scale must have one entry per sampled row")
+        self._check(self.lib.mln_diag_precond_assemble(self.handle, a.ctypes.data, n, m, ptr(idx), ptr(scale), rows, ptr(kj),
+                                                       float(alpha), 1 if fused else 0, out.ctypes.data))
+        return out
+
     def diag_peak(self, what, nbytes=1 << 32):
         r = C.c_double()
         self._check(self.lib.mln_diag_peak(self.handle, int(what), int(nbytes), C.byref(r)))
diff --git a/mellon_amd/csrc/api.hip b/mellon_amd/csrc/api.hip
--- a/mellon_amd/csrc/api.hip
+++ b/mellon_amd/csrc/api.hip
@@ -357,6 +357,45 @@
   if (add_diag != 0.0) MLN_TRY(launch_add_diag(ctx, o.dev, m, m, add_diag));
   MLN_TRY(dev_cholesky_lower(ctx, o.dev, m, m));
   return o.commit();
+}
+
+extern "C" int mln_diag_chol_pair(mln_ctx* ctx, double* A, double* A2, int64_t m, int32_t* bad_out) {
+  if (!ctx || !A || !A2 || !bad_out || m < 1 || m > 65535) return MLN_ERR_ARG;
+  MLN_HIP(ctx, hipSetDevice(ctx->device));
+  *bad_out = 0;
+  const size_t cnt = (size_t)m * m;
+  DevBuf<double> a, a2;
+  MLN_TRY(a2.alloc(ctx, cnt, "A2"));
+  MLN_TRY(a.alloc(ctx, cnt, "A"));
+  MLN_HIP(ctx, hipMemcpyAsync(a, A, sizeof(double) * cnt, hipMemcpyHostToDevice, ctx->stream));
+  MLN_HIP(ctx, hipMemcpyAsync(a2, A2, sizeof(double) * cnt, hipMemcpyHostToDevice, ctx->stream));
+  int bad = 0;
+  const int rc = dev_cholesky_lower2(ctx, a, a2, m, m, &bad);
+  *bad_out = bad;
+  if (rc != MLN_OK && rc != MLN_ERR_NOT_PD) return rc;
+  MLN_HIP(ctx, hipMemcpyAsync(A, a, sizeof(double) * cnt, hipMemcpyDeviceToHost, ctx->stream));
+  MLN_HIP(ctx, hipMemcpyAsync(A2, a2, sizeof(double) * cnt, hipMemcpyDeviceToHost, ctx->stream));
+  MLN_HIP(ctx, hipStreamSynchronize(ctx->stream));
+  return rc;
+}
+
+extern "C" int mln_diag_potrf128(mln_ctx* ctx, double* A, int32_t nb, double* dinv_out, int32_t* info_out) {
+  if (!ctx || !A || !dinv_out || !info_out || nb < 1 || nb > 128) return MLN_ERR_ARG;
+  MLN_HIP(ctx, hipSetDevice(ctx->device));
+  const size_t cnt = (size_t)nb * nb;
+  DevBuf<double> a, dinv;
+  MLN_TRY(a.alloc(ctx, cnt, "A"));
+  MLN_TRY(dinv.alloc_zeroed(ctx, 128 * 128, "Dinv"));
+  MLN_HIP(ctx, hipMemcpyAsync(a, A, sizeof(double) * cnt, hipMemcpyHostToDevice, ctx->stream));
+  MLN_HIP(ctx, hipMemsetAsync(ctx->d_info, 0, sizeof(int) * 2, ctx->stream));
+  MLN_TRY(launch_potrf128(ctx, a, nb, nb, dinv, ctx->d_info, 0));
+  int info = 0;
+  MLN_HIP(ctx, hipMemcpyAsync(&info, ctx->d_info, sizeof(int), hipMemcpyDeviceToHost, ctx->stream));
+  MLN_HIP(ctx, hipMemcpyAsync(A, a, sizeof(double) * cnt, hipMemcpyDeviceToHost, ctx->stream));
+  MLN_HIP(ctx, hipMemcpyAsync(dinv_out, dinv, sizeof(double) * 128 * 128, hipMemcpyDeviceToHost, ctx->stream));
+  MLN_HIP(ctx, hipStreamSynchronize(ctx->stream));
+  *info_out = info;
+  return MLN_OK;
 }
 
 extern "C" int mln_trsm_lower(mln_ctx* ctx, const double* Lf, int64_t m, int32_t trans, double* B, int64_t p) {
diff --git a/mellon_amd/csrc/api_internal.h b/mellon_amd/csrc/api_internal.h
--- a/mellon_amd/csrc/api_internal.h
+++ b/mellon_amd/csrc/api_internal.h
@@ -150,13 +150,17 @@
 int fit_objective_u(mln_fit* f, const double* u, double* loss, double* grad_u, double* z_out,
                            bool use32 = false);
 int fit_solver_alloc(mln_fit* f, int maxcor);
+struct GramExtra {
+  const double* add = nullptr; int64_t ld_add = 0;
+  const int64_t* idx = nullptr; const double* scale = nullptr;
+};
 int gram_of(mln_ctx* ctx, const double* A, int64_t lda, int64_t rows, int64_t m, double alpha, double* G,
-                   int64_t ldg, bool quantised = false);
+                   int64_t ldg, bool quantised = false, const GramExtra* ex = nullptr);
 int emulated_ranks(const mln_ctx* ctx);
 int fit_ensure_kj(mln_fit* f);
 int fit_ensure_lp(mln_fit* f, bool need_tri = true);
 int fit_lp_finish(mln_fit* f, int rc_chol, double t0);
-int fit_gram(mln_fit* f, double* G, int64_t ldg, int64_t row_stride, bool whiten = true);
+int fit_gram(mln_fit* f, double* G, int64_t ldg, int64_t row_stride, bool whiten = true, const double* add = nullptr);
 int fit_gemvT(mln_fit* f, const double* t_dev, double* rhs_dev);
 int fit_factor_precond(mln_fit* f);
 int fit_build_precond(mln_fit* f, int64_t row_stride);
diff --git a/mellon_amd/csrc/api_precond.hip b/mellon_amd/csrc/api_precond.hip
--- a/mellon_amd/csrc/api_precond.hip
+++ b/mellon_amd/csrc/api_precond.hip
@@ -30,7 +30,12 @@
 }
 
 int gram_of(mln_ctx* ctx, const double* A, int64_t lda, int64_t rows, int64_t m, double alpha, double* G,
-                   int64_t ldg, bool quantised) {
+                   int64_t ldg, bool quantised, const GramExtra* ex) {
+  const double* add = ex ? ex->add : nullptr;
+  const int64_t ld_add = ex ? ex->ld_add : 0;
+  const int64_t* idx = ex ? ex->idx : nullptr;
+  const double* scale = ex ? ex->scale : nullptr;
+  if (idx && !quantised) { mln_set_error(ctx, "gram_of: gathered rows go with the integer Gram only"); return MLN_ERR_ARG; }
   int split = quantised ? gram_i8_splits(rows, m) : (int)(rows / 8192);
   if (split < 1) split = 1;
   if (split > 16 && !quantised) split = 16;
@@ -43,13 +48,20 @@
   g.M = m; g.N = m; g.K = rows; g.alpha = alpha; g.beta = 0.0; g.ta = 1; g.tb = 0; g.lower_only = 1;
   g.split_k = split; g.c_split_stride = (int64_t)stride;
   int rc = MLN_OK;
-  if (split > 1) rc = (hipMemsetAsync(parts, 0, sizeof(double) * stride * split, ctx->stream) == hipSuccess) ? MLN_OK : MLN_ERR_HIP;
-  else rc = (hipMemsetAsync(G, 0, sizeof(double) * stride, ctx->stream) == hipSuccess) ? MLN_OK : MLN_ERR_HIP;
+  if (!quantised || rows <= 0)
+    rc = (hipMemsetAsync(g.C, 0, sizeof(double) * stride * split, ctx->stream) == hipSuccess) ? MLN_OK : MLN_ERR_HIP;
   if (rc == MLN_OK && rows > 0)
-    rc = quantised ? launch_gram_i8(ctx, A, lda, rows, m, alpha, g.C, ldg, (int64_t)stride, split) : launch_dgemm(ctx, g);
-  if (rc == MLN_OK && split > 1) rc = launch_sum_partials(ctx, parts, split, (int64_t)stride, G, (int64_t)stride, 0.0);
-  if (rc == MLN_OK && ctx->n_ranks > 1) rc = allreduce_symmetric_lower(ctx, G, m, ldg);
-  else if (rc == MLN_OK) rc = launch_symmetrize_from_lower(ctx, G, m, ldg);
+    rc = quantised ? launch_gram_i8(ctx, A, lda, rows, m, alpha, g.C, ldg, (int64_t)stride, split, idx, scale) : launch_dgemm(ctx, g);
+  if (rc == MLN_OK && ctx->n_ranks > 1) {
+    rc = launch_gram_fold(ctx, g.C, split, (int64_t)stride, nullptr, 0, G, m, ldg);
+    if (rc == MLN_OK) rc = allreduce_symmetric_lower(ctx, G, m, ldg);
+    if (rc == MLN_OK && add) {
+      if (ld_add != ldg) { mln_set_error(ctx, "gram_of: the added matrix has another row pitch"); rc = MLN_ERR_ARG; }
+      else rc = launch_axpby(ctx, m * ldg, 1.0, add, 1.0, G);
+    }
+  } else if (rc == MLN_OK) {
+    rc = launch_gram_fold(ctx, g.C, split, (int64_t)stride, add, ld_add, G, m, ldg);
+  }
   (void)hipStreamSynchronize(ctx->stream);
   return rc;
 }
@@ -91,6 +103,48 @@
   return rc;
 }
 
+extern "C" int mln_diag_precond_assemble(mln_ctx* ctx, const double* A, int64_t n, int64_t m, const int64_t* idx,
+                                         const double* scale, int64_t rows, const double* Kj, double alpha, int32_t fused,
+                                         double* out) {
+  if (!ctx || !A || !out || n < 1 || m < 1 || rows < 1 || ((idx == nullptr) != (scale == nullptr))) return MLN_ERR_ARG;
+  if (!idx && rows != n) return MLN_ERR_ARG;
+  for (int64_t k = 0; idx && k < rows; ++k)
+    if (idx[k] < 0 || idx[k] >= n) return MLN_ERR_ARG;
+  MLN_HIP(ctx, hipSetDevice(ctx->device));
+  const int64_t ld = (m + 1) & ~(int64_t)1;
+  DevBuf<double> a, kj, sc, R, G;
+  DevBuf<int64_t> ix;
+  DevOut o;
+  MLN_TRY(o.init(ctx, out, (size_t)m * m));
+  MLN_TRY(a.alloc_zeroed(ctx, (size_t)n * ld, "A"));
+  MLN_TRY(G.alloc(ctx, (size_t)m * ld, "G"));
+  MLN_HIP(ctx, hipMemcpy2DAsync(a, sizeof(double) * ld, A, sizeof(double) * m, sizeof(double) * m, (size_t)n, hipMemcpyHostToDevice, ctx->stream));
+  GramExtra ex;
+  if (Kj) {
+    MLN_TRY(kj.alloc_zeroed(ctx, (size_t)m * ld, "Kj"));
+    MLN_HIP(ctx, hipMemcpy2DAsync(kj, sizeof(double) * ld, Kj, sizeof(double) * m, sizeof(double) * m, (size_t)m, hipMemcpyHostToDevice, ctx->stream));
+    ex.add = kj; ex.ld_add = ld;
+  }
+  const double* src = a;
+  if (idx) {
+    MLN_TRY(ix.alloc(ctx, (size_t)rows, "idx"));
+    MLN_TRY(sc.alloc(ctx, (size_t)rows, "scale"));
+    MLN_HIP(ctx, hipMemcpyAsync(ix, idx, sizeof(int64_t) * (size_t)rows, hipMemcpyHostToDevice, ctx->stream));
+    MLN_HIP(ctx, hipMemcpyAsync(sc, scale, sizeof(double) * (size_t)rows, hipMemcpyHostToDevice, ctx->stream));
+    if (fused) { ex.idx = ix; ex.scale = sc; }
+    else {
+      MLN_TRY(R.alloc(ctx, (size_t)rows * ld, "R"));
+      MLN_TRY(launch_gather_scale_rows(ctx, a, ld, ix, sc, rows, R));
+      src = R;
+    }
+  }
+  int rc = gram_of(ctx, src, ld, rows, m, alpha, G, ld, true, &ex);
+  if (rc == MLN_OK) rc = launch_copy_block(ctx, G, ld, o.dev, m, m, m);
+  if (rc == MLN_OK) rc = o.commit();
+  (void)hipStreamSynchronize(ctx->stream);
+  return rc;
+}
+
 int emulated_ranks(const mln_ctx* ctx) {
   if (ctx->n_ranks > 1) return 0;
   if (const char* ev = std::getenv("MELLON_AMD_EMULATE_RANKS")) { const int n = std::atoi(ev); return n > 1 ? n : 0; }
@@ -109,16 +163,19 @@
   return launch_symmetrize_from_lower(ctx, f->Kj, f->m, f->ldp);
 }
 
-int fit_gram(mln_fit* f, double* G, int64_t ldg, int64_t row_stride, bool whiten) {
+int fit_gram(mln_fit* f, double* G, int64_t ldg, int64_t row_stride, bool whiten, const double* add) {
   mln_ctx* ctx = f->ctx;
   if (row_stride < 1) row_stride = 1;
   const int64_t first = (row_stride - f->row0 % row_stride) % row_stride;
   const int64_t rows = (f->n > first) ? (f->n - first + row_stride - 1) / row_stride : 0;
   const double* Ls = f->L + first * f->ldl;
-  if (!f->kspace) return gram_of(ctx, Ls, f->ldl * row_stride, rows, f->m, (double)row_stride, G, ldg);
+  if (add && whiten) return MLN_ERR_ARG;
+  GramExtra ex;
+  ex.add = add; ex.ld_add = f->ldp;
+  if (!f->kspace) return gram_of(ctx, Ls, f->ldl * row_stride, rows, f->m, (double)row_stride, G, ldg, false, &ex);
   bool quant = f->cov_bounded01 && f->m >= 256 && row_stride > 1;
   if (const char* ev = mln_experiment("MELLON_AMD_GRAM_I8")) quant = quant && std::atoi(ev) != 0;
-  int rc = gram_of(ctx, Ls, f->ldl * row_stride, rows, f->m, (double)row_stride, G, ldg, quant);
+  int rc = gram_of(ctx, Ls, f->ldl * row_stride, rows, f->m, (double)row_stride, G, ldg, quant, &ex);
   if (rc != MLN_OK || !whiten) return rc;
   MLN_TRY(fit_ensure_lp(f));
   DevBuf<double> T;
@@ -192,9 +249,8 @@
   const int64_t m = f->m, ldg = f->ldl;
   double t0 = now_s();
   MLN_TRY(f->pc.C.alloc(ctx, (size_t)m * ldg, "C"));
-  int rc = fit_gram(f, f->pc.C, ldg, row_stride, false);
-  if (rc == MLN_OK && f->kspace) rc = fit_ensure_kj(f);
-  if (rc == MLN_OK && f->kspace) rc = launch_axpby(ctx, m * ldg, 1.0, f->Kj, 1.0, f->pc.C);
+  int rc = f->kspace ? fit_ensure_kj(f) : MLN_OK;
+  if (rc == MLN_OK) rc = fit_gram(f, f->pc.C, ldg, row_stride, false, f->kspace ? f->Kj.get() : nullptr);
   MLN_HIP(ctx, hipStreamSynchronize(ctx->stream));
   f->times[3] += now_s() - t0;
   double t1 = now_s();
@@ -234,30 +290,33 @@
     *outcome = 1;
     return MLN_OK;
   }
+  bool quant = f->kspace && f->cov_bounded01 && m >= 256;
+  if (const char* ev = mln_experiment("MELLON_AMD_GRAM_I8")) quant = quant && std::atoi(ev) != 0;
   DevBuf<double> R;
-  const int64_t rr = sel.rows > 0 ? sel.rows : 1;
-  int rc = R.alloc(ctx, (size_t)rr * f->ldl, "R");
-  if (rc == MLN_OK) rc = launch_gather_scale_rows(ctx, f->L, f->ldl, sel.idx, sel.scale, sel.rows, R);
+  int rc = f->kspace ? fit_ensure_kj(f) : MLN_OK;
+  if (rc == MLN_OK && !quant) {
+    const int64_t rr = sel.rows > 0 ? sel.rows : 1;
+    rc = R.alloc(ctx, (size_t)rr * f->ldl, "R");
+    if (rc == MLN_OK) rc = launch_gather_scale_rows(ctx, f->L, f->ldl, sel.idx, sel.scale, sel.rows, R);
+  }
   Precond old = std::move(f->pc);
   if (rc == MLN_OK) rc = f->pc.C.alloc(ctx, (size_t)m * ldg, "C");
   lap(1, tl);
   if (rc == MLN_OK) {
-    bool quant = f->kspace && f->cov_bounded01 && m >= 256;
-    if (const char* ev = mln_experiment("MELLON_AMD_GRAM_I8")) quant = quant && std::atoi(ev) != 0;
-    rc = gram_of(ctx, R, f->ldl, sel.rows, m, sel.w_max, f->pc.C, ldg, quant);
+    GramExtra ex;
+    if (f->kspace) { ex.add = f->Kj; ex.ld_add = f->ldp; }
+    if (quant && sel.rows > 0) { ex.idx = sel.idx; ex.scale = sel.scale; }
+    rc = gram_of(ctx, quant ? f->L : R.get(), f->ldl, sel.rows, m, sel.w_max, f->pc.C, ldg, quant, &ex);
   }
   (void)hipStreamSynchronize(ctx->stream);
   R.reset();
   (void)hipStreamSynchronize(ctx->stream);
   sel.reset();
   lap(2, tl);
-  if (rc == MLN_OK && f->kspace) rc = fit_ensure_kj(f);
-  if (rc == MLN_OK && f->kspace) rc = launch_axpby(ctx, m * ldg, 1.0, f->Kj, 1.0, f->pc.C);
-  lap(3, tl);
   if (rc == MLN_OK) rc = fit_factor_precond(f);
   lap(4, tl);
-  if (tr_on) fprintf(stderr, "[trace] rebuild ms: select %.2f, gather %.2f, gram %.2f, + Kj %.2f, factor+inverses+stacks %.2f (rc %d)\n",
-                     1e3 * tt[0], 1e3 * tt[1], 1e3 * tt[2], 1e3 * tt[3], 1e3 * tt[4], rc);
+  if (tr_on) fprintf(stderr, "[trace] rebuild ms: select %.2f, gather %.2f, gram + Kj %.2f, factor+inverses+stacks %.2f (rc %d)\n",
+                     1e3 * tt[0], 1e3 * tt[1], 1e3 * tt[2], 1e3 * tt[4], rc);
   if (rc != MLN_OK) {
     (void)hipStreamSynchronize(ctx->stream);
     f->pc = std::move(old);
diff --git a/mellon_amd/csrc/gram_i8.hip b/mellon_amd/csrc/gram_i8.hip
--- a/mellon_amd/csrc/gram_i8.hip
+++ b/mellon_amd/csrc/gram_i8.hip
@@ -18,6 +18,7 @@
 __device__ __forceinline__ void lds_barrier() { asm volatile("s_waitcnt lgkmcnt(0)\n\ts_barrier" ::: "memory"); }
 
 __global__ __launch_bounds__(256) void k_gram_digits(const double* __restrict__ K, int64_t ldk, int64_t rows, int64_t m,
+                                                     const int64_t* __restrict__ idx, const double* __restrict__ scale,
                                                      int8_t* __restrict__ planes, int64_t Mp, int64_t Kp) {
   __shared__ uint32_t tile[3][64][17];
   const int t = threadIdx.x, li = t & 63, kq = t >> 6;
@@ -31,7 +32,7 @@
     for (int e = 0; e < 4; ++e) {
       const int64_t k = k0 + g * 4 + e;
       double v = 0.0;
-      if (k < rows && gi < m) v = K[k * ldk + gi];
+      if (k < rows && gi < m) v = idx ? K[idx[k] * ldk + gi] * scale[k] : K[k * ldk + gi];
       v = fmin(fmax(v, 0.0), 1.0);
       const int q = (int)rint(v * (double)GQ_SCALE);
       const int d0 = ((q + 128) & 255) - 128;
@@ -219,8 +220,9 @@
 }
 
 int launch_gram_i8(mln_ctx* ctx, const double* K, int64_t ldk, int64_t rows, int64_t m, double alpha, double* parts,
-                   int64_t ldg, int64_t part_stride, int n_splits) {
+                   int64_t ldg, int64_t part_stride, int n_splits, const int64_t* idx, const double* scale) {
   if (rows <= 0 || m <= 0) return MLN_OK;
+  if ((idx == nullptr) != (scale == nullptr)) return MLN_ERR_ARG;
   const int64_t T = (m + GT - 1) / GT, Mp = T * GT;
   int64_t kchunk = (rows + n_splits - 1) / n_splits;
   kchunk = (kchunk + GBK - 1) / GBK * GBK;
@@ -242,7 +244,7 @@
   if (e != hipSuccess) rc = mln_hip_fail(ctx, e, "upload Gram tile list", __FILE__, __LINE__);
   if (rc == MLN_OK) {
     hipLaunchKernelGGL(k_gram_digits, dim3((unsigned)(Kp / 64), (unsigned)(Mp / 64)), dim3(256), 0, ctx->stream, K, ldk, rows, m,
-                       planes, Mp, Kp);
+                       idx, scale, planes.get(), Mp, Kp);
     static bool attr_set = false;
     const int lds_bytes = 2 * GSTAGE;
     if (!attr_set) {
diff --git a/mellon_amd/csrc/linalg.hip b/mellon_amd/csrc/linalg.hip
--- a/mellon_amd/csrc/linalg.hip
+++ b/mellon_amd/csrc/linalg.hip
@@ -128,6 +128,47 @@
   }
 }
 
+__global__ __launch_bounds__(256) void k_gram_fold(const double* parts, int n_parts, int64_t stride, const double* __restrict__ add,
+                                                   int64_t ld_add, double* out, int64_t m, int64_t ld) {
+  __shared__ double tile[32][33];
+  const int64_t bi = blockIdx.y, bj = blockIdx.x;
+  if (bj > bi) return;
+  const int tx = threadIdx.x, ty = threadIdx.y;
+  for (int r = ty; r < 32; r += 8) {
+    const int64_t i = bi * 32 + r, j = bj * 32 + tx;
+    double v = 0.0;
+    if (i < m && j <= i) {
+      double s = 0.0;
+      for (int p = 0; p < n_parts; ++p) s += parts[(int64_t)p * stride + i * ld + j];
+      v = add ? add[i * ld_add + j] + s : s;
+    }
+    tile[r][tx] = v;
+  }
+  __syncthreads();
+  for (int r = ty; r < 32; r += 8) {
+    const int64_t i = bi * 32 + r, j = bj * 32 + tx;
+    if (i < m && j <= i) out[i * ld + j] = tile[r][tx];
+    const int64_t iu = bj * 32 + r, ju = bi * 32 + tx;
+    if (ju < m && ju > iu) out[iu * ld + ju] = tile[tx][r];
+  }
+  if (bj == 0) {
+    for (int r = ty; r < 32; r += 8) {
+      const int64_t i = bi * 32 + r;
+      if (i < m)
+        for (int64_t j = m + tx; j < ld; j += 32) out[i * ld + j] = (add && j < ld_add) ? add[i * ld_add + j] : 0.0;
+    }
+  }
+}
+
+}
+
+int launch_gram_fold(mln_ctx* ctx, const double* parts, int n_parts, int64_t stride, const double* add, int64_t ld_add,
+                     double* out, int64_t m, int64_t ld) {
+  if (m <= 0) return MLN_OK;
+  const unsigned t = (unsigned)((m + 31) / 32);
+  hipLaunchKernelGGL(k_gram_fold, dim3(t, t), dim3(32, 8), 0, ctx->stream, parts, n_parts, stride, add, ld_add, out, m, ld);
+  MLN_HIP(ctx, hipGetLastError());
+  return MLN_OK;
 }
 
 int launch_transpose(mln_ctx* ctx, const double* src, int64_t lds, double* dst, int64_t ldd, int64_t m) {
diff --git a/mellon_amd/csrc/mln_internal.h b/mellon_amd/csrc/mln_internal.h
--- a/mellon_amd/csrc/mln_internal.h
+++ b/mellon_amd/csrc/mln_internal.h
@@ -42,11 +42,13 @@
 int dev_cholesky_lower2(mln_ctx* ctx, double* A, double* A2, int64_t m, int64_t lda, int* bad);
 int launch_add_diag(mln_ctx* ctx, double* A, int64_t m, int64_t lda, double v);
 int launch_symmetrize_from_lower(mln_ctx* ctx, double* A, int64_t m, int64_t lda);
+int launch_gram_fold(mln_ctx* ctx, const double* parts, int n_parts, int64_t stride, const double* add, int64_t ld_add,
+                     double* out, int64_t m, int64_t ld);
 int dev_sym_rank_above(mln_ctx* ctx, double* A, int64_t m, int64_t ld, double tol2, int64_t* rank, double* lambda_max);
 int dev_sym_rank_above_ldl(mln_ctx* ctx, double* A, int64_t m, int64_t ld, double tol2, int64_t* rank, double* lambda_max, bool* ok);
 int gram_i8_splits(int64_t rows, int64_t m);
 int launch_gram_i8(mln_ctx* ctx, const double* K, int64_t ldk, int64_t rows, int64_t m, double alpha, double* parts,
-                   int64_t ldg, int64_t part_stride, int n_splits);
+                   int64_t ldg, int64_t part_stride, int n_splits, const int64_t* idx = nullptr, const double* scale = nullptr);
 int launch_axpby(mln_ctx* ctx, int64_t n, double a, const double* x, double b, double* y);
 
 int launch_kernel_grad(mln_ctx* ctx, const DevCov& cov, const double* x, int64_t n, const double* y, int64_t m,
diff --git a/mellon_amd/csrc/potrf.hip b/mellon_amd/csrc/potrf.hip
--- a/mellon_amd/csrc/potrf.hip
+++ b/mellon_amd/csrc/potrf.hip
@@ -238,6 +238,34 @@
     for (int r = 0; r < 4; ++r) T[(r0 + (lane >> 4) + 4 * r) * LDT + q0 + (lane & 15)] = acc[r];
   };
 
+  auto x_tile = [&](int i, int j) {
+    v4d out;
+    if (j == i) {
+#pragma unroll
+      for (int r = 0; r < 4; ++r) out[r] = Xd[(i * MB + (lane >> 4) + 4 * r) * LDX + (lane & 15)];
+    } else {
+      v4d acc = {0.0, 0.0, 0.0, 0.0};
+      for (int k = j; k < i; ++k) {
+#pragma unroll
+        for (int s = 0; s < 4; ++s) {
+          const double b = (k == j) ? Xd[(j * MB + 4 * s + (lane >> 4)) * LDX + (lane & 15)] : frag(T, LDT, j * MB, k * MB, s, lane);
+          acc = __builtin_amdgcn_mfma_f64_16x16x4f64(frag(T, LDT, i * MB, k * MB, s, lane), b, acc, 0, 0, 0);
+        }
+      }
+      out = v4d{0.0, 0.0, 0.0, 0.0};
+#pragma unroll
+      for (int s = 0; s < 4; ++s)
+        out = __builtin_amdgcn_mfma_f64_16x16x4f64(-frag(Xd + i * MB * LDX, LDX, 0, 0, s, lane), acc[s], out, 0, 0, 0);
+#pragma unroll
+      for (int r = 0; r < 4; ++r) T[(j * MB + (lane & 15)) * LDT + i * MB + 4 * r + (lane >> 4)] = out[r];
+    }
+#pragma unroll
+    for (int r = 0; r < 4; ++r) {
+      Dinv[(i * MB + (lane >> 4) + 4 * r) * NB + j * MB + (lane & 15)] = out[r];
+      if (SIGNED) DinvS[(i * MB + (lane >> 4) + 4 * r) * NB + j * MB + (lane & 15)] = Sg[i * MB + (lane >> 4) + 4 * r] * out[r];
+    }
+  };
+
   if (wave == 0) diag_tile(0);
   __syncthreads();
   TS(2);
@@ -268,6 +296,7 @@
         if (p == 3) TS(26);
       } else {
         for (int t = wave; t < ntri; t += 3) trailing_tile(p, t);
+        for (int j = wave - 1; j <= p; j += 3) x_tile(p, j);
       }
     }
     __syncthreads();
@@ -275,54 +304,13 @@
     if (bad_s) return;
   }
   TS(20);
+  for (int j = wave; j < NMB; j += 4) x_tile(NMB - 1, j);
 
   for (int e = tid; e < NB * NB; e += 256) {
     const int i = e >> 7, j = e & 127;
     if (i < nb && j < nb) A[(int64_t)i * lda + j] = (j <= i) ? T[i * LDT + j] : 0.0;
   }
-  __syncthreads(); TS(21);
-  for (int pass = 0; pass < 2; ++pass) {
-    const int j = pass == 0 ? wave : (NMB - 1 - wave);
-    v4d X[NMB];
-#pragma unroll
-    for (int k = 0; k < NMB; ++k) X[k] = v4d{0.0, 0.0, 0.0, 0.0};
-#pragma unroll
-    for (int k = 0; k < NMB; ++k) {
-      if (k == j) {
-#pragma unroll
-        for (int r = 0; r < 4; ++r) X[k][r] = Xd[(j * MB + (lane >> 4) + 4 * r) * LDX + (lane & 15)];
-      }
-    }
-#pragma unroll
-    for (int i = 1; i < NMB; ++i) {
-      if (i > j) {
-        v4d acc = {0.0, 0.0, 0.0, 0.0};
-#pragma unroll
-        for (int k = 0; k < NMB; ++k) {
-          if (k >= j && k < i) {
-#pragma unroll
-            for (int s = 0; s < 4; ++s)
-              acc = __builtin_amdgcn_mfma_f64_16x16x4f64(frag(T, LDT, i * MB, k * MB, s, lane), X[k][s], acc, 0, 0, 0);
-          }
-        }
-        v4d out = {0.0, 0.0, 0.0, 0.0};
-#pragma unroll
-        for (int s = 0; s < 4; ++s)
-          out = __builtin_amdgcn_mfma_f64_16x16x4f64(-frag(Xd + i * MB * LDX, LDX, 0, 0, s, lane), acc[s], out, 0, 0, 0);
-        X[i] = out;
-      }
-    }
-#pragma unroll
-    for (int i = 0; i < NMB; ++i) {
-      if (i >= j) {
-#pragma unroll
-        for (int r = 0; r < 4; ++r) {
-          Dinv[(i * MB + (lane >> 4) + 4 * r) * NB + j * MB + (lane & 15)] = X[i][r];
-          if (SIGNED) DinvS[(i * MB + (lane >> 4) + 4 * r) * NB + j * MB + (lane & 15)] = Sg[i * MB + (lane >> 4) + 4 * r] * X[i][r];
-        }
-      }
-    }
-  }
+  TS(21);
   __syncthreads(); TS(22);
 }
 
```
